# YuemingJin/STswinCL

Hardware: AMD Instinct MI355X
Metric: input frames/s, TswinPlus fwd+bwd+Adam, 4-frame 512x512 clips (higher is better)
Workload: dtype bf16; 1 GPU; BASELINE.json configs[1]: TswinPlus(12) seg train step, 4 clips/GPU x T=4 frames x 3x512x512, swin res (64,64), OHEM-CE, Adam; T=4 because the reference asserts it (swin_512.py:313); clips_per_gpu=4, frames_per_clip=4, parallelism=dp1, graph_requested=True

## Files before the change

include/stswin_hip.h:

```cpp
#ifndef STSWIN_HIP_H
#define STSWIN_HIP_H
#ifdef __cplusplus
extern "C" {
#endif

#define STSWIN_GF_GELU 1
#define STSWIN_GF_RESID 2
#define STSWIN_GF_MUL_DGELU 4
#define STSWIN_GF_OUT_F32 8
#define STSWIN_GF_ACCUM 16
#define STSWIN_GF_RELU 32
#define STSWIN_GF_MUL_R 8192
#define STSWIN_GF_C2_DGELU 16384
#define STSWIN_GF_CS_PARTIAL 32768
#define STSWIN_GF_CS_SQ 65536
#define STSWIN_GF_TAPSKIP (1 << 29)
#define STSWIN_GF_BIG 128
#define STSWIN_GF_MID 512
#define STSWIN_GF_NOPIPE 1024
#define STSWIN_GF_HALF 2048
#define STSWIN_GF_M32PP (1u << 31)
#define STSWIN_GF_W4R (1 << 30)
#define STSWIN_GF_ROT 4096
#define STSWIN_GF_NOBIG 256
#define STSWIN_GF_WAVES4 64
#define STSWIN_GF_NOREGEPI (1 << 22)
#define STSWIN_GF_NOSTREAM (1 << 23)
#define STSWIN_GF_DUO (1 << 24)
#define STSWIN_GF_STREAM (1 << 25)
#define STSWIN_GF_NONARROW (1 << 26)
#define STSWIN_GF_NODEEP (1 << 27)
#define STSWIN_GF_DEEP (1 << 28)

int stswin_abi_version(void);

int stswin_win_rowmap(int* map, int B, int T, int H, int W, int ws, int shift, int f0, int frames_total, void* stream);
int stswin_win_move(int dtype, const void* in, void* out, int B, int T, int H, int W, int C, int ws, int shift,
                    int f0, int frames_total, int dir, void* stream);
int stswin_merge_rowmap(int* map , int frames, int H, int W, void* stream);
int stswin_conv3x3_rowmap(int* map , int frames, int H, int W, int dilation, void* stream);
int stswin_conv_rowmap(int* map, int frames, int Hin, int Win, int Hout, int Wout, int k, int stride, int pad, int dilation,
                       int inverse, void* stream);
int stswin_stem_im2col(int dtype, const float* img, void* patches, long ld, int frames, int H, int W, int Ho, int Wo,
                       void* stream);
int stswin_stem_s2d(int dtype, const float* img, void* out, int frames, int H, int W, void* stream);
int stswin_stem_conv(const void* rec, const void* wmat, void* y, float* stats, int frames, int H, int W, void* stream);
long stswin_stem_wgrad_scratch(int frames, int Ho, int Wo);
int stswin_stem_wgrad(const void* dy, const void* rec, float* dw, int accumulate, float* scratch, long scratch_floats, int frames, int H, int W,
                      void* stream);
int stswin_conv_pack(int dtype, const float* w, void* fwd, void* dgrad, const int* omap, const int* imap, int co, int ci, int S,
                     int cop, int cip, void* stream);
int stswin_linear_pack(int dtype, const float* w, void* fwd, void* tr, int n, int k, void* stream);
int stswin_linear_pack_multi(int dtype, int count, const float* const* w, void* const* fwd, void* const* tr, const int* n, const int* k,
                             void* stream);
int stswin_conv_pack_multi(int dtype, int count, const float* const* w, void* const* fwd, void* const* dgrad, const int* const* omap,
                           const int* const* imap, const int* ci, const int* S, const int* cop, const int* cip, void* stream);
int stswin_maxpool3x3s2(int dtype, const void* in, long ldi, void* out, long ldo, unsigned char* arg, int frames, int H,
                        int W, int Ho, int Wo, int C, int backward, void* stream);
int stswin_conv3x3_c64(const void* x, const void* wmat, void* y, const void* resid, float* stats, int frames, int H, int W, int sign,
                       void* stream);
long stswin_conv3x3_c64_wgrad_scratch(int frames, int H, int W);
int stswin_conv3x3_c64_wgrad(const void* dy, const void* x, float* dw, int tapminor, int accumulate, float* scratch, long scratch_floats,
                             int frames, int H, int W, void* stream);

int stswin_gemm_nt(int dtype, const void* A, long lda, const int* a_rows, const void* B, long ldb, void* C, long ldc,
                   const int* c_rows, void* C2, long ldc2, const float* bias, const void* R, long ldr,
                   const int* r_rows, int M, int N, int Kseg, int S, float scale, int scale_cols, int flags,
                   float* colsum , void* stream);
int stswin_cs_reduce(const float* partials, int M, int N, float* out, void* stream);
#define STSWIN_TN_OVERWRITE (1 << 27)
#define STSWIN_TN_NO_COMBINE (1 << 26)
long stswin_gemm_nt_splitk_scratch(int M, int N, int Kseg, int S);
int stswin_gemm_nt_splitk(const void* A, long lda, const int* a_rows, const void* B, long ldb, void* C, long ldc, const float* bias, int M, int N,
                          int Kseg, int S, int relu, float* workspace, long workspace_floats, void* stream);
int stswin_tn_fused_hold(int delta);
int stswin_set_cu_budget(int cus);
int stswin_gemm_tn(int dtype, const void* At, long lda, const int* at_rows, const void* Bt, long ldb, const int* bt_rows,
                   float* C, long ldc, int Mk, int Ni, int Nj, int splits, int bseg,
                   float* workspace , long workspace_floats, void* stream);
#define STSWIN_TN_GROUP_DECLINED (-1050)
typedef struct stswin_tn_problem {
  const void* At; long lda; const int* at_rows;
  const void* Bt; long ldb; const int* bt_rows;
  float* C; long ldc;
  int Mk, Ni, Nj, bseg;
  int overwrite;
  int tapminor;
} stswin_tn_problem;
int stswin_gemm_tn_group(int dtype, int count, const stswin_tn_problem* problems, float* workspace, long workspace_floats, int* splits_out,
                         void* stream);
int stswin_tn_combine(const float* workspace, float* C, long ldc, int Ni, int Nj, int splits, int overwrite, int slab_bf16,
                      void* stream);
#define STSWIN_VAR_F32 100
#define STSWIN_VAR_NT_RING256_REGEPI 1
#define STSWIN_VAR_NT_RING256_LDSEPI 2
#define STSWIN_VAR_NT_RING256_NOPIPE 3
#define STSWIN_VAR_NT_RING256_W4 14
#define STSWIN_VAR_NT_STREAM 4
#define STSWIN_VAR_NT_DUO 5
#define STSWIN_VAR_NT_RING256x128_PP 6
#define STSWIN_VAR_NT_MID 7
#define STSWIN_VAR_NT_256x64 8
#define STSWIN_VAR_NT_128x64 9
#define STSWIN_VAR_NT_128x128 10
#define STSWIN_VAR_NT_128x128_W4 11
#define STSWIN_VAR_NT_SPLITK 13
#define STSWIN_VAR_NT_ROWS 12
#define STSWIN_VAR_TN_RING_PLAIN 20
#define STSWIN_VAR_TN_RING_ATROWS 21
#define STSWIN_VAR_TN_RING_BTROWS 22
#define STSWIN_VAR_TN_RING_BSEG 23
#define STSWIN_VAR_TN_128x128 30
#define STSWIN_VAR_TN_128x128_W4 31
#define STSWIN_VAR_TN_ROWS 32
#define STSWIN_VAR_TN_SLABS_F32 0x1000
#define STSWIN_VAR_TN_SLABS_BF16 0x2000
#define STSWIN_VAR_TN_FUSED 0x8000
#define STSWIN_VAR_TN_TAPMINOR 0x4000
#define STSWIN_TN_OUT_TAPMINOR (1 << 25)
int stswin_gemm_nt_qkv_fp8(const void* A, long lda, const int* a_rows, const void* B, long ldb, void* out8, long ld8, float* scales,
                           long ld_scales, const float* bias, int M, int N, int Kseg, float scale, int scale_cols, int rows_per_problem,
                           int head_dim, void* stream);
int stswin_win_attn_fwd_f8(const void* qkv8, long ld8, const float* scales, long ld_scales, void* out, long ldo, const float* biasT,
                           const float* maskT, int nB_, int nW, int T_frames, int ws, int heads, int C, int bias_windows,
                           const int* bias_index, void* stream);
int stswin_win_attn_bwd_f8(const void* qkv8, long ld8, const float* scales, long ld_scales, const void* dout, long lddo, void* dqkv, long lddq,
                           const float* biasT, const float* maskT, float* dbiasT, float* dqkv_colsum, int nB_, int nW, int T_frames, int ws,
                           int heads, int C, float scale, int bias_windows, const int* bias_index, float* scratch, long scratch_floats,
                           void* stream);
int stswin_last_variant(int family);
int stswin_tuning_build(void);

int stswin_slab_fold(const float* ws, long slab_stride, long ws_batch_stride, int nslabs, int seg_len, int nseg, float* out0, float* out1,
                     float* out2, long out_batch_stride, int batch, int accumulate, void* stream);

int stswin_fold_defer(int on, void* stream);
int stswin_fold_flush(void* stream);

long stswin_colsum_scratch(int M, int N);
int stswin_colsum(int dtype, const void* y, long ldy, float* out, int M, int N, float* scratch, void* stream);

int stswin_layernorm_fwd(int dtype, const void* x, long ldx, const int* rows, int S, int Cseg, void* y, long ldy,
                         const float* gamma, const float* beta, float* mean, float* rstd, int M, float eps, void* stream);
int stswin_layernorm_bwd(int dtype, const void* dy, long lddy, const void* x, long ldx, const int* rows, int S, int Cseg,
                         const float* gamma, const float* mean, const float* rstd, void* dx, long lddx, float* dgamma,
                         float* dbeta, int M, int accumulate_dx,
                         float* dxsum ,
                         float* scratch ,
                         void* stream);
int stswin_layernorm_bwd_add(int dtype, const void* dy, long lddy, const void* x, long ldx, const int* rows, int S, int Cseg,
                             const float* gamma, const float* mean, const float* rstd, const void* add, long ldadd, void* dx, long lddx,
                             float* dgamma, float* dbeta, int M, float* dxsum, float* scratch, void* stream);
long stswin_layernorm_bwd_scratch(int M, int C);

int stswin_vec_gather(const float* v, const int* map, float* out, int n, float fill, void* stream);
int stswin_vec_gather_multi(int count, const float* const* v, const int* map, float* const* out, int n, const float* fill, void* stream);

int stswin_bias_expand(const float* table, const long* index, const float* mask, float* out, int N, int heads, int nW,
                       void* stream);
int stswin_bias_expand_multi(int count, const float* const* table, const long* const* index, const float* const* mask, float* const* out,
                             const int* N, const int* heads, const int* nW, void* stream);
int stswin_bias_scatter(const float* dbiasT, const int* order, const int* offs, float* dtable, int N, int heads, int table_rows, int nslabs,
                        void* stream);

int stswin_win_attn_fwd(int dtype, const void* qkv, long ld, void* out, long ldo, const float* biasT, const float* maskT,
                        int nB_, int nW, int T_frames, int ws, int heads, int C, int bias_windows,
                        const int* bias_index, void* stream);
int stswin_win_attn_qkv_fwd(const void* x, long ldx, long x_rows, const int* rmap, const void* w, long ldw, const float* bqkv, void* qkv_out,
                            long ldq, void* out, long ldo, const float* biasT, int nB_, int nW, int T_frames, int ws, int heads, int C,
                            float scale, int bias_windows, const int* bias_index, void* stream);
int stswin_win_attn_fwd_fp8(const void* qkv, long ld, void* out, long ldo, const float* biasT, const float* maskT, int nB_, int nW,
                            int T_frames, int ws, int heads, int C, int bias_windows, const int* bias_index, void* stream);
int stswin_win_attn_bwd(int dtype, const void* qkv, long ld, const void* dout, long lddo, void* dqkv, long lddq,
                        const float* biasT, const float* maskT, float* dbiasT,
                        float* dqkv_q_colsum ,
                        int nB_, int nW, int T_frames, int ws,
                        int heads, int C, float scale, int bias_windows, const int* bias_index,
                        float* scratch , long scratch_floats, void* stream);
long stswin_win_attn_bwd_scratch(int nB_, int ws, int heads, int C);

int stswin_colstats(int dtype, const void* x, long ldx, float* sum , float* sumsq , int M, int C, int groups, int unit_rows,
                    float* scratch , void* stream);
long stswin_colstats_scratch(int dtype, int M, int C, int groups, int unit_rows);
int stswin_cs_group_reduce(const float* table, int M, int N, int groups, int unit_rows, float* sum, float* sumsq, void* stream);

int stswin_bn_table_finalize(const float* table, int M, int N, int groups, int unit_rows, float* mean, float* rstd,
                             float* running_mean, float* running_var, float eps, float momentum, void* stream);
int stswin_bn_finalize(int dtype, const void* x, long ldx, const float* sum, const float* sumsq, float* mean, float* rstd,
                       float* running_mean, float* running_var, int M, int C, int groups, float eps, float momentum,
                       int unit_rows, void* stream);
int stswin_bn_apply(int dtype, const void* x, long ldx, const float* mean, const float* rstd, const float* gamma,
                    const float* beta, const void* resid, long ldr, void* y, long ldy, int M, int C, int groups, int relu,
                    int unit_rows, void* stream);
int stswin_bn_bwd(int dtype, const void* dy, long lddy, const void* x, long ldx,
                  const void* y ,
                  long ldy, const float* mean, const float* rstd, const float* gamma, const float* beta ,
                  float* s1, float* s2, void* dx, long lddx, void* dresid, long lddr,
                  int M, int C, int groups, int relu, int training,
                  int phase ,
                  long rows_total , int unit_rows,
                  float* group_sums ,
                  float* scratch ,
                  void* stream);
long stswin_bn_bwd_scratch(int dtype, int M, int C, int groups, int unit_rows);
int stswin_bn_relu_pool(int dtype, const void* x, long ldx, const float* mean, const float* rstd, const float* gamma, const float* beta,
                        void* out, long ldo, unsigned char* arg, int frames, int H, int W, int C, int groups, int unit_rows, void* stream);
int stswin_rows_broadcast(int dtype, const float* v, void* out, long ldo, int M, int C, int groups, float scale,
                          int accumulate, void* stream);
int stswin_bilinear(int dtype, const void* in, long ldi, void* out, long ldo, int frames, int h, int w, int H, int W, int C,
                    int backward, void* stream);
int stswin_logits_upsample(int dtype, const void* tokens, long ldt, void* nchw, int frames, int h, int w, int H, int W,
                           int nc, int backward, void* stream);

int stswin_ce_fwd(int dtype, const void* logits, const long* labels, float* loss, float* stats, int frames, long HW, int nc,
                  int ignore_index, float thresh, void* stream);
#define STSWIN_OHEM_WORK_BYTES (3 * 2048 * 12 + 48)
int stswin_ohem_select(const float* loss, long n, long n_min, float thresh, const float* stats, void* work, long work_bytes,
                       float* value, float* sel, void* stream);
int stswin_ce_bwd(int dtype, const void* logits, const long* labels, const float* loss, const float* sel,
                  const float* gscale, void* dlogits, int frames, long HW, int nc, int ignore_index, void* stream);

int stswin_contrast_fwd(int dtype, const void* Q, long ldq, const void* const* K5, long ldk, const int* lq,
                        const int* const* lk5, float* pos, float* all, int N, int HW, int C, void* stream);

int stswin_contrast_bank_fwd(int dtype, const void* Q, long ldq, const int* lq, int M, int C, int q_sets, int q_block,
                             const void* bank, long ldb, const int* lb, int maps, int seg, int bank_block, int groups,
                             const int* gmap , float inv_tau, float* pos, float* all,
// ... 130 lines not shown
```

stswincl_amd/csrc/gemm.hip:

```cpp
#include "common.h"
#include "stswin_hip.h"
#include <cstdint>
#include <cstdlib>
#include <type_traits>

enum {
  GF_GELU = STSWIN_GF_GELU, GF_RESID = STSWIN_GF_RESID, GF_MUL_DGELU = STSWIN_GF_MUL_DGELU, GF_OUT_F32 = STSWIN_GF_OUT_F32,
  GF_ACCUM = STSWIN_GF_ACCUM, GF_RELU = STSWIN_GF_RELU, GF_MUL_R = STSWIN_GF_MUL_R, GF_C2_DGELU = STSWIN_GF_C2_DGELU,
  GF_CS_PARTIAL = STSWIN_GF_CS_PARTIAL, GF_CS_SQ = STSWIN_GF_CS_SQ, GF_TAPSKIP = STSWIN_GF_TAPSKIP,
  GF_WAVES4 = STSWIN_GF_WAVES4, GF_BIG = STSWIN_GF_BIG, GF_NOBIG = STSWIN_GF_NOBIG, GF_MID = STSWIN_GF_MID, GF_NOPIPE = STSWIN_GF_NOPIPE,
  GF_HALF = STSWIN_GF_HALF, GF_ROT = STSWIN_GF_ROT, GF_NOREGEPI = STSWIN_GF_NOREGEPI, GF_NOSTREAM = STSWIN_GF_NOSTREAM,
  GF_DUO = STSWIN_GF_DUO, GF_STREAM = STSWIN_GF_STREAM, GF_NONARROW = STSWIN_GF_NONARROW, GF_NODEEP = STSWIN_GF_NODEEP,
  GF_DEEP = STSWIN_GF_DEEP, GF_W4R = STSWIN_GF_W4R, GF_M32PP = (int)STSWIN_GF_M32PP,
};

#ifdef STSWIN_TUNING
#define STSWIN_DBG(flags, bit) (((flags) & (1 << (bit))) != 0)
#else
#define STSWIN_DBG(flags, bit) false
#endif
enum { GF_DEBUG_BITS = (1 << 17) | (1 << 18) | (1 << 19) | (1 << 20) | (1 << 21) };
#ifdef STSWIN_TUNING
static __device__ int g_dbg_stagger[2] = {8, 0};
extern "C" int stswin_debug_set_stagger(int phases, int ticks) {
// ... 216 lines not shown
    char* Bb = Ab + A_BYTES;
#pragma unroll
    for (int i = 0; i < NIA; ++i) glds16(abase[i] + (long)kt * astep[i], Ab + (w * NIA + i) * 1024);
#pragma unroll
    for (int i = 0; i < NIB; ++i) glds16(bbase[i] + (long)ktg * bstep[i], Bb + (w * NIB + i) * 1024);
  };

  f32x4 acc[4][JN];
#pragma unroll
  for (int i = 0; i < 4; ++i)
#pragma unroll
    for (int j = 0; j < JN; ++j) acc[i][j] = (f32x4){0.f, 0.f, 0.f, 0.f};

  int seg = 0, rseg = real_seg(0);
  load_a_bases(rseg);
  auto issue = [&](int tile) {
    const int nseg = tile / kps;
    if (nseg != seg) { seg = nseg; rseg = real_seg(seg); load_a_bases(rseg); }
    stage(rseg * kps + (tile - nseg * kps), tile - nseg * kps, tile % NST);
  };
#pragma unroll
  for (int s0 = 0; s0 < NST - 1; ++s0)
    if (s0 < nt) issue(s0);
  const int fr = l & 15, fq = l >> 4;
  for (int ktg = 0; ktg < nt; ++ktg) {
    if constexpr (NST == 2) {
      wait_vm0();
      __syncthreads();
    } else {
      if (ktg + NST - 1 <= nt) wait_vmcnt<(NST - 2) * (NIA + NIB)>();
      else wait_vm0();
      __builtin_amdgcn_s_barrier();
    }
    if (ktg + NST - 1 < nt) issue(ktg + NST - 1);
    const char* Ab = smem + (ktg % NST) * STAGE;
    const char* Bb = Ab + A_BYTES;
    if constexpr (TT<T>::IS_BF16) {
#pragma unroll
      for (int kk = 0; kk < 2; ++kk) {
        bf16x8 a[4], b[JN];
#pragma unroll
        for (int i = 0; i < 4; ++i) {
          const int row = wr * 64 + i * 16 + fr;
          a[i] = *(const bf16x8*)(Ab + row * ROWB + (((kk * 4 + fq) ^ (row & 7)) << 4));
        }
#pragma unroll
        for (int j = 0; j < JN; ++j) {
          const int row = wc * (16 * JN) + j * 16 + fr;
          b[j] = *(const bf16x8*)(Bb + row * ROWB + (((kk * 4 + fq) ^ (row & 7)) << 4));
        }
#pragma unroll
        for (int i = 0; i < 4; ++i)
#pragma unroll
          for (int j = 0; j < JN; ++j) acc[i][j] = __builtin_amdgcn_mfma_f32_16x16x32_bf16(a[i], b[j], acc[i][j], 0, 0, 0);
      }
    } else {
#pragma unroll
      for (int kk = 0; kk < 8; ++kk) {
        float a[4], b[JN];
#pragma unroll
        for (int i = 0; i < 4; ++i) {
          const int row = wr * 64 + i * 16 + fr;
          a[i] = *(const float*)(Ab + row * ROWB + ((kk ^ (row & 7)) << 4) + fq * 4);
        }
#pragma unroll
        for (int j = 0; j < JN; ++j) {
          const int row = wc * (16 * JN) + j * 16 + fr;
          b[j] = *(const float*)(Bb + row * ROWB + ((kk ^ (row & 7)) << 4) + fq * 4);
        }
#pragma unroll
        for (int i = 0; i < 4; ++i)
#pragma unroll
          for (int j = 0; j < JN; ++j) acc[i][j] = __builtin_amdgcn_mfma_f32_16x16x4f32(a[i], b[j], acc[i][j], 0, 0, 0);
      }
    }
  }

  constexpr int CG = BN / 8;
  const int c8 = (tid % CG) * 8;
  const int gn0 = n0 + c8;
  const int ncols = max(0, min(8, p.N - gn0));
  constexpr int RG = NW * 64 / CG;
  constexpr int NPASS = BM / RG;
  const bool pre_r = (p.flags & (GF_RESID | GF_MUL_DGELU | GF_MUL_R)) && ncols == 8 && (p.ldr % PACK) == 0;
  Vec16<T> rp[NPASS][8 / PACK];
  if (pre_r) {
#pragma unroll
    for (int pass = 0; pass < NPASS; ++pass) {
      const int gm = m0 + pass * RG + tid / CG;
      if (gm < p.M) epi_prefetch<T>(p, rp[pass], gm, gn0);
    }
  }
  __syncthreads();
  float* ct = (float*)smem;
#pragma unroll
  for (int i = 0; i < 4; ++i)
#pragma unroll
    for (int j = 0; j < JN; ++j)
#pragma unroll
      for (int r = 0; r < 4; ++r)
        ct[(wr * 64 + i * 16 + 4 * fq + r) * BN + wc * (16 * JN) + j * 16 + fr] = acc[i][j][r];
  __syncthreads();

  float bv[8], cs[8], cs2[8];
#pragma unroll
  for (int e = 0; e < 8; ++e) { bv[e] = (p.bias && e < ncols) ? p.bias[gn0 + e] : 0.f; cs[e] = 0.f; cs2[e] = 0.f; }
#pragma unroll
  for (int pass = 0; pass < NPASS; ++pass) {
    const int rr = pass * RG + tid / CG;
    const int gm = m0 + rr;
    if (gm >= p.M || ncols <= 0) break;
    float v[8];
    {
      const f32x4 lo = *(const f32x4*)(ct + rr * BN + c8);
      const f32x4 hi = *(const f32x4*)(ct + rr * BN + c8 + 4);
#pragma unroll
      for (int e = 0; e < 4; ++e) { v[e] = lo[e]; v[4 + e] = hi[e]; }
    }
    epi_piece<T>(p, v, bv, cs, gm, gn0, ncols, rp[pass], pre_r);
    if (p.flags & GF_CS_SQ) {
#pragma unroll
      for (int e = 0; e < 8; ++e) cs2[e] += v[e] * v[e];
    }
  }
  if (p.colsum) {
    __syncthreads();
#pragma unroll
    for (int e = 0; e < 8; ++e) ct[(tid / CG) * BN + c8 + e] = cs[e];
    __syncthreads();
    if (tid < BN && n0 + tid < p.N) {
      float t = 0.f;
#pragma unroll
      for (int k = 0; k < RG; ++k) t += ct[k * BN + tid];
      cs_emit(p, m0 / 128, BM / 128, n0 + tid, t);
    }
    if (p.flags & GF_CS_SQ) {
      __syncthreads();
#pragma unroll
      for (int e = 0; e < 8; ++e) ct[(tid / CG) * BN + c8 + e] = cs2[e];
      __syncthreads();
      if (tid < BN && n0 + tid < p.N) {
        float t = 0.f;
#pragma unroll
        for (int k = 0; k < RG; ++k) t += ct[k * BN + tid];
        cs_emit_sq(p, m0 / 128, BM / 128, n0 + tid, t);
      }
    }
  }
}


DEVI int swz64(int row) { return (4 - ((row >> 2) & 3)) & 3; }

template <int BM, int BN, int WM, int WN, int NST, int MINW, int PIPE, bool SWAP = false, bool PERSIST = false>
__global__ __launch_bounds__(WM * WN * 64, MINW) void gemm_nt_ring_kernel(GemmNT p) {
  using T = bf16;
  constexpr int BK = 32, ROWB = 64;
  constexpr int A_BYTES = BM * ROWB, B_BYTES = BN * ROWB, STAGE = A_BYTES + B_BYTES;
  constexpr int TM = BM / WM, TN = BN / WN;
  constexpr bool M32 = PIPE >= 2 && PIPE <= 4;
  constexpr int FRH = M32 ? 32 : 16, FCW = M32 ? 8 : 16;
  constexpr int FI = TM / FRH, FJ = TN / FCW;
  constexpr int NWV = WM * WN, NTHR = NWV * 64;
  constexpr int NIA = BM / 16 / NWV, NIB = BN / 16 / NWV;
  constexpr int PER_STAGE = NIA + NIB;
  constexpr int EROWS = SWAP ? BM : ((NST * STAGE) / (BN * 4) >= BM ? BM : ((NST * STAGE) / (BN * 4) / TM) * TM);
  static_assert(SWAP || (EROWS >= TM && BM % EROWS == 0), "epilogue slab");
  static_assert(!SWAP || BM * BN * 2 <= NST * STAGE, "register epilogue image");
  extern __shared__ __attribute__((aligned(16))) char smem[];
  const int tiles_n = (p.N + BN - 1) / BN, tiles_m = (p.M + BM - 1) / BM;
  const int ntot_ = tiles_m * tiles_n;
  int tix_ = blockIdx.x;
  do {
  int tid_ = threadIdx.x;
  if constexpr (PERSIST) asm volatile("" : "+v"(tid_));
  const int tid = tid_, l = tid & 63, w = __builtin_amdgcn_readfirstlane(tid >> 6);
  const int wr = w / WN, wc = w % WN;
  const int t = xcd_remap(tix_, ntot_);
  int tm = t / tiles_n, tn = t % tiles_n;
  if (tiles_n >= 24) {
    constexpr int GM = 8;
    const int per_group = GM * tiles_n, grp = t / per_group, first = grp * GM;
    const int rows = min(GM, tiles_m - first), in = t - grp * per_group;
    tm = first + in % rows;
    tn = in / rows;
  }
  const int m0 = tm * BM, n0 = tn * BN;

  const int rsub = l >> 2, cphys = l & 3, csrc = cphys ^ swz64(rsub);
  unsigned aoff[NIA], boff[NIB];
  const long arow_lim = (long)(0xFFFFFF00u / (unsigned)(p.lda * sizeof(T))) - 1;
  bool arow_bad = false;
#pragma unroll
  for (int i = 0; i < NIB; ++i) {
    const int gn = n0 + (w * NIB + i) * 16 + rsub;
    boff[i] = gn < p.N ? (unsigned)gn * (unsigned)(p.ldb * sizeof(T)) + csrc * 16 : 0xFFFFFFFFu;
  }
  auto load_a_bases = [&](int seg) {
#pragma unroll
    for (int i = 0; i < NIA; ++i) {
      const int gm = m0 + (w * NIA + i) * 16 + rsub;
      long row = -1;
      if (gm < p.M) row = p.a_rows ? (long)p.a_rows[(long)seg * p.M + gm] : (long)gm;
      aoff[i] = (row >= 0 && row <= arow_lim) ? (unsigned)row * (unsigned)(p.lda * sizeof(T)) + csrc * 16 : 0xFFFFFFFFu;
      arow_bad |= row > arow_lim;
    }
  };
  const int kps = p.Kseg / BK;
  const int qbase = p.qsplit > 0 ? (int)blockIdx.y * p.qsplit : 0;
  const int nt = p.qsplit > 0 ? min(p.qsplit, p.S * kps - qbase) : p.S * kps;
  if (p.qsplit > 0) p.C = (char*)p.C + (long)blockIdx.y * p.M * p.ldc * ((p.flags & GF_OUT_F32) ? 4 : 2);
  int seg = -1;
  auto issue = [&](int q) {
    const int Q = q + qbase;
    int sg = 0, kt = Q;
    if (p.S > 1) { sg = Q / kps; kt = Q - sg * kps; }
    if (sg != seg) { seg = sg; load_a_bases(sg); }
    char* Ab = smem + (q % NST) * STAGE;
    char* Bb = Ab + A_BYTES;
#pragma unroll
    for (int i = 0; i < NIA; ++i) glds16_buf(p.A, aoff[i], kt * (BK * (int)sizeof(T)), Ab + (w * NIA + i) * 1024);
#pragma unroll
    for (int i = 0; i < NIB; ++i) glds16_buf(p.B, boff[i], Q * (BK * (int)sizeof(T)), Bb + (w * NIB + i) * 1024);
  };

  f32x4 acc[M32 ? 1 : FI][M32 ? 1 : FJ];
  f32x16 acc32[M32 ? FI : 1][M32 ? FJ / 4 : 1];
  auto accg = [&](int i, int j) __attribute__((always_inline)) -> f32x4 {
    if constexpr (M32) {
      const int o = (j & 3) * 4;
      return (f32x4){acc32[i][j >> 2][o], acc32[i][j >> 2][o + 1], acc32[i][j >> 2][o + 2], acc32[i][j >> 2][o + 3]};
    } else return acc[i][j];
  };
  auto accs = [&](int i, int j, f32x4 v) __attribute__((always_inline)) {
    if constexpr (M32) {
      const int o = (j & 3) * 4;
      acc32[i][j >> 2][o] = v[0]; acc32[i][j >> 2][o + 1] = v[1]; acc32[i][j >> 2][o + 2] = v[2]; acc32[i][j >> 2][o + 3] = v[3];
    } else acc[i][j] = v;
  };

  const int fr = M32 ? (l & 31) : (l & 15), fq = M32 ? (l >> 5) : (l >> 4), fr15 = fr & 15;
  const int rd_off = fr * ROWB + ((fq ^ swz64(fr)) << 4);
  const int rd_off1 = rd_off ^ 32;
  const bool dbg_ts = STSWIN_DBG(p.flags, 19);
#ifdef STSWIN_TUNING
  unsigned long long dbg_c0 = 0;
  auto stamp = [&](int slot) {
    if (dbg_ts && tid == 0) {
      ((unsigned long long*)p.colsum)[(long)blockIdx.x * 16 + slot] = wall_clock64();
      if (slot == 2) dbg_c0 = clock64();
      if (slot == 3) ((unsigned long long*)p.colsum)[(long)blockIdx.x * 16 + 7] = clock64() - dbg_c0;
    }
  };
#else
  auto stamp = [&](int) {};
#endif
  constexpr bool R_EARLY_OK = SWAP && BM == 256 && BN == 256 && NST == 4 && PER_STAGE == 4 && NTHR == 512;
  bool r_early = false;
  auto issue_r_block = [&](int blk) {
#pragma unroll
    for (int qq = 0; qq < 4; ++qq) {
      const int row = (blk * 4 + qq) * 16 + w * 2 + (l >> 5);
      const int col = min(n0 + (((l & 31) ^ (row & 15)) << 3), p.N - 8);
      glds16_nt((const T*)p.R + (long)min(m0 + row, p.M - 1) * p.ldr + col, smem + ((blk * 4 + qq) * 16 + w * 2) * 512);
    }
  };
#ifdef STSWIN_TUNING
  if (STSWIN_DBG(p.flags, 17) && blockIdx.x < 256) {
    const int ph = g_dbg_stagger[0] > 0 ? g_dbg_stagger[0] : 8, tk = g_dbg_stagger[1] > 0 ? g_dbg_stagger[1] : (nt + 4) * 100 / 8;
    const unsigned long long t_go = wall_clock64() + (unsigned long long)(((blockIdx.x >> 3) % ph) * tk);
    while (wall_clock64() < t_go) __builtin_amdgcn_s_sleep(8);
  }
#endif
  stamp(0);
  auto epilogue = [&]() {
    if (STSWIN_DBG(p.flags, 21)) {
      float t = 0.f;
#pragma unroll
      for (int i = 0; i < FI; ++i)
#pragma unroll
        for (int j = 0; j < FJ; ++j) { const f32x4 q = accg(i, j); t += q[0] + q[1] + q[2] + q[3]; }
      if (t == 123.456f) ((T*)p.C)[tid] = from_f32<T>(t);
      return;
    }
    float* ct = (float*)smem;
    constexpr int CG = BN / 8;
    constexpr int RGP = NTHR / CG;
    const int c8 = (tid % CG) * 8;
    const int gn0 = n0 + c8;
    const int ncols = max(0, min(8, p.N - gn0));
    float bv[8], cs[8];
#pragma unroll
    for (int e = 0; e < 8; ++e) { bv[e] = (p.bias && e < ncols) ? p.bias[gn0 + e] : 0.f; cs[e] = 0.f; }
    constexpr int NPASS = EROWS / RGP;
    const bool pre_r = (p.flags & (GF_RESID | GF_MUL_DGELU | GF_MUL_R)) && ncols == 8 && (p.ldr % 8) == 0;
    Vec16<T> rp[NPASS][1];
#pragma unroll 1
    for (int slab = 0; slab < BM / EROWS; ++slab) {
      if (pre_r) {
#pragma unroll
        for (int pass = 0; pass < NPASS; ++pass) {
          const int gm = m0 + slab * EROWS + pass * RGP + tid / CG;
          if (gm < p.M) epi_prefetch<T>(p, rp[pass], gm, gn0);
        }
      }
      __syncthreads();
      if (wr * TM >= slab * EROWS && wr * TM < (slab + 1) * EROWS) {
        const int rbase = wr * TM - slab * EROWS;
#pragma unroll
        for (int i = 0; i < FI; ++i)
#pragma unroll
          for (int j = 0; j < FJ; ++j)
#pragma unroll
            for (int r = 0; r < 4; ++r) { if constexpr (!M32) ct[(rbase + i * 16 + 4 * fq + r) * BN + wc * TN + j * 16 + fr] = acc[i][j][r]; }
      }
      __syncthreads();
#pragma unroll
      for (int pass = 0; pass < NPASS; ++pass) {
        const int rr = pass * RGP + tid / CG;
        const int gm = m0 + slab * EROWS + rr;
        if (gm >= p.M || ncols <= 0) break;
        float v[8];
        const f32x4 lo = *(const f32x4*)(ct + rr * BN + c8);
        const f32x4 hi = *(const f32x4*)(ct + rr * BN + c8 + 4);
#pragma unroll
        for (int e = 0; e < 4; ++e) { v[e] = lo[e]; v[4 + e] = hi[e]; }
        epi_piece<T>(p, v, bv, cs, gm, gn0, ncols, rp[pass], pre_r);
      }
    }
    if (p.colsum) {
      __syncthreads();
#pragma unroll
      for (int e = 0; e < 8; ++e) ct[(tid / CG) * BN + c8 + e] = cs[e];
      __syncthreads();
      if (tid < BN && n0 + tid < p.N) {
        float tsum = 0.f;
#pragma unroll
        for (int k = 0; k < RGP; ++k) tsum += ct[k * BN + tid];
        cs_emit(p, m0 / 128, BM / 128, n0 + tid, tsum);
      }
    }

  };

  enum { E_BIAS = 1, E_SCALE = 2, E_GELU = 4, E_C2 = 8, E_RESID = 16, E_DGELU = 32, E_COLSUM = 64, E_RELU = 128, E_MULR = 256, E_C2D = 512,
         E_COLSQ = 1024 };
  auto epilogue_body = [&](auto tag) __attribute__((always_inline)) {
    constexpr int MD = decltype(tag)::value;
#define EPI_HAS(bit, rt) (MD >= 0 ? ((MD & (bit)) != 0) : (rt))
    constexpr int PITCH = BN * 2, CPRW = BN / 8, RPP = NTHR / CPRW, NPASS = BM / RPP;
    char* img = smem;
    const bool has_bias = EPI_HAS(E_BIAS, p.bias != nullptr), has_scale = EPI_HAS(E_SCALE, p.scale_cols > 0);
    const bool do_gelu = EPI_HAS(E_GELU, (p.flags & GF_GELU) != 0), has_c2 = EPI_HAS(E_C2, p.C2 != nullptr);
    const bool do_resid = EPI_HAS(E_RESID, (p.flags & GF_RESID) != 0), do_dgelu = EPI_HAS(E_DGELU, (p.flags & GF_MUL_DGELU) != 0);
    const bool do_cs = EPI_HAS(E_COLSUM, p.colsum != nullptr) && !dbg_ts, do_relu = EPI_HAS(E_RELU, (p.flags & GF_RELU) != 0);
    const bool do_mulr = EPI_HAS(E_MULR, (p.flags & GF_MUL_R) != 0), c2_dgelu = EPI_HAS(E_C2D, (p.flags & GF_C2_DGELU) != 0);
    const bool do_sq = do_cs && EPI_HAS(E_COLSQ, (p.flags & GF_CS_SQ) != 0);
    const bool has_r = do_resid || do_dgelu || do_mulr;
    const int colb = n0 + wc * TN + 4 * fq;
    f32x4 bj[FJ];
    if (has_bias) {
#pragma unroll
      for (int j = 0; j < FJ; ++j) bj[j] = *(const f32x4*)(p.bias + min(colb + j * FCW, p.N - 4));
    }
// ... 296 lines not shown
  };
  if constexpr (PIPE != 4) {
    for (int q = 0; q < (PIPE == 7 ? NST : NST - 1) && q < nt; ++q) issue(q);
  }
  if (p.stagger_ticks > 0 && blockIdx.x < 256 && gridDim.y == 1) {
    const unsigned long long t_go = wall_clock64() + (unsigned long long)(((blockIdx.x >> 3) & 7) * p.stagger_ticks);
    while (wall_clock64() < t_go) __builtin_amdgcn_s_sleep(8);
  }
  __builtin_amdgcn_sched_barrier(0);
  if constexpr (M32) {
#pragma unroll
    for (int i = 0; i < FI; ++i)
#pragma unroll
      for (int j = 0; j < FJ / 4; ++j)
#pragma unroll
        for (int e = 0; e < 16; ++e) acc32[i][j][e] = 0.f;
  } else {
#pragma unroll
    for (int i = 0; i < FI; ++i)
#pragma unroll
      for (int j = 0; j < FJ; ++j) acc[i][j] = (f32x4){0.f, 0.f, 0.f, 0.f};
  }
#ifdef STSWIN_TUNING
#include "gemm_nt_ring_tuning.inc"
#else
  static_assert(PIPE == 1 && !PERSIST, "the product library instantiates the ping-pong loop only (other loops: STSWIN_TUNING builds)");
#endif
  {
    static_assert(NST >= 4 && WM == 2, "ping-pong variant: 4-stage ring, two wave rows");
    const bool lag = (wr == 1);
    constexpr int NA = M32 ? 2 * FI : FI, NB = M32 ? FJ / 2 : FJ;
    bf16x8 a[NA], b[NB];
    auto read_frags = [&](int q) {
      const char* Ab = smem + (q % NST) * STAGE;
      const char* Bb = Ab + A_BYTES;
      if constexpr (M32) {
#pragma unroll
        for (int g = 0; g < NB; ++g) b[g] = *(const bf16x8*)(Bb + (wc * TN + (g >> 1) * 32) * ROWB + ((g & 1) ? rd_off1 : rd_off));
#pragma unroll
        for (int g = 0; g < NA; ++g) a[g] = *(const bf16x8*)(Ab + (wr * TM + (g >> 1) * 32) * ROWB + ((g & 1) ? rd_off1 : rd_off));
      } else {
#ifdef STSWIN_DEBUG_HALF_READS
#pragma unroll
      for (int j = 0; j < FJ; j += 2) { b[j] = *(const bf16x8*)(Bb + (wc * TN + j * 16) * ROWB + rd_off); b[j + 1] = b[j]; }
#pragma unroll
      for (int i = 0; i < FI; i += 2) { a[i] = *(const bf16x8*)(Ab + (wr * TM + i * 16) * ROWB + rd_off); a[i + 1] = a[i]; }
#else
#pragma unroll
      for (int j = 0; j < FJ; ++j) b[j] = *(const bf16x8*)(Bb + (wc * TN + j * 16) * ROWB + rd_off);
#pragma unroll
      for (int i = 0; i < FI; ++i) a[i] = *(const bf16x8*)(Ab + (wr * TM + i * 16) * ROWB + rd_off);
#endif
      }
    };
    auto mma_all = [&]() {
      __builtin_amdgcn_s_setprio(1);
      if constexpr (M32) {
        static_assert(!M32 || SWAP, "32x32x16 tiles: register epilogue only");
#pragma unroll
        for (int kh = 0; kh < 2; ++kh)
#pragma unroll
          for (int i = 0; i < FI; ++i)
#pragma unroll
            for (int j = 0; j < FJ / 4; ++j)
              acc32[i][j] = __builtin_amdgcn_mfma_f32_32x32x16_bf16(b[j * 2 + kh], a[i * 2 + kh], acc32[i][j], 0, 0, 0);
      } else {
#pragma unroll
      for (int i = 0; i < FI; ++i)
#pragma unroll
        for (int j = 0; j < FJ; ++j) {
          if constexpr (SWAP) acc[i][j] = __builtin_amdgcn_mfma_f32_16x16x32_bf16(b[j], a[i], acc[i][j], 0, 0, 0);
          else acc[i][j] = __builtin_amdgcn_mfma_f32_16x16x32_bf16(a[i], b[j], acc[i][j], 0, 0, 0);
        }
      }
      __builtin_amdgcn_s_setprio(0);
    };
    auto wait_tile = [&](int kt) {
      const int newer = min(NST - 2, nt - 1 - kt);
      if (newer >= 2) wait_vmcnt<2 * PER_STAGE>();
      else if (newer == 1) wait_vmcnt<PER_STAGE>();
      else wait_vmcnt<0>();
    };
    stamp(1);
    wait_tile(0);
    stamp(2);
    if (lag) __builtin_amdgcn_s_barrier();
    int kt = 0;
    if (p.S == 1) {
      for (; kt + NST - 1 < nt; ++kt) {
#ifdef STSWIN_DEBUG_LOOP_STAMPS
        if (kt == 4) stamp(1);
        if (kt == 8) stamp(2);
        if (kt == 12) stamp(7);
#endif
        __builtin_amdgcn_s_barrier();
        issue(kt + NST - 1);
        read_frags(kt);
        wait_vmcnt<2 * PER_STAGE>();
        __builtin_amdgcn_s_barrier();
        mma_all();
      }
      if constexpr (R_EARLY_OK) {
        if ((p.flags & (GF_RESID | GF_MUL_R | GF_MUL_DGELU)) && !p.r_rows && kt + NST - 1 == nt && !STSWIN_DBG(p.flags, 18)) {
          r_early = true;
          for (; kt < nt; ++kt) {
            __builtin_amdgcn_s_barrier();
            issue_r_block((kt + NST - 1) % NST);
            read_frags(kt);
            wait_vmcnt<2 * PER_STAGE>();
            __builtin_amdgcn_s_barrier();
            mma_all();
          }
        }
      }
      if (kt + NST - 1 == nt && NST == 4) {
        __builtin_amdgcn_s_barrier();
        read_frags(kt);
        wait_vmcnt<PER_STAGE>();
        __builtin_amdgcn_s_barrier();
        mma_all();
        ++kt;
        __builtin_amdgcn_s_barrier();
        read_frags(kt);
        wait_vmcnt<0>();
        __builtin_amdgcn_s_barrier();
        mma_all();
        ++kt;
        __builtin_amdgcn_s_barrier();
        read_frags(kt);
        __builtin_amdgcn_s_barrier();
        mma_all();
        ++kt;
      }
    }
    for (; kt < nt; ++kt) {
      __builtin_amdgcn_s_barrier();
      if (kt + NST - 1 < nt) issue(kt + NST - 1);
      read_frags(kt);
      if (lag && kt + 1 < nt) wait_tile(kt + 1);
      __builtin_amdgcn_s_barrier();
      mma_all();
      if (!lag && kt + 1 < nt) wait_tile(kt + 1);
    }
    if (!lag) __builtin_amdgcn_s_barrier();
    if (arow_bad) __builtin_trap();
    if constexpr (SWAP) epilogue_reg();
    else epilogue();
  }
  if constexpr (PERSIST) {
    tix_ += (int)gridDim.x;
    if (tix_ < ntot_) __syncthreads();
  }
  } while (PERSIST && tix_ < ntot_);
}


#ifdef STSWIN_TUNING
#include "gemm_nt_tuning_kernels.inc"
#endif

struct GemmTN {
  const void* At; long lda; const int* at_rows;
  const void* Bt; long ldb; const int* bt_rows;
  float* C; long ldc;
  int Mk, Ni, Nj;
  int splits;
  int bseg;
  float* slabs;
  int slab_bf16;
  unsigned* tile_cnt; int overwrite; int perm;
};

template <typename T, int NW>
__global__ __launch_bounds__(NW * 64) void gemm_tn_kernel(GemmTN p) {
  constexpr int WN = NW / 2, JN = 128 / WN / 16;
  constexpr int PACK = TT<T>::PACK;
  constexpr int BM = TT<T>::IS_BF16 ? 64 : 32;
  constexpr int ROWB = 128 * sizeof(T);
  constexpr int RPI = 1024 / ROWB;
  constexpr int NI = BM / (NW * RPI);
  constexpr int CPR = ROWB / 16;
  extern __shared__ __attribute__((aligned(16))) char smem[];
  const int tid = threadIdx.x, l = tid & 63, w = wave_id();
  const int wr = w / WN, wc = w % WN;
  const int tiles_j = (p.Nj + 127) >> 7;
  const int split_id = blockIdx.x % p.splits, tile_id = blockIdx.x / p.splits;
  const int i0 = (tile_id / tiles_j) << 7, j0 = (tile_id % tiles_j) << 7;
  const int ntile_all = (p.Mk + BM - 1) / BM;
  const int per = (ntile_all + p.splits - 1) / p.splits;
  const int t_begin = split_id * per, t_end = min(ntile_all, t_begin + per);
  if (t_begin >= t_end) return;

  const char* zero = (const char*)g_stswin_zero;
  const int rsub = l / CPR, cphys = l % CPR;
  long arow[NI], brow[NI];
  int bcol[NI];
  bool btap1[NI];
  const int tap0 = p.bseg > 0 ? j0 / p.bseg : 0;
  const int tap1 = p.bseg > 0 ? min(tap0 + 1, p.Nj / p.bseg - 1) : 0;
#pragma unroll
  for (int i = 0; i < NI; ++i) {
    const int r = (w * NI + i) * RPI + rsub;
    const int cj = j0 + ((cphys & ~15) | ((cphys ^ swz256(r)) & 15)) * PACK;
    bcol[i] = p.bseg > 0 ? cj % p.bseg : cj;
    btap1[i] = p.bseg > 0 && cj / p.bseg != tap0;
  }
  typedef int ivec __attribute__((ext_vector_type(RPI)));
  typedef const __attribute__((address_space(4))) ivec* civec;
  const bool vec_maps = (p.Mk % RPI) == 0;
  auto fetch_rows = [&](int tile) {
    const int mw = tile * BM + w * (NI * RPI);
#pragma unroll
    for (int i = 0; i < NI; ++i) {
      const int mb = mw + i * RPI;
      int va[RPI], vb0[RPI], vb1[RPI];
      if (vec_maps && mb + RPI <= p.Mk) {
        ivec ta, t0, t1;
#pragma unroll
        for (int r = 0; r < RPI; ++r) { ta[r] = mb + r; t0[r] = mb + r; t1[r] = -1; }
        if (p.at_rows) ta = *(civec)(p.at_rows + mb);
        if (p.bseg > 0) {
          t0 = *(civec)(p.bt_rows + (long)tap0 * p.Mk + mb);
          t1 = *(civec)(p.bt_rows + (long)tap1 * p.Mk + mb);
        } else if (p.bt_rows) {
          t0 = *(civec)(p.bt_rows + mb);
        }
#pragma unroll
        for (int r = 0; r < RPI; ++r) { va[r] = ta[r]; vb0[r] = t0[r]; vb1[r] = t1[r]; }
      } else {
#pragma unroll
        for (int r = 0; r < RPI; ++r) {
          const int m = mb + r, mc = min(m, p.Mk - 1);
          va[r] = p.at_rows ? sload(p.at_rows, mc) : mc;
          vb1[r] = -1;
          if (p.bseg > 0) {
            vb0[r] = sload(p.bt_rows, (long)tap0 * p.Mk + mc);
            vb1[r] = sload(p.bt_rows, (long)tap1 * p.Mk + mc);
          } else {
            vb0[r] = p.bt_rows ? sload(p.bt_rows, mc) : mc;
          }
          if (m >= p.Mk) { va[r] = -1; vb0[r] = -1; vb1[r] = -1; }
        }
      }
      int ra = -1, rb = -1;
#pragma unroll
      for (int r = 0; r < RPI; ++r)
        if (rsub == r) { ra = va[r]; rb = btap1[i] ? vb1[r] : vb0[r]; }
      arow[i] = ra; brow[i] = rb;
    }
  };
  auto stage = [&](int buf) {
    char* Ab = smem + buf * 32768;
    char* Bb = Ab + 16384;
#pragma unroll
    for (int i = 0; i < NI; ++i) {
      const int r = (w * NI + i) * RPI + rsub;
      const int cs = (cphys & ~15) | ((cphys ^ swz256(r)) & 15);
      const int ci = i0 + cs * PACK, cj = j0 + cs * PACK;
      const char* sa = (arow[i] >= 0 && ci < p.Ni) ? (const char*)p.At + (arow[i] * p.lda + ci) * sizeof(T) : zero;
      const char* sb = (brow[i] >= 0 && cj < p.Nj) ? (const char*)p.Bt + (brow[i] * p.ldb + bcol[i]) * sizeof(T) : zero;
      glds16_raw(sa, Ab + (w * NI + i) * 1024);
      glds16_raw(sb, Bb + (w * NI + i) * 1024);
    }
  };

  f32x4 acc[4][JN];
#pragma unroll
  for (int i = 0; i < 4; ++i)
#pragma unroll
    for (int j = 0; j < JN; ++j) acc[i][j] = (f32x4){0.f, 0.f, 0.f, 0.f};

  const int fr = l & 15, fq = l >> 4;
  const bool row_active = i0 + wr * 64 < p.Ni;
  fetch_rows(t_begin);
  stage(0);
  if (t_begin + 1 < t_end) fetch_rows(t_begin + 1);
  for (int tk = t_begin; tk < t_end; ++tk) {
    const int buf = (tk - t_begin) & 1;
    wait_vm0();
    __syncthreads();
    if (tk + 1 < t_end) stage(buf ^ 1);
    const char* Ab = smem + buf * 32768;
    const char* Bb = Ab + 16384;
    if (!row_active) {
    } else if constexpr (TT<T>::IS_BF16) {
#pragma unroll
      for (int kk = 0; kk < 2; ++kk) {
        bf16x8 a[4], b[JN];
#pragma unroll
        for (int i = 0; i < 4; ++i)
          a[i] = cat4(lds_tr4(Ab, ROWB, kk * 32 + 8 * fq, wr * 64 + i * 16),
                      lds_tr4(Ab, ROWB, kk * 32 + 8 * fq + 4, wr * 64 + i * 16));
#pragma unroll
        for (int j = 0; j < JN; ++j)
          b[j] = cat4(lds_tr4(Bb, ROWB, kk * 32 + 8 * fq, wc * (16 * JN) + j * 16),
                      lds_tr4(Bb, ROWB, kk * 32 + 8 * fq + 4, wc * (16 * JN) + j * 16));
#pragma unroll
        for (int i = 0; i < 4; ++i)
#pragma unroll
          for (int j = 0; j < JN; ++j) acc[i][j] = __builtin_amdgcn_mfma_f32_16x16x32_bf16(a[i], b[j], acc[i][j], 0, 0, 0);
      }
    } else {
#pragma unroll
      for (int kk = 0; kk < 8; ++kk) {
        const int row = kk * 4 + fq;
        float a[4], b[JN];
// ... 380 lines not shown
  const int seq = xcd_remap((int)blockIdx.x, (int)gridDim.x);
  if constexpr (M3 >= 0) {
    if (seq >= g.first[3]) { gemm_tn_ring_body<M3 < 0 ? 0 : M3, true>(g.q[3], seq - g.first[3], g.first[4] - g.first[3], (int)blockIdx.x); return; }
  }
  if constexpr (M2 >= 0) {
    if (seq >= g.first[2]) { gemm_tn_ring_body<M2 < 0 ? 0 : M2, true>(g.q[2], seq - g.first[2], g.first[3] - g.first[2], (int)blockIdx.x); return; }
  }
  if constexpr (M1 >= 0) {
    if (seq >= g.first[1]) { gemm_tn_ring_body<M1 < 0 ? 0 : M1, true>(g.q[1], seq - g.first[1], g.first[2] - g.first[1], (int)blockIdx.x); return; }
  }
  gemm_tn_ring_body<M0, true>(g.q[0], seq, g.first[1], (int)blockIdx.x);
}
__global__ __launch_bounds__(512, 2) void gemm_tn_ring_group_kernel(GemmTNGroup g) {
  const int seq = xcd_remap((int)blockIdx.x, (int)gridDim.x);
  int i = 0;
  while (i + 1 < g.count && seq >= g.first[i + 1]) ++i;
  const int local = seq - g.first[i], nwg = g.first[i + 1] - g.first[i];
  switch (g.mode[i]) {
    case 0: gemm_tn_ring_body<0, true>(g.q[i], local, nwg, (int)blockIdx.x); break;
    case 1: gemm_tn_ring_body<1, true>(g.q[i], local, nwg, (int)blockIdx.x); break;
    case 2: gemm_tn_ring_body<2, true>(g.q[i], local, nwg, (int)blockIdx.x); break;
    default: gemm_tn_ring_body<3, true>(g.q[i], local, nwg, (int)blockIdx.x); break;
  }
}

__global__ __launch_bounds__(256) void tn_reduce_kernel(const float* slabs, float* C, long ldc, int Ni, int Nj, int splits,
                                                        int overwrite, int slab_bf16, int perm) {
  if (slab_bf16) {
    const long idx = ((long)blockIdx.x * 256 + threadIdx.x) * 8;
    const long total = (long)Ni * Nj;
    if (idx >= total) return;
    const int i = idx / Nj, j = idx % Nj;
    float a[8] = {0.f, 0.f, 0.f, 0.f, 0.f, 0.f, 0.f, 0.f};
    const bf16* src = (const bf16*)slabs + idx;
    int s = 0;
    for (; s + 8 <= splits; s += 8) {
      bf16x8 v[8];
#pragma unroll
      for (int u = 0; u < 8; ++u) v[u] = *(const bf16x8*)(src + (long)(s + u) * total);
#pragma unroll
      for (int u = 0; u < 8; ++u)
#pragma unroll
        for (int e = 0; e < 8; ++e) a[e] += (float)v[u][e];
    }
    for (; s < splits; ++s) {
      const bf16x8 v = *(const bf16x8*)(src + (long)s * total);
#pragma unroll
      for (int e = 0; e < 8; ++e) a[e] += (float)v[e];
    }
    if (perm > 0) {
      const int S = Nj / perm, sg = j / perm, c = j - sg * perm;
      float* d = C + (long)i * ldc + (long)c * S + sg;
#pragma unroll
      for (int e = 0; e < 8; ++e) d[(long)e * S] = overwrite ? a[e] : d[(long)e * S] + a[e];
      return;
    }
    float* dst = C + (long)i * ldc + j;
    if ((ldc & 3) == 0) {
      f32x4 lo = {a[0], a[1], a[2], a[3]}, hi = {a[4], a[5], a[6], a[7]};
      if (!overwrite) { lo += *(const f32x4*)dst; hi += *(const f32x4*)(dst + 4); }
      *(f32x4*)dst = lo;
      *(f32x4*)(dst + 4) = hi;
    } else {
      for (int e = 0; e < 8; ++e) dst[e] = overwrite ? a[e] : dst[e] + a[e];
    }
    return;
  }
  const long idx = ((long)blockIdx.x * 256 + threadIdx.x) * 4;
  if (idx >= (long)Ni * Nj) return;
  const int i = idx / Nj, j = idx % Nj;
  f32x4 a = {0.f, 0.f, 0.f, 0.f};
  for (int s = 0; s < splits; ++s) a += *(const f32x4*)(slabs + (long)s * Ni * Nj + idx);
  if (perm > 0) {
    const int S = Nj / perm, sg = j / perm, c = j - sg * perm;
    float* d = C + (long)i * ldc + (long)c * S + sg;
#pragma unroll
    for (int e = 0; e < 4; ++e) d[(long)e * S] = overwrite ? a[e] : d[(long)e * S] + a[e];
    return;
  }
  float* dst = C + (long)i * ldc + j;
  if (overwrite) {
    if ((ldc & 3) == 0) *(f32x4*)dst = a;
    else { for (int e = 0; e < 4; ++e) dst[e] = a[e]; }
  } else if ((ldc & 3) == 0) { *(f32x4*)dst = *(const f32x4*)dst + a; }
  else { for (int e = 0; e < 4; ++e) dst[e] += a[e]; }
}

static thread_local int g_last_variant[2] = {0, 0};
extern "C" int stswin_tuning_build() {
#ifdef STSWIN_TUNING
  return 1;
#else
  return 0;
#endif
}
extern "C" int stswin_last_variant(int family) { return family >= 0 && family < 2 ? g_last_variant[family] : -1; }

static int set_lds_once(const void* fn) {
  return (int)hipFuncSetAttribute(fn, hipFuncAttributeMaxDynamicSharedMemorySize, 65536);
}

extern "C" int stswin_cs_reduce(const float* partials, int M, int N, float* out, void* stream) {
  if (M <= 0 || N <= 0) return 0;
  if (N % 4) return -1004;
  const int rows = 2 * ((M + 255) / 256);
  const int rc = stswin_fold_launch(partials, N, 0, rows, N, 1, out, nullptr, nullptr, 0, 1, 1, (hipStream_t)stream);
  if (rc) return rc;
  STSWIN_CHECK_LAUNCH();
  return 0;
}

__global__ __launch_bounds__(256) void gemm_nt_rows_kernel(GemmNT p) {
  const int l = threadIdx.x & 63, n = blockIdx.x * 4 + (threadIdx.x >> 6);
  if (n >= p.N) return;
  const bf16* A = (const bf16*)p.A;
  const bf16* Bn = (const bf16*)p.B + (long)n * p.ldb;
  float acc[8] = {0, 0, 0, 0, 0, 0, 0, 0};
  for (int k = l * 8; k < p.Kseg; k += 512) {
    const bf16x8 b = *(const bf16x8*)(Bn + k);
#pragma unroll
    for (int m = 0; m < 8; ++m)
      if (m < p.M) {
        const bf16x8 a = *(const bf16x8*)(A + (long)m * p.lda + k);
#pragma unroll
        for (int e = 0; e < 8; ++e) acc[m] += (float)a[e] * (float)b[e];
      }
  }
#pragma unroll
  for (int m = 0; m < 8; ++m)
    if (m < p.M) {
      float v = wave_sum(acc[m]);
      if (l == 0) {
        if (p.bias) v += p.bias[n];
        if (p.flags & GF_RELU) v = fmaxf(v, 0.f);
        ((bf16*)p.C)[(long)m * p.ldc + n] = (bf16)v;
      }
    }
}
__global__ __launch_bounds__(256) void gemm_tn_rows_kernel(const bf16* At, long lda, const bf16* Bt, long ldb, float* C, long ldc, int Mk, int Ni,
                                                           int Nj, int overwrite) {
  const long idx = (long)blockIdx.x * 256 + threadIdx.x;
  const int pj = Nj / 4;
  if (idx >= (long)Ni * pj) return;
  const int i = (int)(idx / pj), j = (int)(idx % pj) * 4;
  f32x4 v = overwrite ? f32x4{0.f, 0.f, 0.f, 0.f} : *(const f32x4*)(C + (long)i * ldc + j);
  for (int m = 0; m < Mk; ++m) {
    const float a = (float)At[(long)m * lda + i];
    const bf16x4 b = *(const bf16x4*)(Bt + (long)m * ldb + j);
    v += f32x4{a * (float)b[0], a * (float)b[1], a * (float)b[2], a * (float)b[3]};
  }
  *(f32x4*)(C + (long)i * ldc + j) = v;
}

__global__ __launch_bounds__(256) void nt_splitk_combine_kernel(const float* ws, int splits, long slab, int M, int N, bf16* C, long ldc, const float* bias,
                                                                int relu) {
  const long idx = (long)blockIdx.x * 256 + threadIdx.x;
  const int pn = N / 8;
  if (idx >= (long)M * pn) return;
  const int m = (int)(idx / pn), n = (int)(idx % pn) * 8;
  const float* src = ws + (long)m * N + n;
  f32x4 a = *(const f32x4*)src, b = *(const f32x4*)(src + 4);
  for (int j = 1; j < splits; ++j) {
    a += *(const f32x4*)(src + j * slab);
    b += *(const f32x4*)(src + j * slab + 4);
  }
  bf16x8 o;
#pragma unroll
  for (int e = 0; e < 8; ++e) {
    float v = (e < 4 ? a[e] : b[e - 4]) + (bias ? bias[n + e] : 0.f);
    if (relu) v = fmaxf(v, 0.f);
    o[e] = (bf16)v;
  }
  *(bf16x8*)(C + (long)m * ldc + n) = o;
}

__global__ __launch_bounds__(256) void nt_splitk_combine16_kernel(const bf16* ws, int splits, long slab, int M, int N, bf16* C, long ldc, const float* bias,
                                                                  int relu) {
  const long idx = (long)blockIdx.x * 256 + threadIdx.x;
  const int pn = N / 8;
  if (idx >= (long)M * pn) return;
  const int m = (int)(idx / pn), n = (int)(idx % pn) * 8;
  const bf16* src = ws + (long)m * N + n;
  float a[8] = {0, 0, 0, 0, 0, 0, 0, 0};
  for (int j = 0; j < splits; ++j) {
    const bf16x8 v = *(const bf16x8*)(src + j * slab);
#pragma unroll
    for (int e = 0; e < 8; ++e) a[e] += (float)v[e];
  }
  bf16x8 o;
#pragma unroll
  for (int e = 0; e < 8; ++e) {
    float v = a[e] + (bias ? bias[n + e] : 0.f);
    if (relu) v = fmaxf(v, 0.f);
    o[e] = (bf16)v;
  }
  *(bf16x8*)(C + (long)m * ldc + n) = o;
}

static int nt_splitk_plan(int M, int N, int Kseg, int S, int* qsplit_o) {
  if (M < 256 || N < 256 || N % 8 || Kseg % 32) return 0;
  const long tiles = (long)((M + 255) / 256) * ((N + 255) / 256);
  const int nt = S * (Kseg / 32);
  if (tiles > 32 || nt < 64) return 0;
  int splits = (int)(256 / tiles);
  if (splits > nt / 16) splits = nt / 16;
  if (splits < 2) return 0;
  const int qs = (nt + splits - 1) / splits;
  *qsplit_o = qs;
  return (nt + qs - 1) / qs;
}
extern "C" long stswin_gemm_nt_splitk_scratch(int M, int N, int Kseg, int S) {
  int qs = 0;
  const int splits = nt_splitk_plan(M, N, Kseg, S, &qs);
  return splits ? (long)splits * M * N : 0;
}
extern "C" int stswin_gemm_nt_splitk(const void* A, long lda, const int* a_rows, const void* B, long ldb, void* C, long ldc, const float* bias, int M,
                                     int N, int Kseg, int S, int relu, float* workspace, long workspace_floats, void* stream) {
  int qs = 0;
  const int splits = nt_splitk_plan(M, N, Kseg, S, &qs);
  if (!splits) return -1008;
  if (M <= 0 || N <= 0 || Kseg <= 0 || S <= 0 || lda % 8 || ldb % 8) return -1001;
  if (ldc % 8 || ((uintptr_t)C & 15)) return -1008;
  if (!workspace || workspace_floats < (long)splits * M * N) return -1009;
  if ((a_rows ? false : (long)M * lda * 2 > 0xFFFF0000L) || (long)N * ldb * 2 > 0xFFFF0000L) return -1008;
  const char* e16 = getenv("STSWIN_SPLITK_BF16");
  const int b16 = e16 && atoi(e16) ? 1 : 0;
  GemmNT p{A, lda, a_rows, B, ldb, workspace, N, nullptr, nullptr, 0, nullptr, nullptr, 0, nullptr, M, N, Kseg, S, 1.0f, 0, b16 ? 0 : GF_OUT_F32, nullptr, qs};
  static const int attr = (int)hipFuncSetAttribute((const void*)gemm_nt_ring_kernel<256, 256, 2, 4, 4, 2, true>, hipFuncAttributeMaxDynamicSharedMemorySize, 131072) |
                          (int)hipFuncSetAttribute((const void*)gemm_nt_ring_kernel<256, 256, 2, 4, 4, 2, true, true>, hipFuncAttributeMaxDynamicSharedMemorySize, 131072);
  if (attr != 0) return -attr;
  const long tiles = (long)((M + 255) / 256) * ((N + 255) / 256);
  g_last_variant[0] = STSWIN_VAR_NT_SPLITK | (splits << 16);
  if (b16) hipLaunchKernelGGL((gemm_nt_ring_kernel<256, 256, 2, 4, 4, 2, true, true>), dim3((unsigned)tiles, (unsigned)splits), dim3(512), 131072, (hipStream_t)stream, p);
  else hipLaunchKernelGGL((gemm_nt_ring_kernel<256, 256, 2, 4, 4, 2, true>), dim3((unsigned)tiles, (unsigned)splits), dim3(512), 131072, (hipStream_t)stream, p);
  STSWIN_CHECK_LAUNCH();
  const long n = (long)M * (N / 8);
  if (b16) hipLaunchKernelGGL(nt_splitk_combine16_kernel, dim3((unsigned)((n + 255) / 256)), dim3(256), 0, (hipStream_t)stream, (const bf16*)workspace, splits, (long)M * N, M, N,
                     (bf16*)C, ldc, bias, relu);
  else hipLaunchKernelGGL(nt_splitk_combine_kernel, dim3((unsigned)((n + 255) / 256)), dim3(256), 0, (hipStream_t)stream, workspace, splits, (long)M * N, M, N,
                     (bf16*)C, ldc, bias, relu);
  STSWIN_CHECK_LAUNCH();
  return 0;
}

extern "C" int stswin_gemm_nt_qkv_fp8(const void* A, long lda, const int* a_rows, const void* B, long ldb, void* out8, long ld8,
                                      float* scales, long ld_scales, const float* bias, int M, int N, int Kseg, float scale, int scale_cols,
                                      int rows_per_problem, int head_dim, void* stream) {
  if (M <= 0 || N <= 0 || M % 256 || N % 256 || Kseg <= 0 || Kseg % 32 || lda % 8 || ldb % 8) return -1001;
  if ((rows_per_problem != 32 && rows_per_problem != 128) || (head_dim != 128 && head_dim != 256) || scale_cols % head_dim || N % head_dim)
    return -1010;
  if (ld8 % 16 || ((uintptr_t)out8 & 15) || !scales || ld_scales < N / head_dim || (bias && ((uintptr_t)bias & 15))) return -1011;
  if ((!a_rows && (long)M * lda * 2 > 0xFFFF0000L) || (long)N * ldb * 2 > 0xFFFF0000L) return -1008;
  GemmNT p{A, lda, a_rows, B, ldb, out8, ld8, nullptr, scales, ld_scales, bias, nullptr, 0, nullptr, M, N, Kseg, 1, scale, scale_cols, 0, nullptr, 0,
           rows_per_problem, head_dim};
  static const int attr = (int)hipFuncSetAttribute((const void*)gemm_nt_ring_kernel<256, 256, 2, 4, 4, 2, true, true>, hipFuncAttributeMaxDynamicSharedMemorySize, 131072);
  if (attr != 0) return -attr;
  const long tiles = (long)(M / 256) * (N / 256);
  g_last_variant[0] = STSWIN_VAR_NT_RING256_REGEPI;
  hipLaunchKernelGGL((gemm_nt_ring_kernel<256, 256, 2, 4, 4, 2, true, true>), dim3((unsigned)tiles), dim3(512), 131072, (hipStream_t)stream, p);
  STSWIN_CHECK_LAUNCH();
  return 0;
}

extern "C" int stswin_gemm_nt(int dtype, const void* A, long lda, const int* a_rows, const void* B, long ldb,
                              void* C, long ldc, const int* c_rows, void* C2, long ldc2, const float* bias,
                              const void* R, long ldr, const int* r_rows, int M, int N, int Kseg, int S,
                              float scale, int scale_cols, int flags, float* colsum, void* stream) {
  if (M <= 0 || N <= 0) return 0;
#ifndef STSWIN_TUNING
  flags &= ~(GF_MID | GF_HALF | GF_DUO | GF_STREAM | GF_NOPIPE | GF_W4R | GF_M32PP | GF_ROT | GF_DEBUG_BITS);
#endif
  const int bk = dtype == 0 ? 64 : 32;
  if (Kseg <= 0 || Kseg % bk || S <= 0) return -1001;
  if ((flags & GF_ACCUM) && !(flags & GF_OUT_F32)) return -1002;
  if ((flags & GF_CS_SQ) && (!(flags & GF_CS_PARTIAL) || !colsum || (flags & (GF_MID | GF_HALF | GF_DUO | GF_STREAM | GF_NOREGEPI))))
    return -1006;
  if ((flags & GF_CS_PARTIAL) && colsum && ((M + 127) / 128) % 2) {
    stswin_zero_bytes(colsum + (long)(2 * ((M + 255) / 256) - 1) * N, sizeof(float) * N, (hipStream_t)stream);
    if (flags & GF_CS_SQ)
      stswin_zero_bytes(colsum + (long)(4 * ((M + 255) / 256) - 1) * N, sizeof(float) * N, (hipStream_t)stream);
  }
  GemmNT p{A, lda, a_rows, B, ldb, C, ldc, c_rows, C2, ldc2, bias, R, ldr, r_rows, M, N, Kseg, S, scale, scale_cols, flags, colsum};
  if (dtype == 0 && M <= 8 && S == 1 && !a_rows && !c_rows && !C2 && !R && !colsum && !(flags & ~GF_RELU) && scale_cols == 0 && Kseg % 8 == 0 &&
      lda % 8 == 0 && ldb % 8 == 0) {
    g_last_variant[0] = STSWIN_VAR_NT_ROWS;
    hipLaunchKernelGGL(gemm_nt_rows_kernel, dim3((unsigned)((N + 3) / 4)), dim3(256), 0, (hipStream_t)stream, p);
    STSWIN_CHECK_LAUNCH();
    return 0;
  }
  const int nblk = ((M + 127) / 128) * ((N + 127) / 128);
  static int once = set_lds_once((const void*)gemm_nt_kernel<bf16, 4>) | set_lds_once((const void*)gemm_nt_kernel<float, 4>) |
                    set_lds_once((const void*)gemm_nt_kernel<bf16, 8>) | set_lds_once((const void*)gemm_nt_kernel<float, 8>);
  (void)once;
  const bool w8 = (flags & GF_WAVES4) == 0;
  const long big_tiles = (long)((M + 255) / 256) * ((N + 255) / 256);
  const long rounds = (big_tiles + 255) / 256;
  const bool fills = big_tiles * 10 >= rounds * 256 * 9;
  const bool fits32 = (a_rows || (long)M * lda * 2 <= 0xFFFF0000L) && (long)N * ldb * 2 <= 0xFFFF0000L;
  bool big = dtype == 0 && Kseg % 32 == 0 && N >= 256 && M >= 256 && fills && fits32 && !(flags & (GF_NOBIG | GF_WAVES4));
  if ((flags & GF_BIG) && dtype == 0 && Kseg % 32 == 0 && fits32) big = true;
  const bool regepi_ok = !(flags & (GF_OUT_F32 | GF_ACCUM | GF_NOREGEPI)) && N % 8 == 0 && ldc % 8 == 0 && (!C2 || ldc2 % 8 == 0) &&
                         (!R || ldr % 8 == 0) && ((uintptr_t)C % 16 == 0) && (!C2 || (uintptr_t)C2 % 16 == 0) &&
                         (!R || (uintptr_t)R % 16 == 0) && (!bias || (uintptr_t)bias % 16 == 0);
  if ((flags & GF_CS_SQ) && !regepi_ok && !(flags & GF_BIG)) big = false;
  const bool mid_ok = dtype == 0 && Kseg % 32 == 0 && fits32 && !(flags & (GF_NOBIG | GF_WAVES4));
  const bool mid = (flags & GF_MID) && mid_ok;
  const long half_tiles = (long)((M + 255) / 256) * ((N + 127) / 128);
  const long hrounds = (half_tiles + 255) / 256;
  const bool hfills = half_tiles * 10 >= hrounds * 256 * 9;
  (void)hfills;
#ifdef STSWIN_TUNING
  const bool half = (flags & GF_HALF) && mid_ok && !mid;
  if (half && !(flags & GF_BIG)) {
    static int once_half = (int)hipFuncSetAttribute((const void*)gemm_nt_ring_kernel<256, 128, 2, 4, 4, 2, true>, hipFuncAttributeMaxDynamicSharedMemorySize, 98304);
    (void)once_half;
    g_last_variant[0] = STSWIN_VAR_NT_RING256x128_PP;
    hipLaunchKernelGGL((gemm_nt_ring_kernel<256, 128, 2, 4, 4, 2, true>), dim3((unsigned)half_tiles), dim3(512), 98304, (hipStream_t)stream, p);
    STSWIN_CHECK_LAUNCH();
    return 0;
  }
#endif
  if (big && !mid) {
    static int once_big = (int)hipFuncSetAttribute((const void*)gemm_nt_ring_kernel<256, 256, 2, 4, 4, 2, true>, hipFuncAttributeMaxDynamicSharedMemorySize, 131072);
    (void)once_big;
    const bool regepi = !(flags & (GF_OUT_F32 | GF_ACCUM | GF_NOREGEPI)) && N % 8 == 0 && ldc % 8 == 0 && (!C2 || ldc2 % 8 == 0) &&
                        (!R || ldr % 8 == 0) && ((uintptr_t)C % 16 == 0) && (!C2 || (uintptr_t)C2 % 16 == 0) &&
                        (!R || (uintptr_t)R % 16 == 0) && (!bias || (uintptr_t)bias % 16 == 0);
    static int once_swap = (int)hipFuncSetAttribute((const void*)gemm_nt_ring_kernel<256, 256, 2, 4, 4, 2, true, true>, hipFuncAttributeMaxDynamicSharedMemorySize, 131072);
    (void)once_swap;
    if ((flags & GF_CS_SQ) && (!regepi || (flags & GF_NOPIPE))) return -1006;
#ifdef STSWIN_TUNING
    if (regepi && (flags & GF_DUO) && !(flags & GF_NOPIPE)) {
      static int once_duo7 = (int)hipFuncSetAttribute((const void*)gemm_nt_ring_kernel<128, 256, 1, 4, 3, 2, 7, true>, hipFuncAttributeMaxDynamicSharedMemorySize, 73728);
      (void)once_duo7;
      const long duo_tiles = (long)((M + 127) / 128) * ((N + 255) / 256);
      g_last_variant[0] = STSWIN_VAR_NT_DUO;
      hipLaunchKernelGGL((gemm_nt_ring_kernel<128, 256, 1, 4, 3, 2, 7, true>), dim3((unsigned)duo_tiles), dim3(256), 73728, (hipStream_t)stream, p);
      STSWIN_CHECK_LAUNCH();
      return 0;
    }
#endif
#ifdef STSWIN_TUNING
    const bool streamk = regepi && S == 1 && !a_rows && (flags & GF_STREAM) && !(flags & (GF_NOPIPE | GF_NOSTREAM));
    if (streamk) {
      static int once_stream = (int)hipFuncSetAttribute((const void*)gemm_nt_stream_kernel, hipFuncAttributeMaxDynamicSharedMemorySize, 163840);
      (void)once_stream;
      const unsigned grid = (unsigned)(big_tiles < 256 ? big_tiles : 256);
      g_last_variant[0] = STSWIN_VAR_NT_STREAM;
      hipLaunchKernelGGL(gemm_nt_stream_kernel, dim3(grid), dim3(512), 163840, (hipStream_t)stream, p);
      STSWIN_CHECK_LAUNCH();
      return 0;
    }
    if (regepi && (flags & GF_DUO) && (flags & GF_NOPIPE)) {
      static int once_duo = (int)hipFuncSetAttribute((const void*)gemm_nt_ring_kernel<128, 256, 1, 4, 3, 2, false, true>, hipFuncAttributeMaxDynamicSharedMemorySize, 73728);
      (void)once_duo;
      const long duo_tiles = (long)((M + 127) / 128) * ((N + 255) / 256);
      g_last_variant[0] = STSWIN_VAR_NT_DUO;
      hipLaunchKernelGGL((gemm_nt_ring_kernel<128, 256, 1, 4, 3, 2, false, true>), dim3((unsigned)duo_tiles), dim3(256), 73728, (hipStream_t)stream, p);
      STSWIN_CHECK_LAUNCH();
      return 0;
    }
    if (flags & GF_NOPIPE) {
      static int once_np = (int)hipFuncSetAttribute((const void*)gemm_nt_ring_kernel<256, 256, 2, 4, 4, 2, false>, hipFuncAttributeMaxDynamicSharedMemorySize, 131072);
      (void)once_np;
      g_last_variant[0] = STSWIN_VAR_NT_RING256_NOPIPE;
      hipLaunchKernelGGL((gemm_nt_ring_kernel<256, 256, 2, 4, 4, 2, false>), dim3((unsigned)big_tiles), dim3(512), 131072, (hipStream_t)stream, p);
      STSWIN_CHECK_LAUNCH();
      return 0;
    }
#endif
#ifdef STSWIN_TUNING
    static const int env_w4 = getenv("STSWIN_NT_W4") ? atoi(getenv("STSWIN_NT_W4")) : 0;
    if (regepi && (env_w4 == 6 || ((flags & GF_ROT) && (flags & GF_W4R)))) {
      static int once_swp = (int)hipFuncSetAttribute((const void*)gemm_nt_ring_kernel<256, 256, 2, 4, 4, 2, 6, true>, hipFuncAttributeMaxDynamicSharedMemorySize, 131072);
      (void)once_swp;
      g_last_variant[0] = STSWIN_VAR_NT_RING256_W4 + 4;
      hipLaunchKernelGGL((gemm_nt_ring_kernel<256, 256, 2, 4, 4, 2, 6, true>), dim3((unsigned)big_tiles), dim3(512), 131072, (hipStream_t)stream, p);
      STSWIN_CHECK_LAUNCH();
      return 0;
    }
    if (regepi && (env_w4 == 5 || (flags & GF_ROT))) {
      static int once_rot = (int)hipFuncSetAttribute((const void*)gemm_nt_ring_kernel<256, 256, 2, 4, 4, 2, 5, true>, hipFuncAttributeMaxDynamicSharedMemorySize, 131072);
      (void)once_rot;
      g_last_variant[0] = STSWIN_VAR_NT_RING256_W4 + 3;
      hipLaunchKernelGGL((gemm_nt_ring_kernel<256, 256, 2, 4, 4, 2, 5, true>), dim3((unsigned)big_tiles), dim3(512), 131072, (hipStream_t)stream, p);
      STSWIN_CHECK_LAUNCH();
      return 0;
    }
    if (regepi && (env_w4 == 3 || ((flags & GF_M32PP) && (flags & GF_W4R)))) {
      static int once_rs = (int)hipFuncSetAttribute((const void*)gemm_nt_ring_kernel<256, 256, 2, 2, 4, 1, 4, true>, hipFuncAttributeMaxDynamicSharedMemorySize, 131072);
      (void)once_rs;
      g_last_variant[0] = STSWIN_VAR_NT_RING256_W4 + 2;
      hipLaunchKernelGGL((gemm_nt_ring_kernel<256, 256, 2, 2, 4, 1, 4, true>), dim3((unsigned)big_tiles), dim3(256), 131072, (hipStream_t)stream, p);
      STSWIN_CHECK_LAUNCH();
// ... 100 lines not shown
    return 0;
  }
  if (dtype == 0 && w8 && (flags & GF_DEEP)) {
    static int once_d = (int)hipFuncSetAttribute((const void*)gemm_nt_kernel<bf16, 8, 128, 128, 3>, hipFuncAttributeMaxDynamicSharedMemorySize, 98304);
    (void)once_d;
    g_last_variant[0] = STSWIN_VAR_NT_128x128;
    hipLaunchKernelGGL((gemm_nt_kernel<bf16, 8, 128, 128, 3>), dim3(nblk), dim3(512), 98304, (hipStream_t)stream, p);
    STSWIN_CHECK_LAUNCH();
    return 0;
  }
  g_last_variant[0] = (w8 ? STSWIN_VAR_NT_128x128 : STSWIN_VAR_NT_128x128_W4) + (dtype ? STSWIN_VAR_F32 : 0);
  if (dtype == 0) {
    if (w8) hipLaunchKernelGGL((gemm_nt_kernel<bf16, 8>), dim3(nblk), dim3(512), 65536, (hipStream_t)stream, p);
    else hipLaunchKernelGGL((gemm_nt_kernel<bf16, 4>), dim3(nblk), dim3(256), 65536, (hipStream_t)stream, p);
  } else {
    if (w8) hipLaunchKernelGGL((gemm_nt_kernel<float, 8>), dim3(nblk), dim3(512), 65536, (hipStream_t)stream, p);
    else hipLaunchKernelGGL((gemm_nt_kernel<float, 4>), dim3(nblk), dim3(256), 65536, (hipStream_t)stream, p);
  }
  STSWIN_CHECK_LAUNCH();
  return 0;
}

static long tn_resident_workgroups() {
  static thread_local int dev_cached = -1;
  static thread_local long cus = 0;
  int dev = 0;
  if (hipGetDevice(&dev) != hipSuccess) return 0;
  if (dev != dev_cached) {
    int n = 0;
    if (hipDeviceGetAttribute(&n, hipDeviceAttributeMultiprocessorCount, dev) != hipSuccess) n = 0;
    cus = n;
    dev_cached = dev;
  }
  return cus;
}
#include <atomic>
__global__ __launch_bounds__(256) void tn_zero_fill_kernel(float* __restrict__ C, long ldc, int Ni, int Nj) {
  const long n4 = (long)Ni * ((Nj + 3) / 4);
  for (long i = (long)blockIdx.x * 256 + threadIdx.x; i < n4; i += (long)gridDim.x * 256) {
    const long r = i / ((Nj + 3) / 4);
    const int c = (int)(i - r * ((Nj + 3) / 4)) * 4;
    float* q = C + r * ldc + c;
    if (c + 3 < Nj && ((((uintptr_t)q) & 15) == 0)) *(f32x4*)q = (f32x4){0.f, 0.f, 0.f, 0.f};
    else
      for (int e = 0; e < 4 && c + e < Nj; ++e) q[e] = 0.f;
  }
}
static void tn_zero_fill(float* C, long ldc, int Ni, int Nj, hipStream_t stream) {
  const long n4 = (long)Ni * ((Nj + 3) / 4);
  long blocks = (n4 + 255) / 256;
  if (blocks > 4096) blocks = 4096;
  if (blocks < 1) blocks = 1;
  hipLaunchKernelGGL(tn_zero_fill_kernel, dim3((unsigned)blocks), dim3(256), 0, stream, C, ldc, Ni, Nj);
}

#include <mutex>
static std::mutex g_tn_mutex;
static std::atomic<int> g_tn_fused_holds{0};
static unsigned* tn_tile_counters(int tiles, hipStream_t stream) {
  constexpr int REGIONS = 16, PER = 3 * 1024;
  static unsigned* bufs[64] = {nullptr};
  static hipStream_t owners[64][REGIONS];
  static int nown[64] = {0};
  int dev = 0;
  if (tiles > 1024 || hipGetDevice(&dev) != hipSuccess || dev < 0 || dev >= 64) return nullptr;
  std::lock_guard<std::mutex> lock(g_tn_mutex);
  if (!bufs[dev]) {
    hipStreamCaptureStatus cs = hipStreamCaptureStatusNone;
    if (hipStreamIsCapturing(stream, &cs) != hipSuccess || cs != hipStreamCaptureStatusNone) { (void)hipGetLastError(); return nullptr; }
    unsigned* b = nullptr;
    if (hipMalloc((void**)&b, sizeof(unsigned) * REGIONS * PER) != hipSuccess) { (void)hipGetLastError(); return nullptr; }
    if (hipMemset(b, 0, sizeof(unsigned) * REGIONS * PER) != hipSuccess) { (void)hipGetLastError(); (void)hipFree(b); return nullptr; }
    bufs[dev] = b;
  }
  int r = -1;
  for (int i = 0; i < nown[dev]; ++i)
    if (owners[dev][i] == stream) { r = i; break; }
  if (r < 0) {
    if (nown[dev] >= REGIONS) return nullptr;
    r = nown[dev]++;
    owners[dev][r] = stream;
  }
  return bufs[dev] + (size_t)r * PER;
}
static std::atomic<int> g_cu_budget{0};
extern "C" int stswin_set_cu_budget(int cus) {
  const int old = g_cu_budget.load();
  g_cu_budget.store(cus > 0 ? cus : 0);
  return old;
}
int stswin_cu_budget() {
  const int b = g_cu_budget.load();
  return b > 0 ? b : 256;
}

extern "C" int stswin_tn_fused_hold(int delta) {
  if (delta > 0) return g_tn_fused_holds.fetch_add(1) + 1;
  if (delta < 0) {
    int cur = g_tn_fused_holds.load();
    while (cur > 0 && !g_tn_fused_holds.compare_exchange_weak(cur, cur - 1)) {}
    return cur > 0 ? cur - 1 : 0;
  }
  return g_tn_fused_holds.load();
}

typedef stswin_tn_problem StswinTnProblem;
extern "C" int stswin_gemm_tn_group(int dtype, int count, const StswinTnProblem* pr, float* workspace, long workspace_floats,
                                    int* splits_out, void* stream) {
  if (count <= 0) return 0;
  if (count > TN_GROUP_MAX || !pr) return -1052;
  const int declined = -1050;
  if (dtype != 0 || !workspace) return declined;
  { const char* f32_env = getenv("STSWIN_TN_F32_SLABS"); if (f32_env && atoi(f32_env)) return declined; }
  { const char* ef = getenv("STSWIN_TN_FUSED"); if (ef ? atoi(ef) == 0 : g_tn_fused_holds.load() != 0) return declined; }
  { const char* eg = getenv("STSWIN_TN_GROUP"); if (eg && atoi(eg) == 0) return declined; }
  int tiles[TN_GROUP_MAX], nst[TN_GROUP_MAX], rs[TN_GROUP_MAX];
  long tile_stages = 0, total_tiles = 0;
  for (int i = 0; i < count; ++i) {
    const StswinTnProblem& q = pr[i];
    if (q.Mk <= 0 || q.Ni <= 0 || q.Nj <= 0) return -1052;
    if (q.Ni % 8 || q.Nj % 8 || q.lda % 8 || q.ldb % 8) return -1003;
    if (q.bseg < 0 || (q.bseg > 0 && (q.bseg % 8 || !q.bt_rows || q.Nj % q.bseg))) return -1004;
    if (q.Ni < 256 || q.Nj < 256 || q.ldc < 0 || (q.at_rows && q.bt_rows) || ((q.at_rows || q.bt_rows) && q.Mk % 32 != 0)) return declined;
    if ((!q.at_rows && (long)q.Mk * q.lda * 2 > 0xFFFF0000L) || (!q.bt_rows && (long)q.Mk * q.ldb * 2 > 0xFFFF0000L)) return declined;
    if (q.bseg > 0)
      for (int j0 = 0; j0 < q.Nj; j0 += 256)
        if ((j0 + 255 < q.Nj ? j0 + 255 : q.Nj - 1) / q.bseg - j0 / q.bseg > 1) return declined;
    if (q.tapminor && q.bseg <= 0) return -1052;
    tiles[i] = ((q.Ni + 255) / 256) * ((q.Nj + 255) / 256);
    nst[i] = (q.Mk + 31) / 32;
    tile_stages += (long)tiles[i] * nst[i];
    total_tiles += tiles[i];
  }
  if (total_tiles > 1024) return declined;
  const int cus = stswin_cu_budget();
  if (cus > tn_resident_workgroups()) return declined;
  long target = (tile_stages + cus - 1) / cus;
  if (target < 16) target = 16;
  const char* ew = getenv("STSWIN_TN_GROUP_W");
  const long wmap = ew && atoi(ew) >= 100 && atoi(ew) <= 300 ? atoi(ew) : 105;
  long total = 0;
  for (int guard = 0; guard < 4096; ++guard, ++target) {
    total = 0;
    for (int i = 0; i < count; ++i) {
      const long wi = (pr[i].at_rows || pr[i].bt_rows) ? wmap : 100;
      int r = (int)((nst[i] * wi + target * 100 - 1) / (target * 100));
      if (r < 1) r = 1;
      const int per = (nst[i] + r - 1) / r;
      rs[i] = (nst[i] + per - 1) / per;
      total += (long)tiles[i] * rs[i];
    }
    if (total <= cus) break;
  }
  if (total > cus || total * 8 < (long)cus * 7) return declined;
  {
    long wsum = 0, wmax = 0;
    for (int i = 0; i < count; ++i) {
      const long wi = (pr[i].at_rows || pr[i].bt_rows) ? wmap : 100;
      const long per = (nst[i] + rs[i] - 1) / rs[i];
      wsum += (long)tiles[i] * nst[i] * wi;
      if (per * wi > wmax) wmax = per * wi;
    }
    if (wmax * cus * 100 > wsum * 115) return declined;
  }
  long ws_need = 0;
  for (int i = 0; i < count; ++i) {
    if ((long)rs[i] * pr[i].Ni * pr[i].Nj * 2 >= 0x7FFFFFF0L) return declined;
    ws_need += ((long)rs[i] * pr[i].Ni * pr[i].Nj + 1) / 2 + 64;
    ws_need = (ws_need + 63) / 64 * 64;
  }
  if (ws_need > workspace_floats) return declined;
  unsigned* cnt = tn_tile_counters((int)total_tiles, (hipStream_t)stream);
  if (!cnt) return declined;
  GemmTNGroup g;
  g.count = count;
  g.first[0] = 0;
  long wo = 0, to = 0;
  for (int i = 0; i < count; ++i) {
    const StswinTnProblem& q = pr[i];
    const int perm = (q.tapminor && q.bseg > 0) ? q.bseg : 0;
    g.q[i] = GemmTN{q.At, q.lda, q.at_rows, q.Bt, q.ldb, q.bt_rows, q.C, q.ldc, q.Mk, q.Ni, q.Nj, rs[i], q.bseg, workspace + wo, 1,
                    cnt + 3 * to, q.overwrite ? 1 : 0, perm};
    g.mode[i] = q.at_rows ? 1 : (q.bt_rows ? (q.bseg > 0 ? 3 : 2) : 0);
    g.first[i + 1] = g.first[i] + tiles[i] * rs[i];
    wo += ((long)rs[i] * q.Ni * q.Nj + 1) / 2 + 64;
    wo = (wo + 63) / 64 * 64;
    to += tiles[i];
    if (splits_out) splits_out[i] = rs[i];
  }
  for (int i = count; i < TN_GROUP_MAX; ++i) { g.q[i] = g.q[0]; g.mode[i] = 0; g.first[i + 1] = g.first[count]; }
  static int once_g = (int)hipFuncSetAttribute((const void*)gemm_tn_ring_group_kernel, hipFuncAttributeMaxDynamicSharedMemorySize, 131072) |
                      (int)hipFuncSetAttribute((const void*)gemm_tn_ring_group_static_kernel<0, 1, 2, -1>, hipFuncAttributeMaxDynamicSharedMemorySize, 131072) |
                      (int)hipFuncSetAttribute((const void*)gemm_tn_ring_group_static_kernel<0, 0, -1, -1>, hipFuncAttributeMaxDynamicSharedMemorySize, 131072) |
                      (int)hipFuncSetAttribute((const void*)gemm_tn_ring_group_static_kernel<0, 0, 1, 2>, hipFuncAttributeMaxDynamicSharedMemorySize, 131072);
  (void)once_g;
  g_last_variant[1] = STSWIN_VAR_TN_RING_PLAIN | STSWIN_VAR_TN_SLABS_BF16 | STSWIN_VAR_TN_FUSED | (rs[0] << 16);
  const bool m012 = count == 3 && g.mode[0] == 0 && g.mode[1] == 1 && g.mode[2] == 2;
  const bool m00 = count == 2 && g.mode[0] == 0 && g.mode[1] == 0;
  const bool m0012 = count == 4 && g.mode[0] == 0 && g.mode[1] == 0 && g.mode[2] == 1 && g.mode[3] == 2;
  static const char* egd = getenv("STSWIN_TN_GROUP_DYNAMIC");
  if (m012 && !(egd && atoi(egd))) hipLaunchKernelGGL((gemm_tn_ring_group_static_kernel<0, 1, 2, -1>), dim3((unsigned)total), dim3(512), 131072, (hipStream_t)stream, g);
  else if (m00 && !(egd && atoi(egd))) hipLaunchKernelGGL((gemm_tn_ring_group_static_kernel<0, 0, -1, -1>), dim3((unsigned)total), dim3(512), 131072, (hipStream_t)stream, g);
  else if (m0012 && !(egd && atoi(egd))) hipLaunchKernelGGL((gemm_tn_ring_group_static_kernel<0, 0, 1, 2>), dim3((unsigned)total), dim3(512), 131072, (hipStream_t)stream, g);
  else
  hipLaunchKernelGGL(gemm_tn_ring_group_kernel, dim3((unsigned)total), dim3(512), 131072, (hipStream_t)stream, g);
  STSWIN_CHECK_LAUNCH();
  return 0;
}

extern "C" int stswin_gemm_tn(int dtype, const void* At, long lda, const int* at_rows, const void* Bt, long ldb,
                              const int* bt_rows, float* C, long ldc, int Mk, int Ni, int Nj, int splits, int bseg,
                              float* workspace, long workspace_floats, void* stream) {
  if (Mk <= 0 || Ni <= 0 || Nj <= 0) return 0;
  const int overwrite = (splits > 0 && (splits & (1 << 27))) ? 1 : 0;
  const int no_combine = (splits > 0 && (splits & (1 << 26))) ? 1 : 0;
  if (splits > 0) splits &= ~(1 << 26);
  const int perm = (splits > 0 && (splits & (1 << 25)) && bseg > 0 && !no_combine) ? bseg : 0;
  if (splits > 0) splits &= ~(1 << 25);
  const char* f32_env = getenv("STSWIN_TN_F32_SLABS");
  const int f32_slabs = f32_env && atoi(f32_env) ? 1 : 0;
  const int slab_bf16 = (dtype == 0 && !f32_slabs) ? 1 : 0;
  if (splits > 0) splits &= ~(1 << 27);
  const int splits_flags_w4 = (splits > 0 && (splits & (1 << 30))) ? 1 : 0;
  if (splits > 0) splits &= ~(1 << 30);
  const int pack = dtype == 0 ? 8 : 4;
  if (Ni % pack || Nj % pack || lda % pack || ldb % pack) return -1003;
  if (bseg < 0 || (bseg > 0 && (bseg % pack || !bt_rows || Nj % bseg))) return -1004;
  if (dtype == 0 && Mk <= 8 && !at_rows && !bt_rows && bseg == 0 && ldc % 4 == 0) {
    g_last_variant[1] = STSWIN_VAR_TN_ROWS;
    const long nthr = (long)Ni * (Nj / 4);
    hipLaunchKernelGGL(gemm_tn_rows_kernel, dim3((unsigned)((nthr + 255) / 256)), dim3(256), 0, (hipStream_t)stream, (const bf16*)At, lda, (const bf16*)Bt,
                       ldb, C, ldc, Mk, Ni, Nj, overwrite);
    STSWIN_CHECK_LAUNCH();
    return 0;
  }
  if (bseg > 0)
    for (int j0 = 0; j0 < Nj; j0 += 128)
      if ((j0 + 127 < Nj ? j0 + 127 : Nj - 1) / bseg - j0 / bseg > 1) return -1005;
  const int bm = dtype == 0 ? 64 : 32;
  const int ntile = (Mk + bm - 1) / bm;
  const bool force_ring = splits > 0 && (splits & (1 << 29));
  const bool no_ring = splits > 0 && (splits & (1 << 28));
  if (splits > 0) splits &= ~((1 << 29) | (1 << 28));
  bool ring = dtype == 0 && !splits_flags_w4 && !no_ring && (force_ring || (splits <= 0 && Ni >= 256 && Nj >= 256));
  if (ring && (at_rows || bt_rows) && ((at_rows && bt_rows) || Mk % 32 != 0)) ring = false;
  if (ring && ((!at_rows && (long)Mk * lda * 2 > 0xFFFF0000L) || (!bt_rows && (long)Mk * ldb * 2 > 0xFFFF0000L)))
    ring = false;
  if (ring && bseg > 0)
    for (int j0 = 0; j0 < Nj; j0 += 256)
      if ((j0 + 255 < Nj ? j0 + 255 : Nj - 1) / bseg - j0 / bseg > 1) ring = false;
  if (ring) {
    const int t256 = ((Ni + 255) / 256) * ((Nj + 255) / 256);
    const int nst = (Mk + 31) / 32;
    const int cus = stswin_cu_budget();
    int rs = splits > 0 ? splits : cus / t256;
    if (splits <= 0) {
      const int max_by_k = nst / 16 > 0 ? nst / 16 : 1;
      if (rs > max_by_k) rs = max_by_k;
      if (rs < 1) rs = 1;
      while (rs > 1 && workspace && (long)rs * Ni * Nj > workspace_floats) --rs;
      const long blocks = (long)t256 * rs;
      if (blocks < cus * 11 / 16 || (blocks > cus && blocks % cus != 0 && blocks % cus < cus * 25 / 32)) ring = false;
    }
    if (rs > nst) rs = nst;
    { const int per = (nst + rs - 1) / rs; rs = (nst + per - 1) / per; }
    if (ring) {
      const bool slabs = workspace && rs > 1 && (long)rs * Ni * Nj <= workspace_floats;
      if (overwrite && !slabs) tn_zero_fill(C, ldc, Ni, Nj, (hipStream_t)stream);
      unsigned* tile_cnt = nullptr;
      if (slabs && slab_bf16 && !no_combine && ldc >= 0 && (long)t256 * rs <= tn_resident_workgroups() && (long)rs * Ni * Nj * 2 < 0x7FFFFFF0L) {
        const char* ef = getenv("STSWIN_TN_FUSED");
        const bool on = ef ? atoi(ef) != 0 : g_tn_fused_holds.load() == 0;
        if (on) tile_cnt = tn_tile_counters(t256, (hipStream_t)stream);
      }
      GemmTN q{At, lda, at_rows, Bt, ldb, bt_rows, C, ldc, Mk, Ni, Nj, rs, bseg, slabs ? workspace : nullptr, slab_bf16, tile_cnt, overwrite, perm};
      static int once_r = (int)hipFuncSetAttribute((const void*)gemm_tn_ring_kernel<0>, hipFuncAttributeMaxDynamicSharedMemorySize, 131072) |
                          (int)hipFuncSetAttribute((const void*)gemm_tn_ring_kernel<1>, hipFuncAttributeMaxDynamicSharedMemorySize, 131072) |
                          (int)hipFuncSetAttribute((const void*)gemm_tn_ring_kernel<2>, hipFuncAttributeMaxDynamicSharedMemorySize, 131072) |
                          (int)hipFuncSetAttribute((const void*)gemm_tn_ring_kernel<3>, hipFuncAttributeMaxDynamicSharedMemorySize, 131072) |
                          (int)hipFuncSetAttribute((const void*)gemm_tn_ring_kernel<0, true>, hipFuncAttributeMaxDynamicSharedMemorySize, 131072) |
                          (int)hipFuncSetAttribute((const void*)gemm_tn_ring_kernel<1, true>, hipFuncAttributeMaxDynamicSharedMemorySize, 131072) |
                          (int)hipFuncSetAttribute((const void*)gemm_tn_ring_kernel<2, true>, hipFuncAttributeMaxDynamicSharedMemorySize, 131072) |
                          (int)hipFuncSetAttribute((const void*)gemm_tn_ring_kernel<3, true>, hipFuncAttributeMaxDynamicSharedMemorySize, 131072);
      (void)once_r;
      const dim3 grid((unsigned)(t256 * rs));
      g_last_variant[1] = (at_rows ? STSWIN_VAR_TN_RING_ATROWS : (bt_rows && bseg > 0) ? STSWIN_VAR_TN_RING_BSEG : bt_rows ? STSWIN_VAR_TN_RING_BTROWS : STSWIN_VAR_TN_RING_PLAIN) |
                          (slabs ? (slab_bf16 ? STSWIN_VAR_TN_SLABS_BF16 : STSWIN_VAR_TN_SLABS_F32) : 0) | ((slabs && perm) ? 0x4000 : 0) | (rs << 16) |
                          (tile_cnt ? STSWIN_VAR_TN_FUSED : 0);
      if (tile_cnt) {
        if (at_rows) hipLaunchKernelGGL((gemm_tn_ring_kernel<1, true>), grid, dim3(512), 131072, (hipStream_t)stream, q);
        else if (bt_rows && bseg > 0) hipLaunchKernelGGL((gemm_tn_ring_kernel<3, true>), grid, dim3(512), 131072, (hipStream_t)stream, q);
        else if (bt_rows) hipLaunchKernelGGL((gemm_tn_ring_kernel<2, true>), grid, dim3(512), 131072, (hipStream_t)stream, q);
        else hipLaunchKernelGGL((gemm_tn_ring_kernel<0, true>), grid, dim3(512), 131072, (hipStream_t)stream, q);
        STSWIN_CHECK_LAUNCH();
        return 0;
      }
      if (at_rows) hipLaunchKernelGGL(gemm_tn_ring_kernel<1>, grid, dim3(512), 131072, (hipStream_t)stream, q);
      else if (bt_rows && bseg > 0) hipLaunchKernelGGL(gemm_tn_ring_kernel<3>, grid, dim3(512), 131072, (hipStream_t)stream, q);
      else if (bt_rows) hipLaunchKernelGGL(gemm_tn_ring_kernel<2>, grid, dim3(512), 131072, (hipStream_t)stream, q);
      else hipLaunchKernelGGL(gemm_tn_ring_kernel<0>, grid, dim3(512), 131072, (hipStream_t)stream, q);
      if (slabs && !no_combine) {
        const long n4 = slab_bf16 ? ((long)Ni * Nj + 7) / 8 : ((long)Ni * Nj + 3) / 4;
        hipLaunchKernelGGL(tn_reduce_kernel, dim3((unsigned)((n4 + 255) / 256)), dim3(256), 0, (hipStream_t)stream, workspace, C, ldc,
                           Ni, Nj, rs, overwrite, slab_bf16, perm);
      }
      STSWIN_CHECK_LAUNCH();
      return 0;
    }
  }
  if (splits <= 0) {
    const int tiles = ((Ni + 127) / 128) * ((Nj + 127) / 128);
    int rounds = 1;
    if (at_rows || bt_rows)
      for (int r = 4; r >= 2; --r)
        if (ntile / (r * 512 / tiles > 0 ? r * 512 / tiles : 1) >= 32) { rounds = r; break; }
    splits = rounds * 512 / tiles;
    if (splits < 1) splits = 1;
    const int max_by_k = ntile / 8 > 0 ? ntile / 8 : 1;
    if (splits > max_by_k) splits = max_by_k;
    if (splits >= 8) splits &= ~7;
    else { int p2 = 1; while (p2 * 2 <= splits) p2 *= 2; splits = p2; }
  }
  if (splits > ntile) splits = ntile;
  { const int per = (ntile + splits - 1) / splits; splits = (ntile + per - 1) / per; }
  const bool use_slabs = workspace && splits > 1 && (long)splits * Ni * Nj <= workspace_floats;
  if (overwrite && !use_slabs) tn_zero_fill(C, ldc, Ni, Nj, (hipStream_t)stream);
  GemmTN p{At, lda, at_rows, Bt, ldb, bt_rows, C, ldc, Mk, Ni, Nj, splits, bseg, use_slabs ? workspace : nullptr, slab_bf16, nullptr, 0, 0};
  dim3 grid(((Ni + 127) / 128) * ((Nj + 127) / 128) * splits);
  static int once = set_lds_once((const void*)gemm_tn_kernel<bf16, 4>) | set_lds_once((const void*)gemm_tn_kernel<float, 4>) |
                    set_lds_once((const void*)gemm_tn_kernel<bf16, 8>) | set_lds_once((const void*)gemm_tn_kernel<float, 8>);
  (void)once;
  const bool w8 = splits_flags_w4 == 0;
  g_last_variant[1] = ((w8 ? STSWIN_VAR_TN_128x128 : STSWIN_VAR_TN_128x128_W4) + (dtype ? STSWIN_VAR_F32 : 0)) |
                      (use_slabs ? (slab_bf16 ? STSWIN_VAR_TN_SLABS_BF16 : STSWIN_VAR_TN_SLABS_F32) : 0) | ((use_slabs && perm) ? 0x4000 : 0) |
                      (splits << 16);
  if (dtype == 0) {
    if (w8) hipLaunchKernelGGL((gemm_tn_kernel<bf16, 8>), grid, dim3(512), 65536, (hipStream_t)stream, p);
    else hipLaunchKernelGGL((gemm_tn_kernel<bf16, 4>), grid, dim3(256), 65536, (hipStream_t)stream, p);
  } else {
    if (w8) hipLaunchKernelGGL((gemm_tn_kernel<float, 8>), grid, dim3(512), 65536, (hipStream_t)stream, p);
    else hipLaunchKernelGGL((gemm_tn_kernel<float, 4>), grid, dim3(256), 65536, (hipStream_t)stream, p);
  }
  if (use_slabs && !no_combine) {
    const long n4 = slab_bf16 ? ((long)Ni * Nj + 7) / 8 : ((long)Ni * Nj + 3) / 4;
    hipLaunchKernelGGL(tn_reduce_kernel, dim3((unsigned)((n4 + 255) / 256)), dim3(256), 0, (hipStream_t)stream, workspace, C, ldc,
                       Ni, Nj, splits, overwrite, slab_bf16, perm);
  }
  STSWIN_CHECK_LAUNCH();
  return 0;
}

extern "C" int stswin_tn_combine(const float* workspace, float* C, long ldc, int Ni, int Nj, int splits, int overwrite, int slab_bf16,
                                 void* stream) {
  if (!workspace || !C || Ni <= 0 || Nj <= 0 || splits < 2) return -1007;
  const long n4 = slab_bf16 ? ((long)Ni * Nj + 7) / 8 : ((long)Ni * Nj + 3) / 4;
  hipLaunchKernelGGL(tn_reduce_kernel, dim3((unsigned)((n4 + 255) / 256)), dim3(256), 0, (hipStream_t)stream, workspace, C, ldc, Ni, Nj,
// ... 5 lines not shown
```

stswincl_amd/headops.py:

```python
from __future__ import annotations

import os
import weakref
from typing import List, Optional, Sequence, Tuple

import torch
import torch.nn.functional as F

from . import hip
from .ops import compute_dtype, _f32

KGRAN = 64


_INDEX_MAPS = {}
_TORCH_PADVEC = os.environ.get("STSWIN_TORCH_PADVEC") == "1"
_BN_KEEP_Y = os.environ.get("STSWIN_BN_KEEP_Y") == "1"


class Layout:

    def __init__(self, segs: Sequence[Tuple[int, int, int]], width: int):
        self.segs, self.width = list(segs), width
        self.logical = sum(s[1] for s in self.segs)

    @staticmethod
    def dense(c: int) -> "Layout":
        w = (c + KGRAN - 1) // KGRAN * KGRAN
        return Layout([(0, c, 0)], w)

    @staticmethod
    def concat(parts: Sequence["Layout"]) -> "Layout":
        segs, lo, po = [], 0, 0
        for p in parts:
            segs += [(lo + a, n, po + b) for a, n, b in p.segs]
            lo += p.logical
            po += p.width
        return Layout(segs, po)

    @property
    def is_identity(self) -> bool:
        return len(self.segs) == 1 and self.segs[0] == (0, self.width, 0)

    def pad_vec(self, v: torch.Tensor, fill: float = 0.0) -> torch.Tensor:
        if self.is_identity:
            return v.detach().float().contiguous()
        if v.is_cuda and v.dim() == 1 and not _TORCH_PADVEC:
            return hip.vec_gather(v.detach().float().contiguous(), self.index_map(v.device), fill)
        out = torch.full((self.width,), fill, dtype=torch.float32, device=v.device)
        for a, n, b in self.segs:
            out[b:b + n] = v.detach()[a:a + n]
        return out

    def pad_vecs(self, vs, fills):
        vs = [v.detach() for v in vs]
        if (self.is_identity or _TORCH_PADVEC or not all(v.is_cuda and v.dim() == 1 and v.dtype == torch.float32 and v.is_contiguous() for v in vs)
                or len(vs) > 4):
            return [self.pad_vec(v, f) for v, f in zip(vs, fills)]
        return hip.vec_gather_multi(vs, self.index_map(vs[0].device), fills)

    def unpad_vecs(self, vs, into=None):
        ok = (not self.is_identity and not _TORCH_PADVEC and len(vs) <= 4
              and all(v.is_cuda and v.dim() == 1 and v.dtype == torch.float32 and v.is_contiguous() for v in vs)
              and (into is None or all(t.dtype == torch.float32 and t.is_contiguous() and t.numel() == self.logical for t in into)))
        if not ok:
            outs = [self.unpad_vec(v) for v in vs]
            if into is not None:
                for t, o in zip(into, outs):
                    t.copy_(o)
                return list(into)
            return outs
        return hip.vec_gather_multi(vs, self.position_map(vs[0].device), None, outs=into)

    def unpad_vec(self, v: torch.Tensor) -> torch.Tensor:
        if self.is_identity:
            return v
        if v.is_cuda and v.dim() == 1 and v.dtype == torch.float32 and not _TORCH_PADVEC:
            return hip.vec_gather(v.contiguous(), self.position_map(v.device), 0.0)
        return torch.cat([v[..., b:b + n] for a, n, b in self.segs], dim=-1)

    def position_map(self, device) -> torch.Tensor:
        key = ("pos", self.key(), str(device))
        m = _INDEX_MAPS.get(key)
        if m is None:
            m = torch.empty(self.logical, dtype=torch.int32)
            for a, n, b in self.segs:
                m[a:a + n] = torch.arange(b, b + n, dtype=torch.int32)
            m = m.to(device)
            _INDEX_MAPS[key] = m
        return m

    def key(self):
        return (tuple(self.segs), self.width)

    def index_map(self, device) -> torch.Tensor:
        key = (self.key(), str(device))
        m = _INDEX_MAPS.get(key)
        if m is None:
            m = torch.full((self.width,), -1, dtype=torch.int32)
            for a, n, b in self.segs:
                m[b:b + n] = torch.arange(a, a + n, dtype=torch.int32)
            m = m.to(device)
            _INDEX_MAPS[key] = m
        return m


_CW: dict = {}


def _conv_mats(w: torch.Tensor, dt, lin: Layout, lout: Layout, dgrad: bool) -> torch.Tensor:
    key = (id(w), dt, lin.key(), lout.key())
    stamp = (w._version, w.data_ptr(), tuple(w.shape))
    hit = _CW.get(key)
    if hit is None or hit[0]() is not w or hit[1] != stamp:
        omap, imap = lout.index_map(w.device), lin.index_map(w.device)
        fwd, dg = hip.conv_pack(w, dt, omap, imap)
        if len(_CW) > 2048:
            for kk in [kk for kk, v in _CW.items() if v[0]() is None]:
                del _CW[kk]
        hit = (weakref.ref(w), stamp, fwd, dg, omap, imap)
        _CW[key] = hit
    return hit[3] if dgrad else hit[2]


_MAPS: dict = {}


def _conv_maps(frames, Hin, Win, k, stride, pad, dil, device):
    Hout = (Hin + 2 * pad - dil * (k - 1) - 1) // stride + 1
    Wout = (Win + 2 * pad - dil * (k - 1) - 1) // stride + 1
    if k == 1 and stride == 1 and pad == 0:
        return Hout, Wout, None, None
    key = (frames, Hin, Win, k, stride, pad, dil, str(device))
    hit = _MAPS.get(key)
    if hit is None:
        hit = (hip.conv_rowmap(frames, Hin, Win, Hout, Wout, k, stride, pad, dil, False, device),
               hip.conv_rowmap(frames, Hin, Win, Hout, Wout, k, stride, pad, dil, True, device))
        _MAPS[key] = hit
    return Hout, Wout, hit[0], hit[1]


_RESID_GRAD_LINK = os.environ.get("STSWIN_NO_RESID_GRAD_LINK") != "1"
_HALO_CONV = os.environ.get("STSWIN_NO_HALO_CONV") != "1"
_HALO_WGRAD = os.environ.get("STSWIN_NO_HALO_WGRAD") != "1"
_STEM_WGRAD = os.environ.get("STSWIN_NO_STEM_WGRAD") != "1"
_STEM_CONV = os.environ.get("STSWIN_NO_STEM_CONV") != "1"


class ConvTokFn(torch.autograd.Function):

    @staticmethod
    def forward(ctx, x, weight, bias, geom, lin, lout, want_stats=False, link=None):
        ctx.link = link
        frames, Hin, Win, k, stride, pad, dil = geom
        dt = compute_dtype(x)
        X = x.detach().to(dt)
        Hout, Wout, fmap, imap = _conv_maps(frames, Hin, Win, k, stride, pad, dil, x.device)
        Mi, Mo = frames * Hin * Win, frames * Hout * Wout
        assert X.shape == (Mi, lin.width) and X.stride(1) == 1 and weight.shape[-1] == k
        y = torch.empty(Mo, lout.width, dtype=dt, device=x.device)
        tab = hip.stats_table(Mo, lout.width, x.device) if want_stats else None
        ctx.tapskip = hip.GF_TAPSKIP if (k == 3 and stride == 1 and 2 * dil >= Hin + 3 and Mo <= 32768) else 0
        ctx.halo = (_HALO_CONV and bias is None and lin.is_identity and lout.is_identity and X.is_contiguous()
                    and hip.conv3x3_c64_ok(frames, Hin, Win, lin.width, lout.width, k, stride, pad, dil, dt))
        if ctx.halo:
            hip.conv3x3_c64(X, _conv_mats(weight, dt, lin, lout, False), y, frames, Hin, Win, 1, stats_out=tab)
        else:
            hip.gemm_nt(X, _conv_mats(weight, dt, lin, lout, False), y, M=Mo, a_rows=fmap, S=k * k,
                        bias=lout.pad_vec(bias) if bias is not None else None, stats_out=tab, flags=ctx.tapskip)
        ctx.geom = (frames, Hin, Win)
        ctx.cfg = (k, lin, lout, dt, x.dtype, bias is not None, Mi, Mo)
        ctx.save_for_backward(X, weight, fmap, imap)
        if want_stats:
            ctx.mark_non_differentiable(tab)
            ctx.set_materialize_grads(False)
            return y, tab
        return y

    @staticmethod
    @hip.tn_deferred_backward
    def backward(ctx, dy, _dtab=None):
        if dy is None:
            return (None,) * 8
        X, weight, fmap, imap = ctx.saved_tensors
        k, lin, lout, dt, in_dtype, has_bias, Mi, Mo = ctx.cfg
        co, ci = weight.shape[:2]
        S = k * k
        g = dy.detach().to(dt).contiguous()
        from .ops import wgrad_buffer
        dense = lin.is_identity and lout.is_identity
        direct = dense and S == 1
        dwp = (wgrad_buffer(weight, (lout.width, S * lin.width), X.device) if dense
               else torch.empty(lout.width, S * lin.width, dtype=torch.float32, device=X.device))
        if ctx.halo and _HALO_WGRAD and hip.conv3x3_c64_wgrad_ok(*ctx.geom):
            hip.conv3x3_c64_wgrad(g, X, dwp, *ctx.geom, tapminor=True)
            tapminor = True
        else:
            hip.gemm_tn(g, X, dwp, Mk=Mo, bt_rows=fmap, bseg=lin.width if fmap is not None else 0, overwrite=True,
                        tapminor=dense and S > 1)
            tapminor = dense and S > 1 and hip.last_tn_tapminor()
        dx = None
        if ctx.needs_input_grad[0]:
            dx = torch.empty(Mi, lin.width, dtype=dt, device=X.device)
            pend = ctx.link.take(dt, dx.shape) if ctx.link is not None else None
            if ctx.halo:
                hip.conv3x3_c64(g, _conv_mats(weight, dt, lin, lout, True), dx, *ctx.geom, -1, resid=pend)
            else:
                hip.gemm_nt(g, _conv_mats(weight, dt, lin, lout, True), dx, M=Mi, a_rows=imap, S=S, resid=pend,
                            flags=(hip.GF_RESID if pend is not None else 0) | ctx.tapskip)
            dx = dx.to(in_dtype)
            if ctx.link is not None and not ctx.link.last():
                ctx.link.put(dx)
                dx = None
        hip.tn_join()
        if direct or tapminor:
            dw = dwp
        elif dense:
            dw = dwp.clone().view(co, S, ci).permute(0, 2, 1)
        else:
            dw = torch.zeros(co, ci, S, dtype=torch.float32, device=X.device)
            d3 = dwp.view(lout.width, S, lin.width)
            for oa, on, ob in lout.segs:
                for ia, in_, ib in lin.segs:
                    dw[oa:oa + on, ia:ia + in_, :] = d3[ob:ob + on, :, ib:ib + in_].permute(0, 2, 1)
        db = None
        if has_bias:
            dbp = hip.zeros(lout.width, device=X.device)
            hip.colsum(g, dbp)
            db = lout.unpad_vec(dbp)
        if dw is dwp:
            dw = dw.view(co, ci, k, k)
        else:
            dw = dw.reshape(co, ci, k, k)
            from .dp import grad_dest
            slot = getattr(weight, "_stswin_grad_dest", None)
            if dense and slot is not None and dwp.data_ptr() == slot[1].data_ptr():
                dw = dwp.view(co, ci, k, k).copy_(dw)
            elif not dense and slot is not None:
                dest = grad_dest(weight)
                if dest is not None:
                    dw = dest.copy_(dw)
        return dx, dw, db, None, None, None, None, None


class GradLink:

    def __init__(self, convs: int):
        self.left, self.g = convs, None

    def put(self, g):
        self.g = g if self.g is None else self.g + g

    def take(self, dt, shape):
        g, self.g = self.g, None
        self.left -= 1
        if g is None:
            return None
        assert tuple(g.shape) == tuple(shape)
        return g.to(dt).contiguous()

    def last(self):
        return self.left <= 0


_FUSED_BN_STATS = os.environ.get("STSWIN_NO_FUSED_BN_STATS") != "1"


def conv_tokens(x_tok, conv: torch.nn.Conv2d, frames, Hin, Win, lin=None, lout=None, stats=None, link=None):
    k, stride, pad, dil = conv.kernel_size[0], conv.stride[0], conv.padding[0], conv.dilation[0]
    lin = lin or Layout.dense(conv.in_channels)
    lout = lout or Layout.dense(conv.out_channels)
    Hout = (Hin + 2 * pad - dil * (k - 1) - 1) // stride + 1
    Wout = (Win + 2 * pad - dil * (k - 1) - 1) // stride + 1
    Mo = frames * Hout * Wout
    want = (stats and _FUSED_BN_STATS and compute_dtype(x_tok) == torch.bfloat16 and Mo >= 8192 and Mo % 256 == 0
            and lout.width % 4 == 0)
    geom = (frames, Hin, Win, k, stride, pad, dil)
    if want:
        y, tab = ConvTokFn.apply(x_tok, conv.weight, conv.bias, geom, lin, lout, True, link)
    else:
        y, tab = ConvTokFn.apply(x_tok, conv.weight, conv.bias, geom, lin, lout, False, link), None
    return (y, Hout, Wout) if stats is None else (y, Hout, Wout, tab)


_STEM_MAPS: dict = {}


def _stem_rowmap(frames, Ho, Wo, Hs, Ws, device):
    key = (frames, Ho, Wo, Hs, Ws, str(device))
    hit = _STEM_MAPS.get(key)
    if hit is None:
        f, oy, ox = torch.meshgrid(torch.arange(frames, device=device), torch.arange(Ho, device=device),
                                   torch.arange(Wo, device=device), indexing="ij")
        hit = torch.stack([((f * Hs + oy + s) * Ws + ox).reshape(-1) for s in range(4)]).to(torch.int32).contiguous()
        if len(_STEM_MAPS) > 16:
            _STEM_MAPS.clear()
        _STEM_MAPS[key] = hit
    return hit


def _stem_pack(weight, dt):
    w8 = F.pad(weight.detach().float(), (1, 0, 1, 0))
    w8 = w8.view(-1, 3, 4, 2, 4, 2).permute(0, 2, 4, 3, 5, 1).reshape(-1, 4, 4, 12)
    return F.pad(w8, (0, 4)).reshape(-1, 256).to(dt)


def _stem_unpack(dw):
    co = dw.shape[0]
    return dw.view(co, 4, 4, 16)[..., :12].reshape(co, 4, 4, 2, 2, 3).permute(0, 5, 1, 3, 2, 4).reshape(co, 3, 8, 8)[:, :, 1:, 1:]


class StemConvFn(torch.autograd.Function):

    @staticmethod
    def forward(ctx, img, weight, dt, want_stats=False):
        F_, _, Hh, Ww = img.shape
        Ho, Wo = (Hh + 6 - 7) // 2 + 1, (Ww + 6 - 7) // 2 + 1
        im = img.detach().float().contiguous()
        A, Hs, Ws = hip.stem_s2d(im, dt)
        rmap = _stem_rowmap(F_, Ho, Wo, Hs, Ws, img.device)
        y = torch.empty(F_ * Ho * Wo, 64, dtype=dt, device=img.device)
        tab = hip.stats_table(y.shape[0], 64, img.device) if want_stats else None
        if _STEM_CONV and hip.stem_wgrad_ok(Hh, Ww, dt):
            hip.stem_conv(A, _stem_pack(weight, dt), y, F_, Hh, Ww, stats_out=tab)
        else:
            hip.gemm_nt(A, _stem_pack(weight, dt), y, M=y.shape[0], a_rows=rmap, S=4, stats_out=tab)
        ctx.dt, ctx.geom = dt, (F_, Hh, Ww)
        ctx.save_for_backward(A, rmap, weight)
        if want_stats:
            ctx.mark_non_differentiable(tab)
            ctx.set_materialize_grads(False)
            return y, tab
        return y

    @staticmethod
    @hip.tn_deferred_backward
    def backward(ctx, dy, _dtab=None):
        if dy is None:
            return None, None, None, None
        A, rmap, weight = ctx.saved_tensors
        dw = torch.empty(64, 256, dtype=torch.float32, device=A.device)
        g = dy.detach().to(ctx.dt).contiguous()
        if _STEM_WGRAD and hip.stem_wgrad_ok(ctx.geom[1], ctx.geom[2], ctx.dt):
            hip.stem_wgrad(g, A, dw, *ctx.geom)
        else:
            hip.gemm_tn(g, A, dw, Mk=rmap.shape[1], bt_rows=rmap, bseg=64, overwrite=True)
            hip.tn_join()
        dwv = _stem_unpack(dw)
        from .dp import grad_dest
        dest = grad_dest(weight) if getattr(weight, "_stswin_grad_dest", None) is not None else None
        return None, (dest.copy_(dwv) if dest is not None else dwv.contiguous()), None, None


def stem_conv_tokens(img, weight, dt, stats=False):
    F_, _, Hh, Ww = img.shape
    M = F_ * ((Hh - 1) // 2 + 1) * ((Ww - 1) // 2 + 1)
    if stats and _FUSED_BN_STATS and dt == torch.bfloat16 and M >= 8192 and M % 256 == 0:
        return StemConvFn.apply(img, weight, dt, True)
    return StemConvFn.apply(img, weight, dt), None


class MaxPoolTokFn(torch.autograd.Function):

    @staticmethod
    def forward(ctx, x, geom):
        frames, Hh, Ww = geom
        dt = compute_dtype(x)
        X = x.detach().to(dt).contiguous()
        Ho, Wo = (Hh + 2 - 3) // 2 + 1, (Ww + 2 - 3) // 2 + 1
        y = torch.empty(frames * Ho * Wo, X.shape[1], dtype=dt, device=x.device)
        arg = torch.empty(frames * Ho * Wo, X.shape[1], dtype=torch.uint8, device=x.device)
        hip.maxpool3x3s2(X, y, arg, frames, Hh, Ww, Ho, Wo)
        ctx.cfg = (frames, Hh, Ww, Ho, Wo, dt, x.dtype)
        ctx.save_for_backward(arg)
        return y

    @staticmethod
    def backward(ctx, dy):
        (arg,) = ctx.saved_tensors
        frames, Hh, Ww, Ho, Wo, dt, in_dtype = ctx.cfg
        g = dy.detach().to(dt).contiguous()
        dx = torch.empty(frames * Hh * Ww, g.shape[1], dtype=dt, device=g.device)
        hip.maxpool3x3s2(g, dx, arg, frames, Hh, Ww, Ho, Wo, backward=True)
        return dx.to(in_dtype), None


def combine_bn_stats(mean_r: torch.Tensor, m2_r: torch.Tensor, n_r: torch.Tensor):
    n = n_r.sum()
    w = (n_r / n).view(-1, 1, 1)
    mean = (mean_r * w).sum(0)
    m2 = (m2_r + n_r.view(-1, 1, 1) * (mean_r - mean) ** 2).sum(0)
    return mean, m2 / n, n


def refuse_replica(module) -> None:
# ... 127 lines not shown
        return y

    @staticmethod
    def backward(ctx, dy):
        X, y, mean, rstd, gp, bp = ctx.saved_tensors
        training, relu, groups, lay, dt, in_dtype, has_res, world, rows_total = ctx.cfg
        g = rowmajor(dy, dt)
        dx = torch.empty_like(X)
        dres = torch.empty_like(X) if has_res else None
        if training and world > 1:
            import torch.distributed as dist
            s1, s2 = hip.bn_bwd(g, X, y if relu else None, mean, rstd, gp, dx, dres, groups, relu, training, phase=1, beta=bp,
                                unit=ctx.unit)
            loc1, loc2 = s1.clone(), s2.clone()
            both = torch.stack([s1, s2])
            dist.all_reduce(both)
            COLLECTIVES["syncbn_all_reduce"] = COLLECTIVES.get("syncbn_all_reduce", 0) + 1
            both = both * ctx.sum_scale
            hip.bn_bwd(g, X, y if relu else None, mean, rstd, gp, dx, dres, groups, relu, training, phase=2,
                       sums=(both[0].contiguous(), both[1].contiguous()), rows_total=0, beta=bp, unit=ctx.unit)
            s1, s2 = loc1, loc2
        else:
            gs = torch.empty(2, X.shape[1], dtype=torch.float32, device=X.device) if groups > 1 else None
            s1, s2 = hip.bn_bwd(g, X, y if relu else None, mean, rstd, gp, dx, dres, groups, relu, training, beta=bp, unit=ctx.unit,
                                group_sums=gs)
            if gs is not None:
                s1, s2, groups = gs[0:1], gs[1:2], 1
        if groups > 1:
            if s1._base is not None and s2._base is s1._base and s2.storage_offset() == s1.storage_offset() + s1.numel():
                both = torch.as_strided(s1, (2, groups, s1.shape[-1]), (groups * s1.shape[-1], s1.shape[-1], 1)).sum(1)
                s1, s2 = both[0:1], both[1:2]
            else:
                s1, s2 = s1.sum(0, keepdim=True), s2.sum(0, keepdim=True)
        if lay.is_identity:
            dgamma, dbeta = s2[0], s1[0]
        else:
            dgamma, dbeta = lay.unpad_vecs([s2[0].contiguous(), s1[0].contiguous()])
        dres = dres.to(in_dtype) if has_res else None
        if dres is not None and ctx.link is not None:
            ctx.link.put(dres)
            dres = None
        return (dx.to(in_dtype), dgamma, dbeta, None, None, None, None, dres, None, None, None, None, None, None, None, None, None)


class BNTokGroupFn(torch.autograd.Function):

    @staticmethod
    def forward(ctx, n, *args):
        import torch.distributed as dist
        cfgs, tens = args[:n], args[n:]
        world = dist.get_world_size()
        st, packs = [], []
        for i in range(n):
            relu, groups, lay, eps, momentum, unit, out = cfgs[i]
            x, gamma, beta, rmean, rvar = tens[5 * i:5 * i + 5]
            dt = compute_dtype(x)
            X = x.detach().to(dt)
            M, Cp = X.shape
            assert Cp == lay.width
            n_loc = M // groups
            s, ss = hip.colstats(X, groups=groups, unit=unit)
            pivot = (X.view(-1, unit, Cp)[:groups, 0, :] if unit > 0 else X.view(groups, n_loc, Cp)[:, 0, :]).float()
            mean_l = pivot + s / n_loc
            m2_l = ss - s * s / n_loc
            packs.append(torch.stack([mean_l, m2_l, torch.full_like(mean_l, float(n_loc))]).reshape(3, groups * Cp))
            st.append((X, dt, M, Cp, n_loc, x.dtype))
        pack = torch.cat(packs, dim=1).contiguous()
        allp = torch.empty(world * 3, pack.shape[1], dtype=pack.dtype, device=pack.device)
        dist.all_gather_into_tensor(allp, pack)
        COLLECTIVES["syncbn_all_gather"] = COLLECTIVES.get("syncbn_all_gather", 0) + 1
        allp = allp.view(world, 3, -1)
        outs, saved, meta, off = [], [], [], 0
        for i in range(n):
            relu, groups, lay, eps, momentum, unit, out = cfgs[i]
            x, gamma, beta, rmean, rvar = tens[5 * i:5 * i + 5]
            X, dt, M, Cp, n_loc, in_dtype = st[i]
            blk = allp[:, :, off:off + groups * Cp].reshape(world, 3, groups, Cp)
            off += groups * Cp
            n_r = blk[:, 2, 0, 0]
            mean, var, n_tot = combine_bn_stats(blk[:, 0], blk[:, 1], n_r)
            rstd = torch.rsqrt(var + eps)
            unbias = n_tot / (n_tot - 1).clamp(min=1)
            rm, rv = lay.pad_vec(rmean), lay.pad_vec(rvar, 1.0)
            for g in range(groups):
                rm = (1 - momentum) * rm + momentum * mean[g]
                rv = (1 - momentum) * rv + momentum * var[g] * unbias
            rmean.copy_(lay.unpad_vec(rm))
            rvar.copy_(lay.unpad_vec(rv))
            mean, rstd = mean.contiguous(), rstd.contiguous()
            gp, bp = lay.pad_vec(gamma), lay.pad_vec(beta)
            if out is not None:
                assert out.shape == (M, Cp) and out.dtype == dt and out.stride(1) == 1
                y = out.view_as(out)
            else:
                y = torch.empty(M, Cp, dtype=dt, device=x.device)
            hip.bn_apply(X, mean, rstd, gp, bp, y, resid=None, groups=groups, relu=relu, unit=unit)
            outs.append(y)
            keep_y = relu and _BN_KEEP_Y
            saved += [X, y if keep_y else None, mean, rstd, gp, bp if relu else None]
            meta.append((relu, groups, lay, dt, in_dtype, unit, float(n_loc) / n_tot))
        ctx.meta, ctx.n = meta, n
        ctx.save_for_backward(*saved)
        return tuple(outs)

    @staticmethod
    def backward(ctx, *dys):
        import torch.distributed as dist
        n, sv = ctx.n, ctx.saved_tensors
        work, sums = [], []
        for i in range(n):
            relu, groups, lay, dt, in_dtype, unit, sum_scale = ctx.meta[i]
            X, y, mean, rstd, gp, bp = sv[6 * i:6 * i + 6]
            g = rowmajor(dys[i], dt)
            dx = torch.empty_like(X)
            s1, s2 = hip.bn_bwd(g, X, y if relu else None, mean, rstd, gp, dx, None, groups, relu, True, phase=1, beta=bp, unit=unit)
            work.append((g, dx, s1.clone(), s2.clone()))
            sums.append(torch.stack([s1, s2]).reshape(2, -1))
        both = torch.cat(sums, dim=1).contiguous()
        dist.all_reduce(both)
        COLLECTIVES["syncbn_all_reduce"] = COLLECTIVES.get("syncbn_all_reduce", 0) + 1
        grads, off = [], 0
        for i in range(n):
            relu, groups, lay, dt, in_dtype, unit, sum_scale = ctx.meta[i]
            X, y, mean, rstd, gp, bp = sv[6 * i:6 * i + 6]
            g, dx, loc1, loc2 = work[i]
            Cp = X.shape[1]
            blk = (both[:, off:off + groups * Cp] * sum_scale).reshape(2, groups, Cp)
            off += groups * Cp
            hip.bn_bwd(g, X, y if relu else None, mean, rstd, gp, dx, None, groups, relu, True, phase=2,
                       sums=(blk[0].contiguous(), blk[1].contiguous()), rows_total=0, beta=bp, unit=unit)
            s1, s2 = (loc1.sum(0, keepdim=True), loc2.sum(0, keepdim=True)) if groups > 1 else (loc1, loc2)
            grads += [dx.to(in_dtype), lay.unpad_vec(s2[0]), lay.unpad_vec(s1[0]), None, None]
        return (None,) + (None,) * n + tuple(grads)


class syncbn_group:

    def __init__(self):
        self.items, self.out = [], []

    def __enter__(self):
        return self

    def conv_bn_relu(self, x_tok, conv, bn, geom, lin=None, lout=None, relu=True, groups=1, out=None):
        training = bn.training or bn.running_mean is None
        if not (training and _sync_world(bn) > 1):
            self.out.append(conv_bn_relu(x_tok, conv, bn, geom, lin=lin, lout=lout, relu=relu, groups=groups, out=out))
            return len(self.out) - 1
        frames, Hh, Ww = geom
        lout = lout or Layout.dense(conv.out_channels)
        y = conv_tokens(x_tok, conv, frames, Hh, Ww, lin, lout, stats=False)[0]
        return self.bn(y, bn, relu=relu, groups=groups, lay=lout, out=out)

    def bn(self, y, bn, relu=True, groups=1, il_frames=0, lay=None, stats=None, out=None):
        training = bn.training or bn.running_mean is None
        if not (training and _sync_world(bn) > 1):
            self.out.append(batchnorm_tokens(y, bn, relu=relu, groups=groups, lay=lay, il_frames=il_frames, stats=stats, out=out))
            return len(self.out) - 1
        self.out.append(None)
        self.items.append((len(self.out) - 1, y, bn, relu, groups, il_frames, lay or Layout.dense(bn.num_features), out))
        return len(self.out) - 1

    def __exit__(self, et, ev, tb):
        if et is not None or not self.items:
            return False
        cfgs, tens = [], []
        for _, y, bn, relu, groups, il_frames, lay, out in self.items:
            if _BN_VIEWS is not None:
                views, clips = _BN_VIEWS
                if il_frames:
                    groups = groups * views
                else:
                    assert groups == 1, "view batching: contiguous multi-group BatchNorm inside an encoder is not supported"
                    groups, il_frames = views, clips
            if bn.num_batches_tracked is not None:
                if _NBT_PENDING is not None:
                    _NBT_PENDING.append((bn.num_batches_tracked, groups))
                else:
                    bn.num_batches_tracked += groups
            unit = (y.shape[0] // il_frames) if (il_frames and groups > 1) else 0
            cfgs.append((relu, groups, lay, bn.eps, bn.momentum if bn.momentum is not None else 0.1, unit, out))
            tens += [y, bn.weight, bn.bias, bn.running_mean, bn.running_var]
        ys = BNTokGroupFn.apply(len(self.items), *cfgs, *tens)
        for (slot, *_), y in zip(self.items, ys):
            self.out[slot] = y
        return False

    def results(self):
        return list(self.out)


_NBT_PENDING = None
_BN_VIEWS = None


class bn_views:

    def __init__(self, views: int, clips: int):
        assert clips % views == 0
        self.v = (views, clips) if views > 1 else None

    def __enter__(self):
        global _BN_VIEWS
        self.prev, _BN_VIEWS = _BN_VIEWS, self.v
        return self

    def __exit__(self, *exc):
        global _BN_VIEWS
        _BN_VIEWS = self.prev
        return False



class deferred_bn_counters:

    def __enter__(self):
        global _NBT_PENDING
        self.prev, _NBT_PENDING = _NBT_PENDING, []
        return self

    def __exit__(self, *exc):
        global _NBT_PENDING
        pend, _NBT_PENDING = _NBT_PENDING, self.prev
        if pend:
            if self.prev is not None:
                self.prev.extend(pend)
            else:
                per_t = {}
                for t, inc in pend:
                    ent = per_t.setdefault(id(t), [t, 0])
                    ent[1] += inc
                by_inc = {}
                for t, inc in per_t.values():
                    by_inc.setdefault(inc, []).append(t)
                for inc, ts in by_inc.items():
                    torch._foreach_add_(ts, inc)
        return False


def batchnorm_tokens(x, bn: torch.nn.BatchNorm2d, relu=True, resid=None, groups=1, lay: Optional[Layout] = None,
                     il_frames: int = 0, stats=None, resid_link=None, out=None):
    lay = lay or Layout.dense(bn.num_features)
    training = bn.training or bn.running_mean is None
    if _BN_VIEWS is not None and training:
        views, clips = _BN_VIEWS
        if il_frames:
            groups = groups * views
        else:
            assert groups == 1, "view batching: contiguous multi-group BatchNorm inside an encoder is not supported"
            groups, il_frames = views, clips
    if training and bn.num_batches_tracked is not None:
        if _NBT_PENDING is not None:
            _NBT_PENDING.append((bn.num_batches_tracked, groups))
        else:
            bn.num_batches_tracked += groups
    world = _sync_world(bn) if training else 1
    return BNTokFn.apply(x, bn.weight, bn.bias, bn.running_mean, bn.running_var, training, relu, resid, groups, lay,
                         bn.eps, bn.momentum if bn.momentum is not None else 0.1, world,
                         (x.shape[0] // il_frames) if (il_frames and groups > 1) else 0,
                         stats if (training and world == 1) else None, resid_link if resid is not None else None, out)


class BNReluPoolFn(torch.autograd.Function):

    @staticmethod
    def forward(ctx, x, gamma, beta, running_mean, running_var, training, groups, eps, momentum, unit, stats, geom):
        frames, Hh, Ww = geom
        dt = compute_dtype(x)
        X = x.detach().to(dt)
        M, C = X.shape
        if training:
            raw = stats is not None and groups <= 32 and ((unit % 256 == 0) if unit > 0 else ((M // groups) % 256 == 0))
            if raw:
                mean, rstd = hip.bn_table_finalize(stats, M, running_mean, running_var, groups, eps, momentum, unit=unit)
            else:
                s, ss = hip.colstats(X, groups=groups, unit=unit)
                mean, rstd = hip.bn_finalize(X, s, ss, running_mean, running_var, groups, eps, momentum, unit=unit)
        else:
            mean = running_mean.float().view(1, C).expand(groups, C).contiguous()
            rstd = torch.rsqrt(running_var.float() + eps).view(1, C).expand(groups, C).contiguous()
        gp, bp = _f32(gamma), _f32(beta)
        y, arg = hip.bn_relu_pool(X, mean, rstd, gp, bp, frames, Hh, Ww, groups=groups, unit=unit)
        ctx.cfg = (training, groups, unit, geom, x.dtype)
        ctx.save_for_backward(X, arg, mean, rstd, gp, bp)
        return y

    @staticmethod
    def backward(ctx, dy):
        X, arg, mean, rstd, gp, bp = ctx.saved_tensors
        training, groups, unit, (frames, Hh, Ww), in_dtype = ctx.cfg
        g = rowmajor(dy, X.dtype).contiguous()
        Hp, Wp = (Hh - 1) // 2 + 1, (Ww - 1) // 2 + 1
        dz = torch.empty_like(X)
        hip.maxpool3x3s2(g, dz, arg, frames, Hh, Ww, Hp, Wp, backward=True)
        dx = torch.empty_like(X)
        gs = torch.empty(2, X.shape[1], dtype=torch.float32, device=X.device) if groups > 1 else None
        s1, s2 = hip.bn_bwd(dz, X, None, mean, rstd, gp, dx, None, groups, True, training, beta=bp, unit=unit, group_sums=gs)
        if gs is not None:
            s1, s2 = gs[0:1], gs[1:2]
        return (dx.to(in_dtype), s2[0], s1[0]) + (None,) * 9


_FUSED_STEM_TAIL = os.environ.get("STSWIN_NO_FUSED_STEM_TAIL") != "1"


def batchnorm_relu_maxpool_tokens(x, bn: torch.nn.BatchNorm2d, geom, groups=1, il_frames: int = 0, stats=None):
# ... 158 lines not shown
```

stswincl_amd/hip.py:

```python
from __future__ import annotations

import ctypes
import functools
import os
import re
from typing import Optional

import torch

_ROOT = os.path.dirname(os.path.dirname(os.path.abspath(__file__)))
LIB_PATH = os.environ.get("STSWIN_HIP_LIB") or os.path.join(_ROOT, "stswincl_amd", "lib", "libstswin_hip.so")
HEADER_PATH = os.path.join(_ROOT, "include", "stswin_hip.h")
_lib: Optional[ctypes.CDLL] = None

_c_int, _c_float, _c_void_p = ctypes.c_int, ctypes.c_float, ctypes.c_void_p


class StswinHipError(RuntimeError):
    pass


_C_TYPES = {"int": ctypes.c_int, "long": ctypes.c_long, "float": ctypes.c_float, "double": ctypes.c_double}


def _c_value(name: str, expr: str) -> int:
    tokens = re.findall(r"0[xX][0-9a-fA-F]+|\d+|<<|[-+*()]|\S", re.sub(r"(?<=[0-9a-fA-F])[uU]\b", "", expr))
    if not tokens or not all(re.fullmatch(r"0[xX][0-9a-fA-F]+|\d+|<<|[-+*()]", t) for t in tokens):
        raise StswinHipError(f"{HEADER_PATH}: cannot evaluate `#define STSWIN_{name} {expr.strip()}`")
    try:
        v = int(eval(" ".join(tokens), {"__builtins__": {}}))
    except (SyntaxError, TypeError) as e:
        raise StswinHipError(f"{HEADER_PATH}: cannot evaluate `#define STSWIN_{name} {expr.strip()}`") from e
    return v - (1 << 32) if v >= 1 << 31 else v


@functools.lru_cache(maxsize=None)
def _header():
    with open(HEADER_PATH) as f:
        text = re.sub(r"/\*.*?\*/", "", f.read(), flags=re.S)
    protos = {}
    for ret, name, params in re.findall(r"\b(int|long)\s+(stswin_\w+)\s*\(([^()]*)\)\s*;", text):
        argtypes = []
        for p in ([] if params.strip() == "void" else params.split(",")):
            words = [w for w in p.split() if w != "const"]
            if "*" in p:
                argtypes.append(ctypes.c_void_p)
            elif len(words) == 2 and words[0] in _C_TYPES:
                argtypes.append(_C_TYPES[words[0]])
            else:
                raise StswinHipError(f"{HEADER_PATH}: {name}: cannot bind parameter `{p.strip()}`")
        protos[name] = (_C_TYPES[ret], argtypes)
    unparsed = set(re.findall(r"\b(stswin_\w+)\s*\(", text)) - set(protos)
    if unparsed:
        raise StswinHipError(f"{HEADER_PATH}: cannot bind the declaration of {sorted(unparsed)}")
    consts = {name: _c_value(name, expr) for name, expr in re.findall(r"^[ \t]*#[ \t]*define[ \t]+STSWIN_(\w+)[ \t]+(\S.*)$", text, flags=re.M)}
    return protos, consts


globals().update(_header()[1])


def declared_symbols():
    return sorted(_header()[0])


def load() -> ctypes.CDLL:
    global _lib
    if _lib is not None:
        return _lib
    if not os.path.exists(LIB_PATH):
        raise StswinHipError(f"{LIB_PATH} not found: run `python __graft_entry__.py` (build()) first; "
                             "stswincl_amd has no CPU or eager fallback")
    lib = ctypes.CDLL(LIB_PATH)
    protos = _header()[0]
    missing = [s for s in sorted(protos) if not hasattr(lib, s)]
    if missing and not os.environ.get("STSWIN_HIP_LIB"):
        raise StswinHipError(f"libstswin_hip.so lacks declared symbols: {missing}")
    for s, (restype, argtypes) in protos.items():
        if s not in missing:
            fn = getattr(lib, s)
            fn.restype, fn.argtypes = restype, argtypes
    _lib = lib
    return lib


def tuning_build() -> bool:
    return bool(load().stswin_tuning_build())


def tn_fused_holds() -> int:
    return int(load().stswin_tn_fused_hold(0))


class TnFusedHold:

    def __init__(self):
        import weakref
        lib = load()
        lib.stswin_tn_fused_hold(1)
        self._fin = weakref.finalize(self, lib.stswin_tn_fused_hold, -1)

    def release(self):
        self._fin()


def _check(rc: int, what: str) -> None:
    if rc != 0:
        raise StswinHipError(f"{what} failed with code {rc}")


def _dt(t: torch.Tensor) -> int:
    if t.dtype == torch.bfloat16:
        return 0
    if t.dtype == torch.float32:
        return 1
    raise StswinHipError(f"unsupported dtype {t.dtype}")


def _p(t: Optional[torch.Tensor]) -> Optional[int]:
    if t is None:
        return None
    if not t.is_cuda:
        raise StswinHipError("stswincl_amd ops need tensors on the GPU (no CPU path exists)")
    return t.data_ptr()


_RAW_STREAM = getattr(torch._C, "_cuda_getCurrentRawStream", None)


def _stream() -> int:
    if _RAW_STREAM is not None:
        return _RAW_STREAM(torch.cuda.current_device())
    return torch.cuda.current_stream().cuda_stream


def _ld(t: torch.Tensor) -> int:
    assert t.dim() == 2 and t.stride(1) == 1, "expected a row-major 2-D view"
    return t.stride(0)


def _device(d) -> torch.device:
    d = torch.device(d)
    if d.type == "cuda" and d.index is None:
        d = torch.device("cuda", torch.cuda.current_device())
    return d


_ARENA_FLOATS = 1 << 22
_ARENA_MAX_REQUEST = 0 if os.environ.get("STSWIN_NO_ARENA") == "1" else 1 << 18
_ARENAS = {}


def arena_reset(device=None) -> None:
    if device is None:
        _ARENAS.clear()
    else:
        _ARENAS.pop(_device(device), None)


def zeros(*shape, device) -> torch.Tensor:
    if len(shape) == 1 and isinstance(shape[0], (tuple, list, torch.Size)):
        shape = tuple(shape[0])
    n = 1
    for d in shape:
        n *= int(d)
    if n > _ARENA_MAX_REQUEST or n == 0:
        return torch.zeros(shape, dtype=torch.float32, device=device)
    device = _device(device)
    st = _ARENAS.get(device)
    need = (n + 15) // 16 * 16
    if st is None or st[1] + need > _ARENA_FLOATS:
        st = [torch.zeros(_ARENA_FLOATS, dtype=torch.float32, device=device), 0]
        _ARENAS[device] = st
    out = st[0][st[1]:st[1] + n].view(shape)
    st[1] += need
    return out


_SCRATCH = {}
_SCRATCH_RETIRED = []
_DEFER = [False, 0]
_CAPTURED = [False]


def note_capture() -> None:
    _CAPTURED[0] = True


def scratch(device, floats: int) -> torch.Tensor:
    device = _device(device)
    floats = (int(floats) + 63) // 64 * 64
    t = _SCRATCH.get(device)
    off = _DEFER[1] if _DEFER[0] else 0
    if not _CAPTURED[0] and device.type == "cuda" and torch.cuda.is_current_stream_capturing():
        _CAPTURED[0] = True
    if t is None or t.numel() < off + floats:
        if _DEFER[0] and off > 0:
            _check(load().stswin_fold_flush(_stream()), "fold_flush")
            _DEFER[1] = off = 0
        if t is None or t.numel() < floats:
            if t is not None and torch.cuda.is_current_stream_capturing():
                raise StswinHipError("scratch buffer would have to grow during a hipGraph capture: run the step once before capturing")
            if t is not None and _CAPTURED[0]:
                _SCRATCH_RETIRED.append(t)
            t = torch.empty(max(floats, 2 * (t.numel() if t is not None else 0), 1 << 23), dtype=torch.float32, device=device)
            _SCRATCH[device] = t
    if _DEFER[0]:
        _DEFER[1] = off + floats
# ... 200 lines not shown


def stem_conv(A, wmat, y, frames, H, W, stats_out=None):
    Ho, Wo = (H - 1) // 2 + 1, (W - 1) // 2 + 1
    M = frames * Ho * Wo
    assert A.dtype == torch.bfloat16 and A.stride() == (16, 1) and A.shape[0] == frames * (Ho + 3) * (Wo + 3)
    assert wmat.dtype == torch.bfloat16 and wmat.shape == (64, 256) and wmat.is_contiguous()
    assert y.dtype == torch.bfloat16 and y.shape == (M, 64) and y.is_contiguous()
    assert stats_out is None or (stats_out.dtype == torch.float32 and stats_out.numel() == 2 * 2 * ((M + 255) // 256) * 64)
    with _Span("stem_conv_bf16", 2.0 * M * 64 * 147):
        rc = load().stswin_stem_conv(_p(A), _p(wmat), _p(y), _p(stats_out), frames, H, W, _stream())
    _check(rc, "stem_conv")
    return y


def stem_wgrad_ok(H, W, dtype) -> bool:
    return dtype == torch.bfloat16 and ((W - 1) // 2 + 1) % 128 == 0


def stem_wgrad(dy, A, dw, frames, H, W, accumulate=False):
    Ho, Wo = (H - 1) // 2 + 1, (W - 1) // 2 + 1
    assert dy.dtype == torch.bfloat16 and dy.shape == (frames * Ho * Wo, 64) and dy.is_contiguous()
    assert A.dtype == torch.bfloat16 and A.stride() == (16, 1) and A.shape[0] == frames * (Ho + 3) * (Wo + 3)
    assert dw.dtype == torch.float32 and dw.numel() == 64 * 256 and dw.is_contiguous()
    ws = scratch(dy.device, load().stswin_stem_wgrad_scratch(frames, Ho, Wo))
    with _Span("stem_wgrad_bf16", 2.0 * frames * Ho * Wo * 64 * 147):
        rc = load().stswin_stem_wgrad(_p(dy), _p(A), _p(dw), 1 if accumulate else 0, _p(ws), ws.numel(), frames, H, W, _stream())
    _check(rc, "stem_wgrad")
    return dw


def maxpool3x3s2(src, dst, arg, frames, H, W, Ho, Wo, backward=False):
    C = src.shape[1]
    _pair("maxpool3x3s2", src, dst)
    if (Ho, Wo) != ((H - 1) // 2 + 1, (W - 1) // 2 + 1):
        raise StswinHipError(f"maxpool3x3s2: ({Ho}, {Wo}) is not the 3x3 stride-2 pad-1 pool of ({H}, {W})")
    _rows("maxpool3x3s2", src, frames * (Ho * Wo if backward else H * W), "src")
    _rows("maxpool3x3s2", dst, frames * (H * W if backward else Ho * Wo), "dst")
    if arg.dtype != torch.uint8 or arg.device != src.device or tuple(arg.shape) != (frames * Ho * Wo, C) or not arg.is_contiguous():
        raise StswinHipError(f"maxpool3x3s2: arg must be a contiguous uint8 [{frames * Ho * Wo}][{C}] on {src.device}, got "
                             f"{arg.dtype} {tuple(arg.shape)} on {arg.device}")
    _check(load().stswin_maxpool3x3s2(_dt(src), _p(src), _ld(src), _p(dst), _ld(dst), _p(arg), frames, H,
                                      W, Ho, Wo, C, 1 if backward else 0, _stream()), "maxpool3x3s2")
    return dst


def conv3x3_c64_ok(frames, H, W, cin, cout, k, stride, pad, dil, dt) -> bool:
    return (dt == torch.bfloat16 and cin == 64 and cout == 64 and k == 3 and stride == 1 and pad == 1 and dil == 1
            and W in (16, 32, 64, 128) and (H * W) % 256 == 0 and frames > 0)


def conv3x3_c64(x, wmat, y, frames, H, W, sign=1, resid=None, stats_out=None):
    M = frames * H * W
    for t in (x, y, resid):
        assert t is None or (t.dtype == torch.bfloat16 and t.shape == (M, 64) and t.is_contiguous())
    assert wmat.dtype == torch.bfloat16 and wmat.shape == (64, 576) and wmat.is_contiguous()
    assert stats_out is None or (stats_out.dtype == torch.float32 and stats_out.numel() == 2 * 2 * ((M + 255) // 256) * 64)
    with _Span("conv3x3_c64_bf16", 2.0 * M * 64 * 576):
        rc = load().stswin_conv3x3_c64(_p(x), _p(wmat), _p(y), _p(resid), _p(stats_out), frames, H, W, sign, _stream())
    _check(rc, "conv3x3_c64")
    return y


def conv3x3_c64_wgrad_ok(frames, H, W) -> bool:
    return W in (32, 64, 128) and (H * W) % 128 == 0 and frames > 0


def conv3x3_c64_wgrad(dy, x, dw, frames, H, W, tapminor=True, accumulate=False):
    M = frames * H * W
    for t in (dy, x):
        assert t.dtype == torch.bfloat16 and t.shape == (M, 64) and t.is_contiguous()
    assert dw.dtype == torch.float32 and dw.numel() == 64 * 576 and dw.is_contiguous()
    need = load().stswin_conv3x3_c64_wgrad_scratch(frames, H, W)
    ws = scratch(x.device, need)
    with _Span("conv3x3_c64_wgrad_bf16", 2.0 * M * 64 * 576):
        rc = load().stswin_conv3x3_c64_wgrad(_p(dy), _p(x), _p(dw), 1 if tapminor else 0, 1 if accumulate else 0, _p(ws), ws.numel(),
                                             frames, H, W, _stream())
    _check(rc, "conv3x3_c64_wgrad")
    return dw


def stats_table(M: int, N: int, device) -> torch.Tensor:
    return torch.empty(2, 2 * ((M + 255) // 256), N, dtype=torch.float32, device=device)


def cs_group_reduce(table: torch.Tensor, M: int, groups: int, unit: int = 0):
    N = table.shape[2]
    both = torch.empty(2, groups, N, dtype=torch.float32, device=table.device)
    _check(load().stswin_cs_group_reduce(_p(table), M, N, groups, unit, _p(both[0]), _p(both[1]), _stream()), "cs_group_reduce")
    return both[0], both[1]


def bn_table_finalize(table: torch.Tensor, M: int, running_mean, running_var, groups=1, eps=1e-5, momentum=0.1, unit=0):
    N = table.shape[2]
    mean = torch.empty(groups, N, dtype=torch.float32, device=table.device)
    rstd = torch.empty_like(mean)
    _check(load().stswin_bn_table_finalize(_p(table), M, N, groups, unit, _p(mean), _p(rstd), _p(running_mean), _p(running_var),
                                           eps, momentum, _stream()), "bn_table_finalize")
    return mean, rstd


def gemm_nt(A: torch.Tensor, Bw: torch.Tensor, out: torch.Tensor, *, M: int, a_rows=None, c_rows=None, bias=None,
            resid=None, r_rows=None, out2=None, S: int = 1, scale: float = 1.0, scale_cols: int = 0, flags: int = 0,
            colsum_out=None, stats_out=None):
    N, Ktot = Bw.shape
    assert Ktot % S == 0
    Kseg = Ktot // S
    assert A.dtype == Bw.dtype and A.shape[1] >= Kseg
    if not (flags & GF_OUT_F32):
        assert out.dtype == A.dtype
    else:
        assert out.dtype == torch.float32
    cs_table = None
    if stats_out is not None:
        assert colsum_out is None and stats_out.shape == (2, 2 * ((M + 255) // 256), N) and stats_out.is_contiguous()
        flags |= GF_CS_PARTIAL | GF_CS_SQ
        colsum_out = stats_out
    elif colsum_out is not None and M >= _CS_PARTIAL_MIN_M and N % 4 == 0 and not (flags & _GF_DEBUG_STAMPS):
        cs_table = scratch(A.device, 2 * ((M + 255) // 256) * N)
        flags |= GF_CS_PARTIAL
    elif colsum_out is not None and N % 4 and not _WARNED.get("cs_atomic"):
        _WARNED["cs_atomic"] = True
        import warnings
        warnings.warn(f"stswincl_amd.hip.gemm_nt: column sums of an output with N = {N} (not a multiple of 4) are added with fp32 "
                      f"atomics (order-dependent last bits); pad N to a multiple of 4 for bitwise-reproducible sums")
    name = "gemm_nt_bf16" if A.dtype == torch.bfloat16 else "gemm_nt_f32"
    if _SHAPE_NAMES:
        name += f" M={M} N={N} K={Kseg} S={S} a={int(a_rows is not None)} c={int(c_rows is not None)} fl={flags}"
    if (_NT_SPLITK and A.dtype == torch.bfloat16 and out.dtype == torch.bfloat16 and c_rows is None and resid is None and out2 is None
            and colsum_out is None and scale == 1.0 and scale_cols == 0 and not (flags & ~GF_RELU)):
        need = load().stswin_gemm_nt_splitk_scratch(M, N, Kseg, S)
        if need > 0 and _PLAN_ROWS[0] != 1 and load().stswin_gemm_nt_splitk_scratch(M * _PLAN_ROWS[0], N, Kseg, S) <= 0:
            need = 0
        if need > 0:
            ws = scratch(A.device, need)
            with _Span(name, 2.0 * M * N * Ktot):
                rc = load().stswin_gemm_nt_splitk(_p(A), _ld(A), _p(a_rows), _p(Bw), _ld(Bw), _p(out), _ld(out),
                                                  _p(bias), M, N, Kseg, S, 1 if (flags & GF_RELU) else 0, _p(ws), ws.numel(), _stream())
            if rc != -1008:
                _check(rc, "gemm_nt_splitk")
                _log_variant("nt", (M, N, Kseg, S), 0)
                return out
    with _Span(name, 2.0 * M * N * Ktot):
        rc = load().stswin_gemm_nt(
            _dt(A), _p(A), _ld(A), _p(a_rows), _p(Bw), _ld(Bw), _p(out), _ld(out),
            _p(c_rows), _p(out2), _ld(out2) if out2 is not None else 0, _p(bias), _p(resid),
            _ld(resid) if resid is not None else 0, _p(r_rows), M, N, Kseg, S, scale, scale_cols,
            flags, _p(cs_table if cs_table is not None else colsum_out), _stream())
    _check(rc, "gemm_nt")
    _log_variant("nt", (M, N, Kseg, S), 0)
    if cs_table is not None:
        _check(load().stswin_cs_reduce(_p(cs_table), M, N, _p(colsum_out), _stream()), "cs_reduce")
    return out


def gemm_nt_qkv_fp8(A: torch.Tensor, Bw: torch.Tensor, *, M: int, a_rows=None, bias=None, scale: float = 1.0, scale_cols: int = 0,
                    rows_per_problem: int, head_dim: int):
    N, K = Bw.shape
    assert A.dtype == torch.bfloat16 and Bw.dtype == torch.bfloat16 and A.shape[1] >= K
    out8 = torch.empty(M, N, dtype=torch.uint8, device=A.device)
    scales = torch.empty(M // rows_per_problem, N // head_dim, dtype=torch.float32, device=A.device)
    with _Span("gemm_nt_bf16" + (f" M={M} N={N} K={K} S=1 a={int(a_rows is not None)} c=0 fl=fp8out" if _SHAPE_NAMES else ""), 2.0 * M * N * K):
        rc = load().stswin_gemm_nt_qkv_fp8(_p(A), _ld(A), _p(a_rows), _p(Bw), _ld(Bw), _p(out8), N, _p(scales),
                                           N // head_dim, _p(bias), M, N, K, scale, scale_cols, rows_per_problem, head_dim,
                                           _stream())
    _check(rc, "gemm_nt_qkv_fp8")
    return out8, scales


VARIANT_LOG = None


def _log_variant(family: str, shape, fam_id: int) -> None:
    if VARIANT_LOG is not None:
        VARIANT_LOG.append((family, tuple(int(v) for v in shape), int(load().stswin_last_variant(fam_id))))


_WARNED = {}
_GF_DEBUG_STAMPS = 1 << 19
_ATTN_DEBUG_STAMPS = 1 << 30
_NT_SPLITK = os.environ.get("STSWIN_NO_NT_SPLITK") != "1"
_PLAN_ROWS = [1]


class splitk_as_rows:

    def __init__(self, factor: int):
        self.factor = int(factor)

    def __enter__(self):
        self.prev = _PLAN_ROWS[0]
        _PLAN_ROWS[0] = self.factor
        return self

    def __exit__(self, *exc):
        _PLAN_ROWS[0] = self.prev


_CS_PARTIAL_MIN_M = int(os.environ.get("STSWIN_CS_PARTIAL_MIN_M", "1"))
_TN_WS = {}


def _tn_workspace(device, floats=48 * 1024 * 1024):
    ws = _TN_WS.get(device)
    if ws is None:
        ws = torch.empty(floats, dtype=torch.float32, device=device)
        _TN_WS[device] = ws
    return ws


_TN_SIDE = {}
_TN_DEFER = 0
_TN_PENDING = None
_TN_DEFER_ON = os.environ.get("STSWIN_TN_DEFERRED_COMBINE") == "1"


class tn_deferred:

    def __enter__(self):
        global _TN_DEFER
        _TN_DEFER += 1
        return self

    def __exit__(self, *exc):
        global _TN_DEFER
        _TN_DEFER -= 1
        if _TN_DEFER == 0:
            tn_join()
        return False


def tn_deferred_backward(fn):
    import functools

    @functools.wraps(fn)
    def wrapper(ctx, *grads):
        with tn_deferred():
            return fn(ctx, *grads)
    return wrapper


def tn_join():
    global _TN_PENDING
    if _TN_PENDING is not None:
        torch.cuda.current_stream().wait_event(_TN_PENDING)
        _TN_PENDING = None


def gemm_tn(At: torch.Tensor, Bt: torch.Tensor, out_f32: torch.Tensor, *, Mk: int, at_rows=None, bt_rows=None,
            splits: int = 0, bseg: int = 0, atomics: bool = False, overwrite: bool = False, debug_ts: bool = False, tapminor: bool = False):
    if overwrite:
        splits |= TN_OVERWRITE
    if tapminor and bseg > 0:
        splits |= TN_OUT_TAPMINOR
    Ni, Nj = out_f32.shape
    assert out_f32.dtype == torch.float32 and At.dtype == Bt.dtype
    ws = None if atomics or torch.cuda.is_current_stream_capturing() and At.device not in _TN_WS else _tn_workspace(At.device)
    name = "gemm_tn_bf16" if At.dtype == torch.bfloat16 else "gemm_tn_f32"
    if _SHAPE_NAMES:
        name += f" Mk={Mk} Ni={Ni} Nj={Nj} bseg={bseg} a={int(at_rows is not None)} b={int(bt_rows is not None)}"
    defer = _TN_DEFER > 0 and _TN_DEFER_ON and ws is not None and not debug_ts
    tn_join()
    with _Span(name, 2.0 * Mk * Ni * Nj):
        rc = load().stswin_gemm_tn(_dt(At), _p(At), _ld(At), _p(at_rows), _p(Bt), _ld(Bt),
                                   _p(bt_rows), _p(out_f32), (-1 if debug_ts is True else -int(debug_ts)) if debug_ts else _ld(out_f32), Mk, Ni, Nj,
                                   (splits | TN_NO_COMBINE) if defer else splits, bseg, _p(ws),
                                   ws.numel() if ws is not None else 0, _stream())
    _check(rc, "gemm_tn")
    _log_variant("tn", (Mk, Ni, Nj, bseg), 1)
    if defer:
        v = load().stswin_last_variant(1)
        if v & (VAR_TN_SLABS_F32 | VAR_TN_SLABS_BF16):
            global _TN_PENDING
            cur = torch.cuda.current_stream()
            side = _TN_SIDE.get(At.device)
            if side is None:
                side = _TN_SIDE[At.device] = torch.cuda.Stream(device=At.device)
            ev = torch.cuda.Event()
            ev.record(cur)
            side.wait_event(ev)
            _check(load().stswin_tn_combine(_p(ws), _p(out_f32), _ld(out_f32), Ni, Nj, v >> 16, 1 if (splits & TN_OVERWRITE) else 0,
                                            1 if v & VAR_TN_SLABS_BF16 else 0, side.cuda_stream), "tn_combine")
            _TN_PENDING = torch.cuda.Event()
            _TN_PENDING.record(side)
    return out_f32


class _TnProblem(ctypes.Structure):
    _fields_ = [("At", ctypes.c_void_p), ("lda", ctypes.c_long), ("at_rows", ctypes.c_void_p),
                ("Bt", ctypes.c_void_p), ("ldb", ctypes.c_long), ("bt_rows", ctypes.c_void_p),
                ("C", ctypes.c_void_p), ("ldc", ctypes.c_long),
                ("Mk", ctypes.c_int), ("Ni", ctypes.c_int), ("Nj", ctypes.c_int), ("bseg", ctypes.c_int),
                ("overwrite", ctypes.c_int), ("tapminor", ctypes.c_int)]


LAST_TN_GROUP_SPLITS: list = []


def gemm_tn_group(problems) -> bool:
    n = len(problems)
    if n == 0:
        return True
    first = problems[0]["At"]
    if n > 4 or first.dtype != torch.bfloat16 or torch.cuda.is_current_stream_capturing() and first.device not in _TN_WS:
        return False
    arr = (_TnProblem * n)()
# ... 1547 lines not shown
```

stswincl_amd/net/Ours/ASPP.py:

```python
from __future__ import annotations

import torch
import torch.nn as nn

from ... import headops as H


class ASPP(nn.Module):
    def __init__(self, num_classes):
        super().__init__()
        nc = 1024
        self.conv_1x1_1 = nn.Conv2d(nc, nc // 2, kernel_size=1)
        self.bn_conv_1x1_1 = nn.BatchNorm2d(nc // 2)
        self.conv_3x3_1 = nn.Conv2d(nc, nc // 2, kernel_size=3, stride=1, padding=6, dilation=6)
        self.bn_conv_3x3_1 = nn.BatchNorm2d(nc // 2)
        self.conv_3x3_2 = nn.Conv2d(nc, nc // 2, kernel_size=3, stride=1, padding=12, dilation=12)
        self.bn_conv_3x3_2 = nn.BatchNorm2d(nc // 2)
        self.conv_3x3_3 = nn.Conv2d(nc, nc // 2, kernel_size=3, stride=1, padding=18, dilation=18)
        self.bn_conv_3x3_3 = nn.BatchNorm2d(nc // 2)
        self.avg_pool = nn.AdaptiveAvgPool2d(1)
        self.conv_1x1_2 = nn.Conv2d(nc, nc // 2, kernel_size=1)
        self.bn_conv_1x1_2 = nn.BatchNorm2d(nc // 2)
        self.conv_1x1_3 = nn.Conv2d(nc // 2 * 5, nc // 2, kernel_size=1)
        self.bn_conv_1x1_3 = nn.BatchNorm2d(nc // 2)
        self.conv_1x1_4 = nn.Conv2d(nc // 2, num_classes, kernel_size=1)
        self.num_classes = num_classes

    def forward_tokens(self, x, geom):
        f, h, w = geom
        if self.training and f == 1:
            raise ValueError(f"Expected more than 1 value per channel when training, got input size torch.Size([1, 512, 1, 1])")
        nb = self.conv_1x1_1.out_channels
        buf, (v1, v2, v3, v4, v5) = H.concat_buffer(x.shape[0], [nb] * 5, H.compute_dtype(x), x.device)
        with H.syncbn_group() as g:
            g.conv_bn_relu(x, self.conv_1x1_1, self.bn_conv_1x1_1, geom, out=v1)
            g.conv_bn_relu(x, self.conv_3x3_1, self.bn_conv_3x3_1, geom, out=v2)
            g.conv_bn_relu(x, self.conv_3x3_2, self.bn_conv_3x3_2, geom, out=v3)
            g.conv_bn_relu(x, self.conv_3x3_3, self.bn_conv_3x3_3, geom, out=v4)
            g.conv_bn_relu(H.AvgPoolTokFn.apply(x, f), self.conv_1x1_2, self.bn_conv_1x1_2, (f, 1, 1))
        o1, o2, o3, o4, img = g.results()
        img = H.BroadcastTokFn.apply(img, h * w, v5)
        cat = H.ConcatColsFn.apply(buf, (nb,) * 5, o1, o2, o3, o4, img)
        out = H.conv_bn_relu(cat, self.conv_1x1_3, self.bn_conv_1x1_3, geom)
        return H.conv1x1_tokens(out, self.conv_1x1_4, f, h, w)

    def forward(self, feature_map):
        f, c, h, w = feature_map.shape
        out = self.forward_tokens(H.to_tokens(feature_map), (f, h, w))
        return H.from_tokens(out, f, h, w)[:, :self.num_classes]


ASPPv5 = ASPP
```

Measured before the change: 609.1 frames/s.

## Group ASPP dilated 3x3 convs into one grouped split-K NT GEMM launch

Adds a grouped NT GEMM kernel that runs up to three independent GEMM problems in one launch, split-K planned together to fill the CU budget, with one shared combine kernel for the split slabs. The three dilated ASPP 3x3 convolutions now share input tokens and go through this path in forward and dgrad, and their wgrad goes through the grouped TN path via a new static mode-3 kernel. The TN grouping acceptance thresholds are also relaxed for conv sets. The aim is to cut under-occupied launches and tail effects on the small ASPP feature map, at the cost of extra fp32 slab traffic and more complex dispatch.

```diff
diff --git a/include/stswin_hip.h b/include/stswin_hip.h
--- a/include/stswin_hip.h
+++ b/include/stswin_hip.h
@@ -73,6 +73,19 @@
 long stswin_gemm_nt_splitk_scratch(int M, int N, int Kseg, int S);
 int stswin_gemm_nt_splitk(const void* A, long lda, const int* a_rows, const void* B, long ldb, void* C, long ldc, const float* bias, int M, int N,
                           int Kseg, int S, int relu, float* workspace, long workspace_floats, void* stream);
+enum { STSWIN_NT_GROUP_DECLINED = -1051, STSWIN_NT_GROUP_MAX = 3, STSWIN_VAR_NT_GROUP = 15 };
+typedef struct stswin_nt_problem {
+  const void* A; long lda; const int* a_rows;
+  const void* B; long ldb;
+  void* C; long ldc;
+  const float* bias;
+  int M, N, Kseg, S;
+  int flags;
+  int splits;
+} stswin_nt_problem;
+long stswin_gemm_nt_group_scratch(int count, const stswin_nt_problem* problems);
+int stswin_gemm_nt_group(int count, const stswin_nt_problem* problems, float* workspace, long workspace_floats, int* splits_out,
+                         void* stream);
 int stswin_tn_fused_hold(int delta);
 int stswin_set_cu_budget(int cus);
 int stswin_gemm_tn(int dtype, const void* At, long lda, const int* at_rows, const void* Bt, long ldb, const int* bt_rows,
diff --git a/stswincl_amd/csrc/gemm.hip b/stswincl_amd/csrc/gemm.hip
--- a/stswincl_amd/csrc/gemm.hip
+++ b/stswincl_amd/csrc/gemm.hip
@@ -392,8 +392,8 @@
 
 DEVI int swz64(int row) { return (4 - ((row >> 2) & 3)) & 3; }
 
-template <int BM, int BN, int WM, int WN, int NST, int MINW, int PIPE, bool SWAP = false, bool PERSIST = false>
-__global__ __launch_bounds__(WM * WN * 64, MINW) void gemm_nt_ring_kernel(GemmNT p) {
+template <int BM, int BN, int WM, int WN, int NST, int MINW, int PIPE, bool SWAP = false, bool PERSIST = false, bool GROUPED = false>
+DEVI void gemm_nt_ring_body(GemmNT p, const int tix0, const unsigned ysplit) {
   using T = bf16;
   constexpr int BK = 32, ROWB = 64;
   constexpr int A_BYTES = BM * ROWB, B_BYTES = BN * ROWB, STAGE = A_BYTES + B_BYTES;
@@ -410,13 +410,13 @@
   extern __shared__ __attribute__((aligned(16))) char smem[];
   const int tiles_n = (p.N + BN - 1) / BN, tiles_m = (p.M + BM - 1) / BM;
   const int ntot_ = tiles_m * tiles_n;
-  int tix_ = blockIdx.x;
+  int tix_ = tix0;
   do {
   int tid_ = threadIdx.x;
   if constexpr (PERSIST) asm volatile("" : "+v"(tid_));
   const int tid = tid_, l = tid & 63, w = __builtin_amdgcn_readfirstlane(tid >> 6);
   const int wr = w / WN, wc = w % WN;
-  const int t = xcd_remap(tix_, ntot_);
+  const int t = GROUPED ? tix_ : xcd_remap(tix_, ntot_);
   int tm = t / tiles_n, tn = t % tiles_n;
   if (tiles_n >= 24) {
     constexpr int GM = 8;
@@ -447,9 +447,9 @@
     }
   };
   const int kps = p.Kseg / BK;
-  const int qbase = p.qsplit > 0 ? (int)blockIdx.y * p.qsplit : 0;
+  const int qbase = p.qsplit > 0 ? (int)ysplit * p.qsplit : 0;
   const int nt = p.qsplit > 0 ? min(p.qsplit, p.S * kps - qbase) : p.S * kps;
-  if (p.qsplit > 0) p.C = (char*)p.C + (long)blockIdx.y * p.M * p.ldc * ((p.flags & GF_OUT_F32) ? 4 : 2);
+  if (p.qsplit > 0) p.C = (char*)p.C + (long)ysplit * p.M * p.ldc * ((p.flags & GF_OUT_F32) ? 4 : 2);
   int seg = -1;
   auto issue = [&](int q) {
     const int Q = q + qbase;
@@ -1052,6 +1052,27 @@
     if (tix_ < ntot_) __syncthreads();
   }
   } while (PERSIST && tix_ < ntot_);
+}
+
+template <int BM, int BN, int WM, int WN, int NST, int MINW, int PIPE, bool SWAP = false, bool PERSIST = false>
+__global__ __launch_bounds__(WM * WN * 64, MINW) void gemm_nt_ring_kernel(GemmNT p) {
+  gemm_nt_ring_body<BM, BN, WM, WN, NST, MINW, PIPE, SWAP, PERSIST>(p, (int)blockIdx.x, blockIdx.y);
+}
+
+#define NT_GROUP_MAX STSWIN_NT_GROUP_MAX
+struct GemmNTGroup { GemmNT q[NT_GROUP_MAX]; int first[NT_GROUP_MAX + 1]; int tiles[NT_GROUP_MAX]; };
+__global__ __launch_bounds__(512, 2) void gemm_nt_ring_group_kernel(GemmNTGroup g) {
+  const int seq = xcd_remap((int)blockIdx.x, (int)gridDim.x);
+  if (seq >= g.first[2]) {
+    const int local = seq - g.first[2], sp = local / g.tiles[2];
+    gemm_nt_ring_body<256, 256, 2, 4, 4, 2, 1, false, false, true>(g.q[2], local - sp * g.tiles[2], sp);
+  } else if (seq >= g.first[1]) {
+    const int local = seq - g.first[1], sp = local / g.tiles[1];
+    gemm_nt_ring_body<256, 256, 2, 4, 4, 2, 1, false, false, true>(g.q[1], local - sp * g.tiles[1], sp);
+  } else {
+    const int sp = seq / g.tiles[0];
+    gemm_nt_ring_body<256, 256, 2, 4, 4, 2, 1, false, false, true>(g.q[0], seq - sp * g.tiles[0], sp);
+  }
 }
 
 
@@ -1738,9 +1759,7 @@
   *(f32x4*)(C + (long)i * ldc + j) = v;
 }
 
-__global__ __launch_bounds__(256) void nt_splitk_combine_kernel(const float* ws, int splits, long slab, int M, int N, bf16* C, long ldc, const float* bias,
-                                                                int relu) {
-  const long idx = (long)blockIdx.x * 256 + threadIdx.x;
+DEVI void nt_splitk_combine_piece(const long idx, const float* ws, int splits, long slab, int M, int N, bf16* C, long ldc, const float* bias, int relu) {
   const int pn = N / 8;
   if (idx >= (long)M * pn) return;
   const int m = (int)(idx / pn), n = (int)(idx % pn) * 8;
@@ -1758,6 +1777,25 @@
     o[e] = (bf16)v;
   }
   *(bf16x8*)(C + (long)m * ldc + n) = o;
+}
+__global__ __launch_bounds__(256) void nt_splitk_combine_kernel(const float* ws, int splits, long slab, int M, int N, bf16* C, long ldc, const float* bias,
+                                                                int relu) {
+  nt_splitk_combine_piece((long)blockIdx.x * 256 + threadIdx.x, ws, splits, slab, M, N, C, ldc, bias, relu);
+}
+struct NtGroupCombine {
+  const float* ws[NT_GROUP_MAX]; bf16* C[NT_GROUP_MAX]; const float* bias[NT_GROUP_MAX]; long ldc[NT_GROUP_MAX];
+  int splits[NT_GROUP_MAX], M[NT_GROUP_MAX], N[NT_GROUP_MAX], relu[NT_GROUP_MAX]; int first[NT_GROUP_MAX + 1];
+};
+__global__ __launch_bounds__(256) void nt_group_combine_kernel(NtGroupCombine t) {
+  const int b = (int)blockIdx.x;
+#pragma unroll
+  for (int i = NT_GROUP_MAX - 1; i >= 0; --i) {
+    if (b >= t.first[i] && b < t.first[i + 1]) {
+      nt_splitk_combine_piece((long)(b - t.first[i]) * 256 + threadIdx.x, t.ws[i], t.splits[i], (long)t.M[i] * t.N[i], t.M[i], t.N[i], t.C[i], t.ldc[i],
+                              t.bias[i], t.relu[i]);
+      return;
+    }
+  }
 }
 
 __global__ __launch_bounds__(256) void nt_splitk_combine16_kernel(const bf16* ws, int splits, long slab, int M, int N, bf16* C, long ldc, const float* bias,
@@ -1826,6 +1864,99 @@
   else hipLaunchKernelGGL(nt_splitk_combine_kernel, dim3((unsigned)((n + 255) / 256)), dim3(256), 0, (hipStream_t)stream, workspace, splits, (long)M * N, M, N,
                      (bf16*)C, ldc, bias, relu);
   STSWIN_CHECK_LAUNCH();
+  return 0;
+}
+
+int stswin_cu_budget();
+static int nt_group_plan(int count, const stswin_nt_problem* pr, int* rs, int* per, int* tiles, long* need) {
+  if (count <= 0 || count > NT_GROUP_MAX || !pr) return -1052;
+  { const char* eg = getenv("STSWIN_NT_GROUP"); if (eg && atoi(eg) == 0) return STSWIN_NT_GROUP_DECLINED; }
+  int nst[NT_GROUP_MAX], forced = 0;
+  long total_tiles = 0;
+  for (int i = 0; i < count; ++i) {
+    const stswin_nt_problem& q = pr[i];
+    if (q.M <= 0 || q.N <= 0 || q.Kseg <= 0 || q.S <= 0 || !q.A || !q.B || !q.C || q.splits < 0 || q.lda % 8 || q.ldb % 8) return -1001;
+    if (q.flags & ~(GF_RELU | GF_TAPSKIP)) return -1001;
+    if (q.M < 256 || q.N < 256 || q.N % 8 || q.Kseg % 32 || q.ldc % 8 || ((uintptr_t)q.C & 15)) return STSWIN_NT_GROUP_DECLINED;
+    if ((q.a_rows ? false : (long)q.M * q.lda * 2 > 0xFFFF0000L) || (long)q.N * q.ldb * 2 > 0xFFFF0000L) return STSWIN_NT_GROUP_DECLINED;
+    tiles[i] = ((q.M + 255) / 256) * ((q.N + 255) / 256);
+    nst[i] = q.S * (q.Kseg / 32);
+    total_tiles += tiles[i];
+    forced += q.splits > 0;
+  }
+  if (forced != 0 && forced != count) return -1052;
+  const int cus = stswin_cu_budget();
+  if (forced) {
+    for (int i = 0; i < count; ++i) rs[i] = pr[i].splits < nst[i] ? pr[i].splits : nst[i];
+  } else {
+    if (total_tiles > cus) return STSWIN_NT_GROUP_DECLINED;
+    long total = 0;
+    for (int L = 16; L <= (1 << 20); ++L) {
+      total = 0;
+      for (int i = 0; i < count; ++i) { rs[i] = (nst[i] + L - 1) / L; total += (long)tiles[i] * rs[i]; }
+      if (total <= cus) break;
+    }
+    if (total > cus || total * 4 < (long)cus * 3) return STSWIN_NT_GROUP_DECLINED;
+  }
+  *need = 0;
+  for (int i = 0; i < count; ++i) {
+    if (rs[i] > 31) return STSWIN_NT_GROUP_DECLINED;
+    per[i] = (nst[i] + rs[i] - 1) / rs[i];
+    rs[i] = (nst[i] + per[i] - 1) / per[i];
+    if (rs[i] > 1) *need += (long)rs[i] * pr[i].M * pr[i].N;
+  }
+  return 0;
+}
+extern "C" long stswin_gemm_nt_group_scratch(int count, const stswin_nt_problem* pr) {
+  int rs[NT_GROUP_MAX], per[NT_GROUP_MAX], tiles[NT_GROUP_MAX];
+  long need = 0;
+  return nt_group_plan(count, pr, rs, per, tiles, &need) == 0 ? need : 0;
+}
+extern "C" int stswin_gemm_nt_group(int count, const stswin_nt_problem* pr, float* workspace, long workspace_floats, int* splits_out,
+                                    void* stream) {
+  if (count == 0) return 0;
+  int rs[NT_GROUP_MAX], per[NT_GROUP_MAX], tiles[NT_GROUP_MAX];
+  long need = 0;
+  const int rc = nt_group_plan(count, pr, rs, per, tiles, &need);
+  if (rc != 0) return rc;
+  if (need > 0 && (!workspace || workspace_floats < need || ((uintptr_t)workspace & 15))) return STSWIN_NT_GROUP_DECLINED;
+  static const int attr = (int)hipFuncSetAttribute((const void*)gemm_nt_ring_group_kernel, hipFuncAttributeMaxDynamicSharedMemorySize, 131072);
+  if (attr != 0) return -attr;
+  GemmNTGroup g;
+  NtGroupCombine c;
+  g.first[0] = 0;
+  c.first[0] = 0;
+  long wo = 0;
+  int word = STSWIN_VAR_NT_GROUP;
+  for (int i = 0; i < NT_GROUP_MAX; ++i) {
+    if (i >= count) {
+      g.q[i] = g.q[0]; g.tiles[i] = 1; g.first[i + 1] = g.first[i];
+      c.ws[i] = nullptr; c.C[i] = nullptr; c.bias[i] = nullptr; c.ldc[i] = 0; c.splits[i] = 0; c.M[i] = 0; c.N[i] = 8; c.relu[i] = 0;
+      c.first[i + 1] = c.first[i];
+      continue;
+    }
+    const stswin_nt_problem& q = pr[i];
+    const bool split = rs[i] > 1;
+    const int relu = (q.flags & GF_RELU) ? 1 : 0;
+    float* slabs = workspace + wo;
+    g.q[i] = GemmNT{q.A, q.lda, q.a_rows, q.B, q.ldb, split ? (void*)slabs : q.C, split ? (long)q.N : q.ldc, nullptr, nullptr, 0,
+                    split ? nullptr : q.bias, nullptr, 0, nullptr, q.M, q.N, q.Kseg, q.S, 1.0f, 0,
+                    split ? (int)GF_OUT_F32 : (relu ? (int)GF_RELU : 0), nullptr, split ? per[i] : 0};
+    g.tiles[i] = tiles[i];
+    g.first[i + 1] = g.first[i] + tiles[i] * rs[i];
+    c.ws[i] = slabs; c.C[i] = (bf16*)q.C; c.bias[i] = q.bias; c.ldc[i] = q.ldc; c.splits[i] = rs[i]; c.M[i] = q.M; c.N[i] = q.N; c.relu[i] = relu;
+    c.first[i + 1] = c.first[i] + (split ? (int)(((long)q.M * (q.N / 8) + 255) / 256) : 0);
+    if (split) wo += (long)rs[i] * q.M * q.N;
+    if (splits_out) splits_out[i] = rs[i];
+    word |= rs[i] << (16 + 5 * i);
+  }
+  g_last_variant[0] = word;
+  hipLaunchKernelGGL(gemm_nt_ring_group_kernel, dim3((unsigned)g.first[NT_GROUP_MAX]), dim3(512), 131072, (hipStream_t)stream, g);
+  STSWIN_CHECK_LAUNCH();
+  if (c.first[NT_GROUP_MAX] > 0) {
+    hipLaunchKernelGGL(nt_group_combine_kernel, dim3((unsigned)c.first[NT_GROUP_MAX]), dim3(256), 0, (hipStream_t)stream, c);
+    STSWIN_CHECK_LAUNCH();
+  }
   return 0;
 }
 
@@ -2232,7 +2363,9 @@
     }
     if (total <= cus) break;
   }
-  if (total > cus || total * 8 < (long)cus * 7) return declined;
+  bool conv_set = true;
+  for (int i = 0; i < count; ++i) conv_set = conv_set && pr[i].bseg > 0;
+  if (total > cus || (conv_set ? total * 4 < (long)cus * 3 : total * 8 < (long)cus * 7)) return declined;
   {
     long wsum = 0, wmax = 0;
     for (int i = 0; i < count; ++i) {
@@ -2241,7 +2374,7 @@
       wsum += (long)tiles[i] * nst[i] * wi;
       if (per * wi > wmax) wmax = per * wi;
     }
-    if (wmax * cus * 100 > wsum * 115) return declined;
+    if (wmax * cus * 100 > wsum * (conv_set ? 134 : 115)) return declined;
   }
   long ws_need = 0;
   for (int i = 0; i < count; ++i) {
@@ -2272,16 +2405,19 @@
   static int once_g = (int)hipFuncSetAttribute((const void*)gemm_tn_ring_group_kernel, hipFuncAttributeMaxDynamicSharedMemorySize, 131072) |
                       (int)hipFuncSetAttribute((const void*)gemm_tn_ring_group_static_kernel<0, 1, 2, -1>, hipFuncAttributeMaxDynamicSharedMemorySize, 131072) |
                       (int)hipFuncSetAttribute((const void*)gemm_tn_ring_group_static_kernel<0, 0, -1, -1>, hipFuncAttributeMaxDynamicSharedMemorySize, 131072) |
-                      (int)hipFuncSetAttribute((const void*)gemm_tn_ring_group_static_kernel<0, 0, 1, 2>, hipFuncAttributeMaxDynamicSharedMemorySize, 131072);
+                      (int)hipFuncSetAttribute((const void*)gemm_tn_ring_group_static_kernel<0, 0, 1, 2>, hipFuncAttributeMaxDynamicSharedMemorySize, 131072) |
+                      (int)hipFuncSetAttribute((const void*)gemm_tn_ring_group_static_kernel<3, 3, 3, -1>, hipFuncAttributeMaxDynamicSharedMemorySize, 131072);
   (void)once_g;
   g_last_variant[1] = STSWIN_VAR_TN_RING_PLAIN | STSWIN_VAR_TN_SLABS_BF16 | STSWIN_VAR_TN_FUSED | (rs[0] << 16);
   const bool m012 = count == 3 && g.mode[0] == 0 && g.mode[1] == 1 && g.mode[2] == 2;
   const bool m00 = count == 2 && g.mode[0] == 0 && g.mode[1] == 0;
   const bool m0012 = count == 4 && g.mode[0] == 0 && g.mode[1] == 0 && g.mode[2] == 1 && g.mode[3] == 2;
+  const bool m333 = count == 3 && g.mode[0] == 3 && g.mode[1] == 3 && g.mode[2] == 3;
   static const char* egd = getenv("STSWIN_TN_GROUP_DYNAMIC");
   if (m012 && !(egd && atoi(egd))) hipLaunchKernelGGL((gemm_tn_ring_group_static_kernel<0, 1, 2, -1>), dim3((unsigned)total), dim3(512), 131072, (hipStream_t)stream, g);
   else if (m00 && !(egd && atoi(egd))) hipLaunchKernelGGL((gemm_tn_ring_group_static_kernel<0, 0, -1, -1>), dim3((unsigned)total), dim3(512), 131072, (hipStream_t)stream, g);
   else if (m0012 && !(egd && atoi(egd))) hipLaunchKernelGGL((gemm_tn_ring_group_static_kernel<0, 0, 1, 2>), dim3((unsigned)total), dim3(512), 131072, (hipStream_t)stream, g);
+  else if (m333 && !(egd && atoi(egd))) hipLaunchKernelGGL((gemm_tn_ring_group_static_kernel<3, 3, 3, -1>), dim3((unsigned)total), dim3(512), 131072, (hipStream_t)stream, g);
   else
   hipLaunchKernelGGL(gemm_tn_ring_group_kernel, dim3((unsigned)total), dim3(512), 131072, (hipStream_t)stream, g);
   STSWIN_CHECK_LAUNCH();
diff --git a/stswincl_amd/headops.py b/stswincl_amd/headops.py
--- a/stswincl_amd/headops.py
+++ b/stswincl_amd/headops.py
@@ -160,7 +160,7 @@
         assert X.shape == (Mi, lin.width) and X.stride(1) == 1 and weight.shape[-1] == k
         y = torch.empty(Mo, lout.width, dtype=dt, device=x.device)
         tab = hip.stats_table(Mo, lout.width, x.device) if want_stats else None
-        ctx.tapskip = hip.GF_TAPSKIP if (k == 3 and stride == 1 and 2 * dil >= Hin + 3 and Mo <= 32768) else 0
+        ctx.tapskip = _tapskip(k, stride, dil, Hin, Mo)
         ctx.halo = (_HALO_CONV and bias is None and lin.is_identity and lout.is_identity and X.is_contiguous()
                     and hip.conv3x3_c64_ok(frames, Hin, Win, lin.width, lout.width, k, stride, pad, dil, dt))
         if ctx.halo:
@@ -187,11 +187,8 @@
         co, ci = weight.shape[:2]
         S = k * k
         g = dy.detach().to(dt).contiguous()
-        from .ops import wgrad_buffer
         dense = lin.is_identity and lout.is_identity
-        direct = dense and S == 1
-        dwp = (wgrad_buffer(weight, (lout.width, S * lin.width), X.device) if dense
-               else torch.empty(lout.width, S * lin.width, dtype=torch.float32, device=X.device))
+        dwp = _wgrad_dest(weight, lin, lout, S, X.device)
         if ctx.halo and _HALO_WGRAD and hip.conv3x3_c64_wgrad_ok(*ctx.geom):
             hip.conv3x3_c64_wgrad(g, X, dwp, *ctx.geom, tapminor=True)
             tapminor = True
@@ -213,34 +210,137 @@
                 ctx.link.put(dx)
                 dx = None
         hip.tn_join()
-        if direct or tapminor:
-            dw = dwp
-        elif dense:
-            dw = dwp.clone().view(co, S, ci).permute(0, 2, 1)
-        else:
-            dw = torch.zeros(co, ci, S, dtype=torch.float32, device=X.device)
-            d3 = dwp.view(lout.width, S, lin.width)
-            for oa, on, ob in lout.segs:
-                for ia, in_, ib in lin.segs:
-                    dw[oa:oa + on, ia:ia + in_, :] = d3[ob:ob + on, :, ib:ib + in_].permute(0, 2, 1)
-        db = None
-        if has_bias:
-            dbp = hip.zeros(lout.width, device=X.device)
-            hip.colsum(g, dbp)
-            db = lout.unpad_vec(dbp)
-        if dw is dwp:
-            dw = dw.view(co, ci, k, k)
-        else:
-            dw = dw.reshape(co, ci, k, k)
-            from .dp import grad_dest
-            slot = getattr(weight, "_stswin_grad_dest", None)
-            if dense and slot is not None and dwp.data_ptr() == slot[1].data_ptr():
-                dw = dwp.view(co, ci, k, k).copy_(dw)
-            elif not dense and slot is not None:
-                dest = grad_dest(weight)
-                if dest is not None:
-                    dw = dest.copy_(dw)
+        dw, db = _wgrad_finish(dwp, tapminor, g, weight, k, lin, lout, has_bias)
         return dx, dw, db, None, None, None, None, None
+
+
+def _wgrad_dest(weight, lin, lout, S, device):
+    from .ops import wgrad_buffer
+    if lin.is_identity and lout.is_identity:
+        return wgrad_buffer(weight, (lout.width, S * lin.width), device)
+    return torch.empty(lout.width, S * lin.width, dtype=torch.float32, device=device)
+
+
+def _wgrad_finish(dwp, tapminor, g, weight, k, lin, lout, has_bias):
+    co, ci = weight.shape[:2]
+    S = k * k
+    dense = lin.is_identity and lout.is_identity
+    if (dense and S == 1) or tapminor:
+        dw = dwp
+    elif dense:
+        dw = dwp.clone().view(co, S, ci).permute(0, 2, 1)
+    else:
+        dw = torch.zeros(co, ci, S, dtype=torch.float32, device=dwp.device)
+        d3 = dwp.view(lout.width, S, lin.width)
+        for oa, on, ob in lout.segs:
+            for ia, in_, ib in lin.segs:
+                dw[oa:oa + on, ia:ia + in_, :] = d3[ob:ob + on, :, ib:ib + in_].permute(0, 2, 1)
+    db = None
+    if has_bias:
+        dbp = hip.zeros(lout.width, device=dwp.device)
+        hip.colsum(g, dbp)
+        db = lout.unpad_vec(dbp)
+    if dw is dwp:
+        dw = dw.view(co, ci, k, k)
+    else:
+        dw = dw.reshape(co, ci, k, k)
+        from .dp import grad_dest
+        slot = getattr(weight, "_stswin_grad_dest", None)
+        if dense and slot is not None and dwp.data_ptr() == slot[1].data_ptr():
+            dw = dwp.view(co, ci, k, k).copy_(dw)
+        elif not dense and slot is not None:
+            dest = grad_dest(weight)
+            if dest is not None:
+                dw = dest.copy_(dw)
+    return dw, db
+
+
+def _tapskip(k, stride, dil, Hin, Mo):
+    return hip.GF_TAPSKIP if (k == 3 and stride == 1 and 2 * dil >= Hin + 3 and Mo <= 32768) else 0
+
+
+class ConvTokGroupFn(torch.autograd.Function):
+
+    @staticmethod
+    def forward(ctx, geoms, n, *args):
+        xs, wb = args[:n], args[n:]
+        dt = compute_dtype(xs[0])
+        X = xs[0].detach().to(dt)
+        assert all(x_.data_ptr() == xs[0].data_ptr() and x_.shape == xs[0].shape for x_ in xs) and X.stride(1) == 1
+        ys, cfgs, saved, problems = [], [], [], []
+        for i in range(n):
+            frames, Hin, Win, k, stride, pad, dil = geoms[i]
+            weight, bias = wb[2 * i], wb[2 * i + 1]
+            lin, lout = Layout.dense(weight.shape[1]), Layout.dense(weight.shape[0])
+            Hout, Wout, fmap, imap = _conv_maps(frames, Hin, Win, k, stride, pad, dil, X.device)
+            Mi, Mo = frames * Hin * Win, frames * Hout * Wout
+            assert X.shape == (Mi, lin.width) and weight.shape[-1] == k
+            y = torch.empty(Mo, lout.width, dtype=dt, device=X.device)
+            tapskip = _tapskip(k, stride, dil, Hin, Mo)
+            problems.append(dict(A=X, Bw=_conv_mats(weight, dt, lin, lout, False), out=y, M=Mo, a_rows=fmap, S=k * k,
+                                 bias=lout.pad_vec(bias) if bias is not None else None, flags=tapskip))
+            ys.append(y)
+            cfgs.append((k, lin, lout, bias is not None, Mi, Mo, tapskip))
+            saved += [weight, fmap, imap]
+        _gemm_nt_each_or_grouped(problems)
+        ctx.cfgs, ctx.n, ctx.dts = cfgs, n, (dt, xs[0].dtype)
+        ctx.save_for_backward(X, *saved)
+        return tuple(ys)
+
+    @staticmethod
+    @hip.tn_deferred_backward
+    def backward(ctx, *dys):
+        X, saved = ctx.saved_tensors[0], ctx.saved_tensors[1:]
+        n, (dt, in_dtype) = ctx.n, ctx.dts
+        gs, wprobs, problems, dxs = [], [], [], []
+        for i in range(n):
+            k, lin, lout, has_bias, Mi, Mo, tapskip = ctx.cfgs[i]
+            weight, fmap, imap = saved[3 * i:3 * i + 3]
+            S = k * k
+            g = dys[i].detach().to(dt).contiguous()
+            gs.append(g)
+            wprobs.append(dict(At=g, Bt=X, out=_wgrad_dest(weight, lin, lout, S, X.device), Mk=Mo, bt_rows=fmap,
+                               bseg=lin.width if fmap is not None else 0, overwrite=True, tapminor=S > 1))
+            if ctx.needs_input_grad[2 + i]:
+                dx = torch.empty(Mi, lin.width, dtype=dt, device=X.device)
+                problems.append(dict(A=g, Bw=_conv_mats(weight, dt, lin, lout, True), out=dx, M=Mi, a_rows=imap, S=S, flags=tapskip))
+                dxs.append(dx)
+            else:
+                dxs.append(None)
+        if len(wprobs) > 1 and dt == torch.bfloat16 and nt_group_enabled() and hip.gemm_tn_group(wprobs):
+            tapminor = [q["tapminor"] for q in wprobs]
+        else:
+            tapminor = []
+            for q in wprobs:
+                hip.gemm_tn(q["At"], q["Bt"], q["out"], Mk=q["Mk"], bt_rows=q["bt_rows"], bseg=q["bseg"], overwrite=True, tapminor=q["tapminor"])
+                tapminor.append(q["tapminor"] and hip.last_tn_tapminor())
+        _gemm_nt_each_or_grouped(problems)
+        hip.tn_join()
+        grads = []
+        for i in range(n):
+            k, lin, lout, has_bias, Mi, Mo, tapskip = ctx.cfgs[i]
+            grads += list(_wgrad_finish(wprobs[i]["out"], tapminor[i], gs[i], saved[3 * i], k, lin, lout, has_bias))
+        return (None, None, *[dx.to(in_dtype) if dx is not None else None for dx in dxs], *grads)
+
+
+def _gemm_nt_each_or_grouped(problems):
+    if not problems or (len(problems) > 1 and hip.gemm_nt_group(problems)):
+        return
+    for q in problems:
+        hip.gemm_nt(q["A"], q["Bw"], q["out"], M=q["M"], a_rows=q["a_rows"], S=q["S"], bias=q.get("bias"), flags=q["flags"])
+
+
+def nt_group_enabled() -> bool:
+    return os.environ.get("STSWIN_NT_GROUP", "1") != "0"
+
+
+def conv_tokens_group(x_tok, convs, frames, Hin, Win):
+    rev = list(convs)[::-1]
+    geoms = tuple((frames, Hin, Win, c.kernel_size[0], c.stride[0], c.padding[0], c.dilation[0]) for c in rev)
+    wb = []
+    for c in rev:
+        wb += [c.weight, c.bias]
+    return list(ConvTokGroupFn.apply(geoms, len(rev), *([x_tok] * len(rev)), *wb))[::-1]
 
 
 class GradLink:
@@ -674,6 +774,17 @@
         y = conv_tokens(x_tok, conv, frames, Hh, Ww, lin, lout, stats=False)[0]
         return self.bn(y, bn, relu=relu, groups=groups, lay=lout, out=out)
 
+    def conv_bn_relu_group(self, x_tok, branches, geom):
+        frames, Hh, Ww = geom
+        convs = [c for c, _, _ in branches]
+        if not (nt_group_enabled() and 2 <= len(convs) <= hip.NT_GROUP_MAX and compute_dtype(x_tok) == torch.bfloat16
+                and frames * Hh * Ww < 8192 and len({c.in_channels for c in convs}) == 1
+                and all(c.kernel_size[0] > 1 and c.stride[0] == 1 and 2 * c.padding[0] == c.dilation[0] * (c.kernel_size[0] - 1)
+                        and c.groups == 1 and c.in_channels % KGRAN == 0 and c.out_channels % KGRAN == 0 for c in convs)):
+            return [self.conv_bn_relu(x_tok, c, b, geom, out=o) for c, b, o in branches]
+        ys = conv_tokens_group(x_tok, convs, frames, Hh, Ww)
+        return [self.bn(y, b, lay=Layout.dense(c.out_channels), out=o) for y, (c, b, o) in zip(ys, branches)]
+
     def bn(self, y, bn, relu=True, groups=1, il_frames=0, lay=None, stats=None, out=None):
         training = bn.training or bn.running_mean is None
         if not (training and _sync_world(bn) > 1):
diff --git a/stswincl_amd/hip.py b/stswincl_amd/hip.py
--- a/stswincl_amd/hip.py
+++ b/stswincl_amd/hip.py
@@ -54,6 +54,8 @@
     if unparsed:
         raise StswinHipError(f"{HEADER_PATH}: cannot bind the declaration of {sorted(unparsed)}")
     consts = {name: _c_value(name, expr) for name, expr in re.findall(r"^[ \t]*#[ \t]*define[ \t]+STSWIN_(\w+)[ \t]+(\S.*)$", text, flags=re.M)}
+    for body in re.findall(r"\benum\s*\{([^{}]*)\}", text):
+        consts.update({name: _c_value(name, expr) for name, expr in re.findall(r"\bSTSWIN_(\w+)\s*=\s*([^,]+)", body)})
     return protos, consts
 
 
@@ -560,6 +562,54 @@
     if cs_table is not None:
         _check(load().stswin_cs_reduce(_p(cs_table), M, N, _p(colsum_out), _stream()), "cs_reduce")
     return out
+
+
+class _NtProblem(ctypes.Structure):
+    _fields_ = [("A", ctypes.c_void_p), ("lda", ctypes.c_long), ("a_rows", ctypes.c_void_p),
+                ("B", ctypes.c_void_p), ("ldb", ctypes.c_long),
+                ("C", ctypes.c_void_p), ("ldc", ctypes.c_long),
+                ("bias", ctypes.c_void_p),
+                ("M", ctypes.c_int), ("N", ctypes.c_int), ("Kseg", ctypes.c_int), ("S", ctypes.c_int),
+                ("flags", ctypes.c_int), ("splits", ctypes.c_int)]
+
+
+LAST_NT_GROUP_SPLITS: list = []
+
+
+def gemm_nt_group(problems) -> bool:
+    n = len(problems)
+    if n == 0:
+        return True
+    if n > NT_GROUP_MAX or any(q["A"].dtype != torch.bfloat16 or q["Bw"].dtype != torch.bfloat16 or q["out"].dtype != torch.bfloat16
+                               for q in problems):
+        return False
+    arr = (_NtProblem * n)()
+    flops = 0.0
+    for i, q in enumerate(problems):
+        A, Bw, out, S = q["A"], q["Bw"], q["out"], q.get("S", 1)
+        N, Ktot = Bw.shape
+        assert Ktot % S == 0 and A.shape[1] >= Ktot // S and out.shape[1] == N
+        ar, bias = q.get("a_rows"), q.get("bias")
+        arr[i] = _NtProblem(A.data_ptr(), _ld(A), ar.data_ptr() if ar is not None else None, Bw.data_ptr(), _ld(Bw), out.data_ptr(), _ld(out),
+                            bias.data_ptr() if bias is not None else None, q["M"], N, Ktot // S, S, q.get("flags", 0), q.get("splits", 0))
+        flops += 2.0 * q["M"] * N * Ktot
+    lib = load()
+    need = lib.stswin_gemm_nt_group_scratch(n, arr)
+    ws = scratch(problems[0]["A"].device, need) if need > 0 else None
+    sp = (_c_int * n)()
+    name = "gemm_nt_bf16"
+    if _SHAPE_NAMES:
+        name += " group " + " + ".join(f"M={q['M']} N={q['Bw'].shape[0]} K={q['Bw'].shape[1]}" for q in problems)
+    with _Span(name, flops) as span:
+        rc = lib.stswin_gemm_nt_group(n, arr, _p(ws), ws.numel() if ws is not None else 0, sp, _stream())
+        if rc == NT_GROUP_DECLINED:
+            span.cancel()
+    if rc == NT_GROUP_DECLINED:
+        return False
+    _check(rc, "gemm_nt_group")
+    LAST_NT_GROUP_SPLITS[:] = list(sp)
+    _log_variant("nt_group", (n, problems[0]["M"]) + tuple(sp), 0)
+    return True
 
 
 def gemm_nt_qkv_fp8(A: torch.Tensor, Bw: torch.Tensor, *, M: int, a_rows=None, bias=None, scale: float = 1.0, scale_cols: int = 0,
diff --git a/stswincl_amd/net/Ours/ASPP.py b/stswincl_amd/net/Ours/ASPP.py
--- a/stswincl_amd/net/Ours/ASPP.py
+++ b/stswincl_amd/net/Ours/ASPP.py
@@ -34,9 +34,8 @@
         buf, (v1, v2, v3, v4, v5) = H.concat_buffer(x.shape[0], [nb] * 5, H.compute_dtype(x), x.device)
         with H.syncbn_group() as g:
             g.conv_bn_relu(x, self.conv_1x1_1, self.bn_conv_1x1_1, geom, out=v1)
-            g.conv_bn_relu(x, self.conv_3x3_1, self.bn_conv_3x3_1, geom, out=v2)
-            g.conv_bn_relu(x, self.conv_3x3_2, self.bn_conv_3x3_2, geom, out=v3)
-            g.conv_bn_relu(x, self.conv_3x3_3, self.bn_conv_3x3_3, geom, out=v4)
+            g.conv_bn_relu_group(x, [(self.conv_3x3_1, self.bn_conv_3x3_1, v2), (self.conv_3x3_2, self.bn_conv_3x3_2, v3),
+                                     (self.conv_3x3_3, self.bn_conv_3x3_3, v4)], geom)
             g.conv_bn_relu(H.AvgPoolTokFn.apply(x, f), self.conv_1x1_2, self.bn_conv_1x1_2, (f, 1, 1))
         o1, o2, o3, o4, img = g.results()
         img = H.BroadcastTokFn.apply(img, h * w, v5)
```

After: 613.6 frames/s (median of 6 runs). Within noise of the previous version (+0.7%).
